# kamperh/segmentalist

Measured on AMD Instinct MI355X. Metric: Gibbs sweeps/sec (10k utts, D=100, K=1000) at 1/2/4/8 MI355X, higher is better.
Workload: dtype fp16 one-product filter + fp16x2 second stage, float32 reference arithmetic for the results; 1 GPU; SegmentalKMeansWordseg batch-synchronous sweep (BASELINE.json configs[2]); utterances=10000, landmarks_per_utt=20, n_slices_max=6, embeddings=1050000, D=100, K=1000, parallelism=utterance shards x1, ONE all-gather of the packed block statistics per sweep, collective=none (single process), sweep_launch=plain launches, corpus=one device holds all rows, device_memory_allocated_bytes_rank0=1237140480, components_after=815

## Files before the change

### include/segk.h

```cpp
#ifndef SEGK_H
#define SEGK_H

#include <stdint.h>

#ifdef __cplusplus
extern "C" {
#endif

#define SEGK_OK 0
#define SEGK_ERR_ARG (-1)
#define SEGK_ERR_HIP (-2)
#define SEGK_ERR_NO_DEVICE (-3)
#define SEGK_ERR_UNSUPPORTED (-4)

#define SEGK_F32 0
#define SEGK_F64 1

typedef struct segk_ctx segk_ctx;

int32_t segk_create(int32_t device_id, segk_ctx **out_ctx);
int32_t segk_destroy(segk_ctx *ctx);
const char *segk_last_error(void);
#define SEGK_ABI_VERSION 15
int32_t segk_abi_version(void);

int32_t segk_profile_enable(segk_ctx *ctx, int32_t on);
int32_t segk_profile_read(segk_ctx *ctx, float *ms_out, int64_t *rows_out, int32_t max);
int32_t segk_profile_last_kind(segk_ctx *ctx);
int32_t segk_profile_last_launches(segk_ctx *ctx);

int32_t segk_graph_begin(segk_ctx *ctx, void *stream);
int32_t segk_graph_end(segk_ctx *ctx, void *stream, void **exec_out);
int32_t segk_graph_launch(segk_ctx *ctx, void *exec, void *stream);
int32_t segk_graph_destroy(segk_ctx *ctx, void *exec);

typedef struct segk_corpus {
    const void *X;
    const float *X32;
    int32_t x_dtype;
    int32_t D;
    int64_t n_emb;
    int64_t ldx;
    int64_t ld32;
    const float *xnorm;
    const int32_t *vec_ids;
    const double *durations;
    const int32_t *lengths;
    int32_t n_utt;
    int32_t N_max;
    const void *Xb3;
    int32_t sp_pieces;
    int32_t band_W;
    const int32_t *band_ids;
    const double *band_dur;
} segk_corpus;

int32_t segk_corpus_prepare(segk_ctx *ctx, const segk_corpus *c, float *X32_out, float *xnorm_out,
                            void *stream);
int64_t segk_corpus_b3_bytes(int64_t n_emb, int32_t D);
int32_t segk_corpus_prepare_b3(segk_ctx *ctx, const segk_corpus *c, void *Xb3_out, int32_t pieces,
                               void *stream);

typedef struct segk_kmeans {
    void *means;
    double *mean_numerators;
    int64_t *counts;
    const void *random_means;
    int32_t *assignments;
    int32_t *K;
    int32_t K_max;
    float *tiles;
    double *mnorm_max;
    float *tiles_b3;
} segk_kmeans;

int64_t segk_kmeans_tiles_floats(int32_t K_max, int32_t D);
int32_t segk_kmeans_mark_duplicates(segk_ctx *ctx, const segk_corpus *c, const segk_kmeans *m, int32_t *n_marked,
                                    void *stream);
int64_t segk_kmeans_tiles_b3_floats(int32_t K_max, int32_t D);

int32_t segk_kmeans_init_stats(segk_ctx *ctx, const segk_corpus *c, segk_kmeans *m, void *stream);

int32_t segk_kmeans_prepare(segk_ctx *ctx, const segk_corpus *c, segk_kmeans *m, void *stream);

typedef struct segk_cand {
    int32_t *k;
    float *f;
    double *s;
    int32_t *queue;
    int32_t *count;
} segk_cand;

int32_t segk_kmeans_score(segk_ctx *ctx, const segk_corpus *c, const segk_kmeans *m,
                          const int32_t *ids, int64_t row0, int64_t n, const segk_cand *cand,
                          int32_t *status, void *stream);

int32_t segk_kmeans_score_hinted(segk_ctx *ctx, const segk_corpus *c, const segk_kmeans *m,
                                 const int32_t *ids, int64_t row0, int64_t n, const segk_cand *cand,
                                 const int32_t *hint_remap, int32_t *status, void *stream);

int32_t segk_kmeans_clear_queue(segk_ctx *ctx, const segk_cand *cand, void *stream);
int32_t segk_kmeans_filter(segk_ctx *ctx, const segk_corpus *c, const segk_kmeans *m,
                           const int32_t *ids, int64_t row0, int64_t n, const segk_cand *cand,
                           void *stream);
int32_t segk_kmeans_resolve(segk_ctx *ctx, const segk_corpus *c, const segk_kmeans *m,
                            const int32_t *ids, int64_t row0, int64_t n, const segk_cand *cand,
                            int32_t *status, void *stream);

int32_t segk_kmeans_stage_counts(segk_ctx *ctx, const segk_cand *cand, int32_t *out, void *stream);

int32_t segk_kmeans_hint_feedback(segk_ctx *ctx, uint32_t *launched, uint32_t *seen, int32_t *permille);

int32_t segk_kmeans_delta_stats(segk_ctx *ctx, int32_t *out);

int32_t segk_kmeans_exact_max(segk_ctx *ctx, const segk_corpus *c, const segk_kmeans *m,
                              const int32_t *ids, int64_t n, const segk_cand *cand,
                              double *out_max, int32_t *out_arg, void *stream);

int32_t segk_kmeans_neg_sqrd_norm(segk_ctx *ctx, const segk_corpus *c, const segk_kmeans *m,
                                  int64_t row, void *out, void *stream);

int32_t segk_kmeans_segment(segk_ctx *ctx, const segk_corpus *c, const segk_kmeans *m,
                            const int32_t *utts, int32_t utt0, int32_t n_utts,
                            int32_t n_slices_min, int32_t n_slices_max, double wip,
                            const segk_cand *cand, uint8_t *boundaries, int32_t *old_tok,
                            int32_t *new_tok, int32_t *new_k, int32_t *n_old, int32_t *n_new,
                            int32_t *n_flag, double *out_total, int32_t *status, void *stream);

int32_t segk_kmeans_update_utt(segk_ctx *ctx, const segk_corpus *c, segk_kmeans *m,
                               int32_t utt, const int32_t *old_tok, const int32_t *new_tok,
                               const int32_t *new_k, const int32_t *n_old, const int32_t *n_new,
                               int32_t *status, void *stream);

int32_t segk_kmeans_add_item(segk_ctx *ctx, const segk_corpus *c, segk_kmeans *m, int64_t i,
                             int32_t k, int32_t *status, void *stream);
int32_t segk_kmeans_del_item(segk_ctx *ctx, const segk_corpus *c, segk_kmeans *m, int64_t i,
                             int32_t *status, void *stream);
int32_t segk_kmeans_clean_components(segk_ctx *ctx, const segk_corpus *c, segk_kmeans *m,
                                     int32_t *status, void *stream);

int32_t segk_kmeans_del_component(segk_ctx *ctx, const segk_corpus *c, segk_kmeans *m, int32_t k,
                                  int32_t *status, void *stream);

int32_t segk_kmeans_sequential_sweep(segk_ctx *ctx, const segk_corpus *c, segk_kmeans *m,
                                     const int32_t *order, int32_t n_order, int32_t n_slices_min,
                                     int32_t n_slices_max, double wip, const segk_cand *cand,
                                     uint64_t *keys_scratch, uint8_t *boundaries, int32_t *old_tok,
                                     int32_t *new_tok, int32_t *new_k, int32_t *n_old, int32_t *n_new,
                                     int32_t *n_flag, double *out_total, int32_t *status, void *stream);

int64_t segk_kmeans_batch_record_words(int32_t K_max, int32_t D, int32_t n_blocks_local, int32_t flag_cap,
                                       int32_t flag_row_bytes);
int32_t segk_kmeans_batch_scratch_words(int32_t K_max, int64_t n_slots, int32_t n_blocks_local, int64_t *sorted_words,
                                        int64_t *koff_words);
int32_t segk_kmeans_batch_partials(segk_ctx *ctx, const segk_corpus *c, const segk_kmeans *m,
                                   const int32_t *blk_lo, int32_t n_blocks_local,
                                   const int32_t *new_tok, const int32_t *new_k, const int32_t *n_flag,
                                   const double *out_total, int32_t *sorted_scratch,
                                   int32_t *koff_scratch, double *record, int32_t flag_cap, int32_t flag_rows,
                                   double *out_scalars, void *stream);
int32_t segk_kmeans_batch_finalize(segk_ctx *ctx, const segk_corpus *c, segk_kmeans *m,
                                   int32_t utt_lo, int32_t utt_hi, const double *records,
                                   int32_t n_blocks_total, int32_t n_blocks_per_rank,
                                   int64_t rank_stride, int32_t flag_cap, int32_t flag_rows, int32_t my_rank,
                                   int32_t *new_k, int32_t *remap_scratch, double *out_scalars,
                                   int32_t *status, void *stream);
int32_t segk_kmeans_batch_record(segk_ctx *ctx, const segk_corpus *c, const segk_kmeans *m, int32_t utt_lo,
                                 int32_t utt_hi, const int32_t *new_tok, const int32_t *new_k,
                                 const int32_t *status, double *out_scalars, void *stream);
int32_t segk_kmeans_assignments_from_tokens(segk_ctx *ctx, const segk_corpus *c, segk_kmeans *m,
                                            int32_t utt_lo, int32_t utt_hi, const int32_t *new_tok,
                                            const int32_t *new_k, const int32_t *n_new,
                                            void *stream);

int32_t segk_kmeans_sum_neg_sqrd_norm(segk_ctx *ctx, const segk_corpus *c, const segk_kmeans *m,
                                      double *out, void *stream);

typedef struct segk_fbgmm {
    int32_t cov_type;
    int32_t K_max;
    double alpha;
    double lms;
    double k_0, v_0;
    const double *prior_a;
    const double *prior_b;
    const double *prior_c;
    double *stat_a;
    double *stat_b;
    double *log_prod;
    double *pred;
    int64_t *counts;
    int32_t *assignments;
    int32_t *K;
    int64_t *lm_unigram;
    int64_t *lm_bigram;
    double lm_lambda, lm_a, lm_b;
    double *kconst;
} segk_fbgmm;

int32_t segk_fbgmm_record_metrics(segk_ctx *ctx, const segk_corpus *c, const struct segk_fbgmm *f,
                                  int32_t urn, double urn_a, double *out, void *stream);

int32_t segk_fbgmm_init_stats(segk_ctx *ctx, const segk_corpus *c, segk_fbgmm *f, void *stream);

int32_t segk_fbgmm_update(segk_ctx *ctx, const segk_corpus *c, segk_fbgmm *f, int32_t op,
                          int32_t utt, int64_t item, int32_t k, const uint8_t *boundaries,
                          void *stream);

int32_t segk_fbgmm_score(segk_ctx *ctx, const segk_corpus *c, const segk_fbgmm *f,
                         const int32_t *ids, int64_t row0, int64_t n, double *out, void *stream);

int32_t segk_fbgmm_pred_vector(segk_ctx *ctx, const segk_corpus *c, const segk_fbgmm *f,
                               int64_t row, double *out, void *stream);

int32_t segk_unigram_segment(segk_ctx *ctx, const segk_corpus *c, int32_t utt, int32_t viterbi,
                             int32_t n_slices_min, int32_t n_slices_max, double wip,
                             double time_power_term, double log_p_continue, double anneal_temp,
                             const double *score, const double *ustream, int64_t *ucursor,
                             int64_t ucap, uint8_t *boundaries, int32_t *new_tok, int32_t *n_new,
                             double *out_logprob, int32_t *status, void *stream);

int32_t segk_fbgmm_assign(segk_ctx *ctx, const segk_corpus *c, segk_fbgmm *f, int32_t utt,
                          int32_t map_assign, int32_t j_prev, double anneal_temp, const int32_t *new_tok,
                          const int32_t *n_new, const double *ustream, int64_t *ucursor,
                          int64_t ucap, int32_t *status, void *stream);

int32_t segk_fbgmm_sequential_sweep(segk_ctx *ctx, const segk_corpus *c, segk_fbgmm *f, const int32_t *order, int32_t n_order,
                                    const int32_t *row_start, int32_t viterbi, int32_t map_assign, int32_t n_slices_min,
                                    int32_t n_slices_max, double wip, double time_power_term, double log_p_continue,
                                    double anneal_temp_fb, double anneal_temp_am, double *score, const double *ustream,
                                    int64_t *ucursor, int64_t ucap, uint8_t *boundaries, int32_t *new_tok, int32_t *n_new,
                                    double *out_logprob, int32_t *status, void *stream);

int32_t segk_fbgmm_gibbs_items(segk_ctx *ctx, const segk_corpus *c, segk_fbgmm *f, const int32_t *ids,
                               int64_t n, int32_t consider_unassigned, double anneal_temp,
                               const double *ustream, int64_t *ucursor, int64_t ucap, int32_t *status,
                               void *stream);

typedef struct {
    int32_t n_slices, n_blocks;
    int32_t u_max;
    int32_t fast_dp;
    const int32_t *utt_range;
    const int32_t *row_range;
    double *partials;
    double *cnt;
    double *mean_t, *q_t;
    double *lconst, *zconst, *half;
    double *scal;
    int32_t *slot;
    int32_t *lm_tok;
    uint64_t seed;
    float *y;
    int64_t ldy;
    float *tiles32;
    void *y16;
    float *tiles16;
    float *rows32;
    double *consts16;
    const double *prior_rows;
    const double *centre;
    float *tab32;
} segk_fbatch;

int32_t segk_fbb_collect(segk_ctx *ctx, const segk_corpus *c, const uint8_t *boundaries,
                         int32_t *new_tok, int32_t *n_new, void *stream);
// ... 87 lines not shown
```

### segmentalist_amd/_abi.py

```python
import ctypes as C
import os
import subprocess

_HERE = os.path.dirname(os.path.abspath(__file__))
LIB_PATH = os.environ.get("SEGK_LIB_PATH") or os.path.join(_HERE, "libsegk.so")

SEGK_F32, SEGK_F64 = 0, 1
SEGK_ERR_UNSUPPORTED = -4
ABI_VERSION = 15


class SegkError(RuntimeError):
    pass


class Corpus(C.Structure):
    _fields_ = [
        ("X", C.c_void_p), ("X32", C.c_void_p), ("x_dtype", C.c_int32), ("D", C.c_int32),
        ("n_emb", C.c_int64), ("ldx", C.c_int64), ("ld32", C.c_int64), ("xnorm", C.c_void_p),
        ("vec_ids", C.c_void_p), ("durations", C.c_void_p), ("lengths", C.c_void_p),
        ("n_utt", C.c_int32), ("N_max", C.c_int32), ("Xb3", C.c_void_p), ("sp_pieces", C.c_int32), ("band_W", C.c_int32),
        ("band_ids", C.c_void_p), ("band_dur", C.c_void_p),
    ]


class KMeansDev(C.Structure):
    _fields_ = [
        ("means", C.c_void_p), ("mean_numerators", C.c_void_p), ("counts", C.c_void_p),
        ("random_means", C.c_void_p), ("assignments", C.c_void_p), ("K", C.c_void_p),
        ("K_max", C.c_int32), ("tiles", C.c_void_p), ("mnorm_max", C.c_void_p), ("tiles_b3", C.c_void_p),
    ]


class FbatchDev(C.Structure):
    _fields_ = [
        ("n_slices", C.c_int32), ("n_blocks", C.c_int32), ("u_max", C.c_int32), ("fast_dp", C.c_int32),
        ("utt_range", C.c_void_p), ("row_range", C.c_void_p), ("partials", C.c_void_p), ("cnt", C.c_void_p),
        ("mean_t", C.c_void_p), ("q_t", C.c_void_p), ("lconst", C.c_void_p), ("zconst", C.c_void_p),
        ("half", C.c_void_p), ("scal", C.c_void_p), ("slot", C.c_void_p), ("lm_tok", C.c_void_p),
        ("seed", C.c_uint64), ("y", C.c_void_p), ("ldy", C.c_int64), ("tiles32", C.c_void_p),
        ("y16", C.c_void_p), ("tiles16", C.c_void_p), ("rows32", C.c_void_p), ("consts16", C.c_void_p),
        ("prior_rows", C.c_void_p), ("centre", C.c_void_p), ("tab32", C.c_void_p),
    ]


class CandDev(C.Structure):
    _fields_ = [("k", C.c_void_p), ("f", C.c_void_p), ("s", C.c_void_p), ("queue", C.c_void_p),
                ("count", C.c_void_p)]


class FbgmmDev(C.Structure):
    _fields_ = [
        ("cov_type", C.c_int32), ("K_max", C.c_int32), ("alpha", C.c_double), ("lms", C.c_double),
        ("k_0", C.c_double), ("v_0", C.c_double), ("prior_a", C.c_void_p), ("prior_b", C.c_void_p),
        ("prior_c", C.c_void_p), ("stat_a", C.c_void_p), ("stat_b", C.c_void_p), ("log_prod", C.c_void_p),
        ("pred", C.c_void_p), ("counts", C.c_void_p), ("assignments", C.c_void_p), ("K", C.c_void_p),
        ("lm_unigram", C.c_void_p), ("lm_bigram", C.c_void_p), ("lm_lambda", C.c_double), ("lm_a", C.c_double),
        ("lm_b", C.c_double), ("kconst", C.c_void_p),
    ]


_P = C.c_void_p
_i32, _i64, _f64, _u64 = C.c_int32, C.c_int64, C.c_double, C.c_uint64
_CP, _KP, _FP, _DP = C.POINTER(Corpus), C.POINTER(KMeansDev), C.POINTER(FbgmmDev), C.POINTER(CandDev)
_BP = C.POINTER(FbatchDev)

SIGNATURES = {
    "segk_create": (_i32, [_i32, C.POINTER(_P)]),
    "segk_destroy": (_i32, [_P]),
    "segk_last_error": (C.c_char_p, []),
    "segk_abi_version": (_i32, []),
    "segk_corpus_prepare": (_i32, [_P, _CP, _P, _P, _P]),
    "segk_kmeans_tiles_floats": (_i64, [_i32, _i32]),
    "segk_kmeans_prepare": (_i32, [_P, _CP, _KP, _P]),
    "segk_kmeans_mark_duplicates": (_i32, [_P, _CP, _KP, _P, _P]),
    "segk_kmeans_init_stats": (_i32, [_P, _CP, _KP, _P]),
    "segk_kmeans_score": (_i32, [_P, _CP, _KP, _P, _i64, _i64, _DP, _P, _P]),
    "segk_kmeans_score_hinted": (_i32, [_P, _CP, _KP, _P, _i64, _i64, _DP, _P, _P, _P]),
    "segk_kmeans_clear_queue": (_i32, [_P, _DP, _P]),
    "segk_kmeans_filter": (_i32, [_P, _CP, _KP, _P, _i64, _i64, _DP, _P]),
    "segk_kmeans_resolve": (_i32, [_P, _CP, _KP, _P, _i64, _i64, _DP, _P, _P]),
    "segk_kmeans_stage_counts": (_i32, [_P, _DP, C.POINTER(_i32), _P]),
    "segk_kmeans_hint_feedback": (_i32, [_P, C.POINTER(C.c_uint32), C.POINTER(C.c_uint32), C.POINTER(_i32)]),
    "segk_kmeans_delta_stats": (_i32, [_P, C.POINTER(_i32)]),
    "segk_kmeans_exact_max": (_i32, [_P, _CP, _KP, _P, _i64, _DP, _P, _P, _P]),
    "segk_kmeans_neg_sqrd_norm": (_i32, [_P, _CP, _KP, _i64, _P, _P]),
    "segk_kmeans_segment": (_i32, [_P, _CP, _KP, _P, _i32, _i32, _i32, _i32, _f64, _DP, _P, _P, _P, _P, _P, _P,
                                   _P, _P, _P, _P]),
    "segk_dp_tri": (_i32, [_P, _i32, _P, _P, _P, _i32, _i32, _i32, _f64, _f64, _P, _i64, _P, _i64, _P, _P, _P,
                           _P, _i64, _P]),
    "segk_kmeans_update_utt": (_i32, [_P, _CP, _KP, _i32, _P, _P, _P, _P, _P, _P, _P]),
    "segk_kmeans_sequential_sweep": (_i32, [_P, _CP, _KP, _P, _i32, _i32, _i32, _f64, _DP, _P, _P, _P, _P, _P, _P, _P, _P, _P,
                                            _P, _P]),
    "segk_kmeans_add_item": (_i32, [_P, _CP, _KP, _i64, _i32, _P, _P]),
    "segk_kmeans_del_item": (_i32, [_P, _CP, _KP, _i64, _P, _P]),
    "segk_kmeans_clean_components": (_i32, [_P, _CP, _KP, _P, _P]),
    "segk_kmeans_del_component": (_i32, [_P, _CP, _KP, _i32, _P, _P]),
    "segk_kmeans_batch_record_words": (_i64, [_i32, _i32, _i32, _i32, _i32]),
    "segk_kmeans_batch_scratch_words": (_i32, [_i32, _i64, _i32, C.POINTER(_i64), C.POINTER(_i64)]),
    "segk_kmeans_batch_partials": (_i32, [_P, _CP, _KP, _P, _i32, _P, _P, _P, _P, _P, _P, _P, _i32, _i32, _P, _P]),
    "segk_kmeans_batch_finalize": (_i32, [_P, _CP, _KP, _i32, _i32, _P, _i32, _i32, _i64, _i32, _i32, _i32, _P, _P, _P, _P,
                                          _P]),
    "segk_kmeans_batch_record": (_i32, [_P, _CP, _KP, _i32, _i32, _P, _P, _P, _P, _P]),
    "segk_kmeans_assignments_from_tokens": (_i32, [_P, _CP, _KP, _i32, _i32, _P, _P, _P, _P]),
    "segk_kmeans_sum_neg_sqrd_norm": (_i32, [_P, _CP, _KP, _P, _P]),
    "segk_fbgmm_record_metrics": (_i32, [_P, _CP, _FP, _i32, _f64, _P, _P]),
    "segk_fbgmm_init_stats": (_i32, [_P, _CP, _FP, _P]),
    "segk_fbgmm_update": (_i32, [_P, _CP, _FP, _i32, _i32, _i64, _i32, _P, _P]),
    "segk_fbgmm_score": (_i32, [_P, _CP, _FP, _P, _i64, _i64, _P, _P]),
    "segk_fbgmm_pred_vector": (_i32, [_P, _CP, _FP, _i64, _P, _P]),
    "segk_unigram_segment": (_i32, [_P, _CP, _i32, _i32, _i32, _i32, _f64, _f64, _f64, _f64, _P, _P, _P, _i64, _P,
                                    _P, _P, _P, _P, _P]),
    "segk_fbgmm_assign": (_i32, [_P, _CP, _FP, _i32, _i32, _i32, _f64, _P, _P, _P, _P, _i64, _P, _P]),
    "segk_fbgmm_gibbs_items": (_i32, [_P, _CP, _FP, _P, _i64, _i32, _f64, _P, _P, _i64, _P, _P]),
    "segk_fbgmm_sequential_sweep": (_i32, [_P, _CP, _FP, _P, _i32, _P, _i32, _i32, _i32, _i32, _f64, _f64, _f64, _f64, _f64,
                                           _P, _P, _P, _i64, _P, _P, _P, _P, _P, _P]),
    "segk_fbb_collect": (_i32, [_P, _CP, _P, _P, _P, _P]),
    "segk_fbb_partials": (_i32, [_P, _CP, _FP, _BP, _i32, _i32, _i32, _P, _P, _P]),
    "segk_fbb_prepare": (_i32, [_P, _CP, _FP, _BP, _i32, _P]),
    "segk_fbb_score": (_i32, [_P, _CP, _FP, _BP, _i32, _i32, _i32, _P, _P, _P]),
    "segk_fbb_score_diag32": (_i32, [_P, _CP, _FP, _BP, _i32, _i32, _i32, _P, _P, _P]),
    "segk_calibrate_vlog": (_i32, [_P, C.POINTER(_f64), _P]),
    "segk_fbb_make_y": (_i32, [_P, _CP, _BP, _P]),
    "segk_fbb_prior_rows": (_i32, [_P, _CP, _FP, _P, _P]),
    "segk_fbb_score_f32": (_i32, [_P, _CP, _FP, _BP, _P, _i64, _P, _P]),
    "segk_fbb_segment": (_i32, [_P, _CP, _FP, _BP, _i32, _i32, _i32, _P, _u64, _i32, _i32, _f64, _f64, _f64, _P, _P,
                                _P, _P, _P, _P, _P]),
    "segk_fbb_assign": (_i32, [_P, _CP, _FP, _BP, _i32, _i32, _i32, _P, _u64, _f64, _P, _P, _P, _i64, _P]),
    "segk_fbb_assign_diag32": (_i32, [_P, _CP, _FP, _BP, _i32, _i32, _i32, _P, _u64, _f64, _P, _P, _P]),
    "segk_fbb_segment_map": (_i32, [_P, _CP, _FP, _BP, _i32, _i32, _i32, _P, _u64, _i32, _i32, _f64, _f64, _P, _P, _P, _P,
                                    _P, _P, _P]),
    "segk_fbb_assign_map": (_i32, [_P, _CP, _FP, _BP, _i32, _i32, _i32, _P, _u64, _P, _P, _i32, _P]),
    "segk_fbb_step_diag32": (_i32, [_P, _CP, _FP, _BP, _i32, _i32, _i32, _P, _u64, _i32, _i32, _f64, _f64, _f64, _f64,
                                    _P, _P, _P, _P, _P, _P, _P]),
    "segk_fbb_token_scores": (_i32, [_P, _CP, _FP, _BP, _P, _i64, _P, _i64, _P]),
    "segk_fbb_set_probe": (_i32, [_P, _P, _P, _i64]),
    "segk_fbi_assign": (_i32, [_P, _CP, _FP, _BP, _i32, _i32, _i32, _P, _u64, _f64, _i32, _P, _P, _P, _i64, _P]),
    "segk_fbt_assign": (_i32, [_P, _CP, _FP, _BP, _i32, _i32, _i32, _P, _P, _u64, _f64, _P, _P, _P, _i64, _P]),
    "segk_fbb_lm_apply": (_i32, [_P, _CP, _FP, _BP, _i32, _i32, _P]),
    "segk_fbb_lm_fill": (_i32, [_P, _CP, _FP, _BP, _i32, _i32, _i32, _P, _P, _P, _P]),
    "segk_fbb_canonical": (_i32, [_P, _CP, _FP, _BP, _P, _P]),
    "segk_corpus_prepare_b3": (_i32, [_P, _CP, _P, _i32, _P]),
    "segk_corpus_b3_bytes": (_i64, [_i64, _i32]),
    "segk_kmeans_tiles_b3_floats": (_i64, [_i32, _i32]),
    "segk_graph_begin": (_i32, [_P, _P]),
    "segk_graph_end": (_i32, [_P, _P, C.POINTER(_P)]),
    "segk_graph_launch": (_i32, [_P, _P, _P]),
    "segk_graph_destroy": (_i32, [_P, _P]),
    "segk_profile_enable": (_i32, [_P, _i32]),
    "segk_profile_read": (_i32, [_P, _P, _P, _i32]),
    "segk_profile_last_kind": (_i32, [_P]),
    "segk_profile_last_launches": (_i32, [_P]),
    "segk_logsumexp": (_f64, [_P, _i64]),
    "segk_draw": (_i32, [_P, _i64, _f64]),
    "segk_sum_doubles": (_f64, [_P, _i64]),
    "segk_sum_ints": (_i64, [_P, _i64]),
    "segk_sum_log": (_f64, [_P, _i64]),
    "segk_sum_square_a_times_b": (_f64, [_P, _P, _i64]),
}

_lib = None


def build(force=False):
    if force and os.path.exists(LIB_PATH):
        os.remove(LIB_PATH)
    subprocess.check_call(["make", "-C", os.path.join(_HERE, "csrc"), "-s"])
    if not os.path.exists(LIB_PATH):
        raise SegkError("building libsegk.so failed")


def lib():
    global _lib
    if _lib is None:
        if not os.path.exists(LIB_PATH):
            raise SegkError(
                "%s not found: build it with `python -c 'import __graft_entry__ as g; g.build()'` "
                "or `make -C segmentalist_amd/csrc`.  segmentalist_amd has no CPU fallback." % LIB_PATH)
        L = C.CDLL(LIB_PATH)
        for name, (res, args) in SIGNATURES.items():
            try:
                fn = getattr(L, name)
            except AttributeError:
                raise SegkError("libsegk.so does not export %s (stale build?)" % name)
            fn.restype = res
            fn.argtypes = args
        got = int(L.segk_abi_version())
        if got != ABI_VERSION:
            raise SegkError("libsegk.so reports ABI version %d, this binding is written against %d (include/segk.h "
                            "SEGK_ABI_VERSION): rebuild the library (`make -C segmentalist_amd/csrc`)" % (got, ABI_VERSION))
        _lib = L
    return _lib


def check(rc):
    if rc != 0:
        raise SegkError("libsegk error %d: %s" % (rc, lib().segk_last_error().decode()))


_ctx = {}


def ctx(device_index=None):
    import torch
    if not torch.cuda.is_available():
        raise SegkError("no ROCm device visible: segmentalist_amd runs its hot path on MI355X only "
                        "(there is no CPU fallback)")
    if device_index is None:
        device_index = torch.cuda.current_device()
    if device_index not in _ctx:
        h = C.c_void_p()
        check(lib().segk_create(int(device_index), C.byref(h)))
        _ctx[device_index] = h
    return _ctx[device_index]


def stream():
    import torch
    return C.c_void_p(torch.cuda.current_stream().cuda_stream)


def ptr(t):
    if t is None:
        return None
    return C.c_void_p(t.data_ptr())
```

### segmentalist_amd/csrc/segk_host.cpp

```cpp
#include <math.h>
#include <stdarg.h>
#include <stdlib.h>
#include <map>
#include <mutex>
#include <tuple>

#include "segk_internal.h"

static thread_local char g_err[512] = "";

void segk_set_error(const char *fmt, ...)
{
    va_list ap;
    va_start(ap, fmt);
    vsnprintf(g_err, sizeof(g_err), fmt, ap);
    va_end(ap);
}

int segk_ws_realloc(segk_ctx *ctx, void **buf, size_t bytes, hipStream_t st)
{
    SEGK_REQUIRE(!ctx->capturing, "workspaces must exist before a graph capture (run the sequence once first)");
    SEGK_CHECK_HIP(hipStreamSynchronize(st));
    if (*buf) (void)hipFree(*buf);
    *buf = nullptr;
// ... 103 lines not shown
        if (ctx->fb_fp_dev) (void)hipFree(ctx->fb_fp_dev);
        if (ctx->fbs_buf) (void)hipFree(ctx->fbs_buf);
        if (ctx->flag_ovf) (void)hipFree(ctx->flag_ovf);
        if (ctx->hint_part) (void)hipFree(ctx->hint_part);
        if (ctx->ws_u64) (void)hipFree(ctx->ws_u64);
        if (ctx->hint_fb) (void)hipFree(ctx->hint_fb);
        if (ctx->delta_buf) (void)hipFree(ctx->delta_buf);
        if (ctx->delta_host) (void)hipHostFree((void *)ctx->delta_host);
        if (ctx->pre_thr) (void)hipFree(ctx->pre_thr);
        if (ctx->band_mask) (void)hipFree(ctx->band_mask);
        if (ctx->miss_host) (void)hipHostFree((void *)ctx->miss_host);
        if (ctx->brute_ws) (void)hipFree(ctx->brute_ws);
        if (ctx->pre_queue) (void)hipFree(ctx->pre_queue);
        if (ctx->row_hash) (void)hipFree(ctx->row_hash);
        if (ctx->rb_sorted) (void)hipFree(ctx->rb_sorted);
        if (ctx->rb_koff) (void)hipFree(ctx->rb_koff);
        if (ctx->rb_misc) (void)hipFree(ctx->rb_misc);
        if (ctx->rb_term) (void)hipFree(ctx->rb_term);
        if (ctx->fc_terms) (void)hipFree(ctx->fc_terms);
        if (ctx->fcb_ll) (void)hipFree(ctx->fcb_ll);
        if (ctx->fbi_z) (void)hipFree(ctx->fbi_z);
        if (ctx->fbt_tok) (void)hipFree(ctx->fbt_tok);
        for (int i = 0; i < SEGK_PROF_SLOTS; i++)
            for (int j = 0; j < 2; j++)
                if (ctx->prof_ev[i][j]) (void)hipEventDestroy(ctx->prof_ev[i][j]);
    }
    free(ctx);
    return SEGK_OK;
}

int32_t segk_profile_enable(segk_ctx *ctx, int32_t on)
{
    SEGK_REQUIRE(ctx, "ctx");
    if (on)
        for (int i = 0; i < SEGK_PROF_SLOTS; i++)
            for (int j = 0; j < 2; j++)
                if (!ctx->prof_ev[i][j]) SEGK_CHECK_HIP(hipEventCreate(&ctx->prof_ev[i][j]));
    ctx->prof_on = on > 0 ? on : 0;
    ctx->prof_calls = 0;
    ctx->prof_n = 0;
    if (on) ctx->prof_kind = -1;
    return SEGK_OK;
}

int32_t segk_profile_read(segk_ctx *ctx, float *ms_out, int64_t *rows_out, int32_t max)
{
    SEGK_REQUIRE(ctx && ms_out && rows_out, "arguments");
    const int have = ctx->prof_n < SEGK_PROF_SLOTS ? ctx->prof_n : SEGK_PROF_SLOTS;
    const int n = have < max ? have : max;
    for (int i = 0; i < n; i++) {
        const int slot = (ctx->prof_n - n + i) % SEGK_PROF_SLOTS;
        SEGK_CHECK_HIP(hipEventSynchronize(ctx->prof_ev[slot][1]));
        SEGK_CHECK_HIP(hipEventElapsedTime(&ms_out[i], ctx->prof_ev[slot][0], ctx->prof_ev[slot][1]));
        rows_out[i] = ctx->prof_rows[slot];
    }
    return n;
}

int32_t segk_profile_last_kind(segk_ctx *ctx)
{
    return ctx ? ctx->prof_kind : -1;
}

int32_t segk_profile_last_launches(segk_ctx *ctx)
{
    return ctx && ctx->prof_launches > 0 ? ctx->prof_launches : 1;
}

int32_t segk_graph_begin(segk_ctx *ctx, void *stream)
{
    SEGK_REQUIRE(ctx && stream, "segk_graph_begin needs a context and a non-default stream");
    SEGK_REQUIRE(!ctx->capturing, "a capture is already open on this context");
    SEGK_REQUIRE(!ctx->prof_on, "segk_profile_enable(1) records events between launches: not inside a capture");
    SEGK_CHECK_HIP(hipStreamBeginCapture((hipStream_t)stream, hipStreamCaptureModeRelaxed));
    ctx->capturing = 1;
    return SEGK_OK;
}

int32_t segk_graph_end(segk_ctx *ctx, void *stream, void **exec_out)
{
    SEGK_REQUIRE(ctx && stream && exec_out, "arguments");
    SEGK_REQUIRE(ctx->capturing, "no capture open");
    ctx->capturing = 0;
    *exec_out = nullptr;
    hipGraph_t graph = nullptr;
    SEGK_CHECK_HIP(hipStreamEndCapture((hipStream_t)stream, &graph));
    hipGraphExec_t exec = nullptr;
    const hipError_t e = hipGraphInstantiate(&exec, graph, nullptr, nullptr, 0);
    (void)hipGraphDestroy(graph);
    if (e != hipSuccess) {
        segk_set_error("segk_graph_end: hipGraphInstantiate -> %s", hipGetErrorString(e));
        return SEGK_ERR_HIP;
    }
    *exec_out = (void *)exec;
    return SEGK_OK;
}

int32_t segk_graph_launch(segk_ctx *ctx, void *exec, void *stream)
{
    (void)ctx;
    SEGK_REQUIRE(exec, "exec");
    SEGK_CHECK_HIP(hipGraphLaunch((hipGraphExec_t)exec, (hipStream_t)stream));
    return SEGK_OK;
}

int32_t segk_graph_destroy(segk_ctx *ctx, void *exec)
{
    (void)ctx;
    if (exec) SEGK_CHECK_HIP(hipGraphExecDestroy((hipGraphExec_t)exec));
    return SEGK_OK;
}

int32_t segk_kmeans_stage_counts(segk_ctx *ctx, const segk_cand *cand, int32_t *out, void *stream)
{
    SEGK_REQUIRE(ctx && cand && cand->count && out, "arguments");
    hipStream_t st = (hipStream_t)stream;
    out[0] = -1;
    int32_t hdr[16] = {0};
    if (ctx->pre_queue) SEGK_CHECK_HIP(hipMemcpyAsync(hdr, ctx->pre_queue, sizeof(hdr), hipMemcpyDeviceToHost, st));
    SEGK_CHECK_HIP(hipMemcpyAsync(&out[1], cand->count, sizeof(int32_t), hipMemcpyDeviceToHost, st));
    SEGK_CHECK_HIP(hipStreamSynchronize(st));
    if (ctx->pre_queue) {
        out[0] = 0;
        for (int i = 0; i < 16; i++) out[0] += hdr[i];
    }
    return SEGK_OK;
}

int32_t segk_kmeans_hint_feedback(segk_ctx *ctx, uint32_t *launched, uint32_t *seen, int32_t *permille)
{
    SEGK_REQUIRE(ctx && launched && seen && permille, "arguments");
    *launched = ctx->miss_seq;
    *seen = 0;
    *permille = 0;
    if (ctx->miss_host) {
        const unsigned long long w = *ctx->miss_host;
        *seen = (uint32_t)(w >> 32);
        *permille = (int32_t)(w & 0xffffffffull);
    }
    return SEGK_OK;
}

int32_t segk_kmeans_delta_stats(segk_ctx *ctx, int32_t *out)
{
    SEGK_REQUIRE(ctx && out, "arguments");
    out[0] = -1; out[1] = 0; out[2] = 0; out[3] = 0;
    if (ctx->delta_host) {
        out[0] = ctx->delta_host[0] - 1;
        for (int i = 1; i < 4; i++) out[i] = ctx->delta_host[i];
    }
    return SEGK_OK;
}

double segk_logsumexp(const double *a, int64_t n)
{
    double mx = a[0], s = 0.0;
    for (int64_t j = 1; j < n; j++)
        if (a[j] > mx) mx = a[j];
    for (int64_t j = 0; j < n; j++) s += exp(a[j] - mx);
    return log(s) + mx;
}

int32_t segk_draw(const double *p_k, int64_t n, double u)
{
    for (int64_t i = 0; i < n; i++) {
        u = u - p_k[i];
        if (u < 0) return (int32_t)i;
    }
    return (int32_t)(n - 1);
}

double segk_sum_doubles(const double *y, int64_t n)
{
    double s = y[0];
    for (int64_t i = 1; i < n; i++) s += y[i];
    return s;
}

int64_t segk_sum_ints(const int64_t *y, int64_t n)
{
    int64_t s = y[0];
    for (int64_t i = 1; i < n; i++) s += y[i];
    return s;
}

double segk_sum_log(const double *y, int64_t n)
{
    double s = log(y[0]);
    for (int64_t i = 1; i < n; i++) s += log(y[i]);
    return s;
}

double segk_sum_square_a_times_b(const double *a, const double *b, int64_t n)
{
    double s = 0.0;
    for (int64_t i = 0; i < n; i++) s += a[i] * a[i] * b[i];
    return s;
}

}


static std::mutex g_attr_mu;
static std::map<std::pair<int, const void *>, size_t> g_dyn_lds;
static std::map<std::tuple<int, const void *, int, size_t>, int> g_occupancy;

hipError_t segk_dyn_lds(const void *fn, size_t lds)
{
    if (lds <= 48 * 1024) return hipSuccess;
    int dev = 0;
    hipError_t e = hipGetDevice(&dev);
    if (e != hipSuccess) return e;
    std::lock_guard<std::mutex> lock(g_attr_mu);
    size_t &have = g_dyn_lds[std::make_pair(dev, fn)];
    if (have >= lds) return hipSuccess;
    e = hipFuncSetAttribute(fn, hipFuncAttributeMaxDynamicSharedMemorySize, (int)lds);
    if (e == hipSuccess) have = lds;
    return e;
}

hipError_t segk_occupancy(const void *fn, int threads, size_t lds, int *wg_per_cu)
{
    int dev = 0;
    hipError_t e = hipGetDevice(&dev);
    if (e != hipSuccess) return e;
    {
        std::lock_guard<std::mutex> lock(g_attr_mu);
        auto it = g_occupancy.find(std::make_tuple(dev, fn, threads, lds));
        if (it != g_occupancy.end()) {
            *wg_per_cu = it->second;
            return hipSuccess;
        }
    }
    e = segk_dyn_lds(fn, lds);
    if (e != hipSuccess) return e;
    int occ = 0;
    e = hipOccupancyMaxActiveBlocksPerMultiprocessor(&occ, fn, threads, lds);
    if (e != hipSuccess) return e;
    *wg_per_cu = occ > 0 ? occ : 1;
    std::lock_guard<std::mutex> lock(g_attr_mu);
    g_occupancy[std::make_tuple(dev, fn, threads, lds)] = *wg_per_cu;
    return hipSuccess;
}
```

### segmentalist_amd/csrc/segk_internal.h

```cpp
#pragma once
#include <hip/hip_runtime.h>
#include <stdint.h>
#include <stdio.h>
#include <stdlib.h>
#include <string.h>

#include "../../include/segk.h"

#define SEGK_WS_ENTRIES (256 * 1024)
#define SEGK_PROF_SLOTS 256

struct segk_ctx {
    int device_id;
    int n_cu;
    char arch[64];
    int32_t *ws_k;
    float *ws_f;
    unsigned long long *ws_u64;
    int32_t *pre_queue;
    int64_t pre_cap;
    float *sp2_part;
    int32_t *sp2_ticket;
    int64_t sp2_blocks;
    void *chain_buf;
    size_t chain_bytes;
    double *fb_ktab;
    int64_t fb_ktab_n;
    double fb_ktab_v0;
    int fb_ktab_D;
    double *fb_ptab;
    int64_t fb_ptab_n;
    unsigned long long fb_ptab_fp;
    int64_t fb_ptab_rows;
    int fb_ptab_D;
    unsigned long long *fb_fp_dev;
    int fb_ptab_nt, fb_ptab_cov;
    double fb_ptab_k0, fb_ptab_v0;
    void *fbchain_buf;
    size_t fbchain_bytes;
    void *fbchain_lm;
    size_t fbchain_lm_bytes;
    void *fbchain_terms;
    size_t fbchain_terms_bytes;
    int32_t *fbs_buf;
    size_t fbs_bytes;
    const void *fbb_scal_zeroed;
    const void *fbb_scal_stream;
    int prof_launches;
    int32_t *defer_zero;
    int pre_zeroed;
    int capturing;
    unsigned long long *row_hash;
    const void *row_hash_means;
    int32_t *rb_sorted;
    int64_t rb_cap;
    int32_t *rb_koff;
    int rb_K;
    int32_t *rb_misc;
    double *rb_term;
    double *fc_terms;
    int64_t fc_terms_n;
    double *fcb_ll;
    int64_t fcb_ll_n;
    double *fbi_z;
    int64_t fbi_z_n;
    int32_t *fbt_tok;
    int64_t fbt_tok_n;
    void *hint_part;
    size_t hint_part_bytes;
    float *pre_thr;
    int64_t pre_thr_cap;
    void *band_mask;
    size_t band_mask_bytes;
    volatile unsigned long long *miss_host;
    unsigned long long *miss_dev;
    unsigned int miss_seq;
    void *delta_buf;
    size_t delta_bytes;
    unsigned int delta_seq;
    int delta_valid;
    const void *delta_key[6];
    int64_t delta_key_n[5];
    int delta_pending;
    const void *delta_pending_remap, *delta_pending_K, *delta_pending_stream;
    int delta_pending_cap, delta_pending_budget, delta_pending_seq;
    volatile int32_t *delta_host;
    int32_t *delta_host_dev;
    void *hint_fb;
    unsigned int hint_fb_launch;
    unsigned long long *brute_ws;
    int64_t brute_ws_cap;
    int32_t *flag_ovf;
    int64_t flag_ovf_cap;
    double *probe_alpha, *probe_ll;
    int64_t probe_ll_ld;
    int prof_on, prof_n, prof_kind;
    unsigned int prof_calls;
    hipEvent_t prof_ev[SEGK_PROF_SLOTS][2];
    int64_t prof_rows[SEGK_PROF_SLOTS];
};

static inline bool segk_prof_now(segk_ctx *ctx)
{
    if (!ctx->prof_on) return false;
    return (ctx->prof_calls++ % (unsigned int)ctx->prof_on) == 0u;
}


void segk_set_error(const char *fmt, ...);

static inline int segk_env_int(const char *name, int dflt)
{
    const char *e = getenv(name);
    return e ? atoi(e) : dflt;
}

#ifdef SEGK_DEV
static inline int segk_dev_env(const char *name) { return segk_env_int(name, 0); }
#else
static inline int segk_dev_env(const char *) { return 0; }
#endif

int segk_rows_by_label(segk_ctx *ctx, const int32_t *labels, int64_t n, int K_max, const int32_t **blk_lo, int *n_blocks,
                       const int32_t **sorted, const int32_t **koff, void *stream);

#define SEGK_CHECK_HIP(expr)                                                                  \
    do {                                                                                      \
        hipError_t _e = (expr);                                                               \
        if (_e != hipSuccess) {                                                               \
            segk_set_error("%s:%d: %s -> %s", __FILE__, __LINE__, #expr, hipGetErrorString(_e)); \
            return SEGK_ERR_HIP;                                                              \
        }                                                                                     \
    } while (0)

#define SEGK_REQUIRE(cond, msg)                                             \
    do {                                                                    \
        if (!(cond)) {                                                      \
            segk_set_error("%s:%d: %s (%s)", __FILE__, __LINE__, msg, #cond); \
            return SEGK_ERR_ARG;                                            \
        }                                                                   \
    } while (0)

#define SEGK_LAUNCH_CHECK() SEGK_CHECK_HIP(hipGetLastError())

#define SEGK_REFUSE_FULLCOV(f, who)                                                                                 \
    do {                                                                                                            \
        if ((f) && (f)->cov_type == 2) {                                                                            \
            segk_set_error("%s: full-covariance components (cov_type 2) are not supported by this entry point", who); \
            return SEGK_ERR_UNSUPPORTED;                                                                            \
        }                                                                                                           \
    } while (0)
int segk_fc_check(const segk_corpus *c, const segk_fbgmm *f, const char *who);
int segk_fc_init_stats(segk_ctx *ctx, const segk_corpus *c, segk_fbgmm *f, void *stream);
int segk_fc_update(const segk_corpus *c, segk_fbgmm *f, int op, int utt, int64_t item, int k, const uint8_t *boundaries, void *stream);
int segk_fc_score(segk_ctx *ctx, const segk_corpus *c, const segk_fbgmm *f, const int32_t *ids, int64_t row0, int64_t n, double *out,
                  void *stream);
int segk_fc_pred_vector(const segk_corpus *c, const segk_fbgmm *f, int64_t row, double *out, void *stream);
int segk_fc_assign(const segk_corpus *c, segk_fbgmm *f, int utt, int map_assign, double anneal_temp, const int32_t *new_tok,
                   const int32_t *n_new, const double *ustream, int64_t *ucursor, int64_t ucap, int32_t *status, void *stream);
int segk_fc_gibbs_items(const segk_corpus *c, segk_fbgmm *f, const int32_t *ids, int64_t n, int consider_unassigned,
                        double anneal_temp, const double *ustream, int64_t *ucursor, int64_t ucap, int32_t *status, void *stream);

int segk_ws_realloc(segk_ctx *ctx, void **buf, size_t bytes, hipStream_t st);
template <class T, class N>
static inline int segk_ws_grow(segk_ctx *ctx, T **buf, N *have, N need, size_t bytes, hipStream_t st)
{
    if (*have >= need) return SEGK_OK;
    *have = 0;
    if (int rc = segk_ws_realloc(ctx, (void **)buf, bytes, st)) return rc;
    *have = need;
    return SEGK_OK;
}

hipError_t segk_dyn_lds(const void *fn, size_t lds);
hipError_t segk_occupancy(const void *fn, int threads, size_t lds, int *wg_per_cu);

static inline __host__ __device__ int segk_G(int D) { return (D + 3) / 4; }
#define SEGK_G_BUCKETS {1, 2, 4, 6, 8, 10, 13, 16, 20, 25, 26, 28, 32, 33, 34, 40, 50, 64, 75, 100}
static inline __host__ __device__ int segk_gmax(int D)
{
    const int b[] = SEGK_G_BUCKETS;
    int G = segk_G(D);
    for (unsigned i = 0; i < sizeof(b) / sizeof(b[0]); i++)
        if (G <= b[i]) return b[i];
    return -1;
}
static inline __host__ __device__ int segk_tile_stride(int D)
{
    int gm = segk_gmax(D);
    if (gm < 0) gm = segk_G(D);
    int f = gm * 128 + 32;
    return (f + 1023) / 1024 * 1024;
}
static inline __host__ __device__ int segk_n_tiles(int K_max) { return (K_max + 31) / 32; }

#define SEGK_SP_HEADER 64
static inline __host__ __device__ int segk_b3_dim(int pos)
{
    const int q = pos & 15, h = q >> 3, i = q & 7;
    return (pos & ~15) + 8 * (i >> 2) + 4 * h + (i & 3);
}
static inline __host__ __device__ int segk_b3_kp(int D) { return (D + 15) & ~15; }
static inline __host__ __device__ int segk_sp_tile_stride(int D, int P)
{
    return ((segk_b3_kp(D) / 16) * P * 256 + 32 + 1023) / 1024 * 1024;
}

int segk_launch_score_lse(segk_ctx *ctx, const float *Y, int64_t ldy, int D2, const int32_t *ids, int64_t row0, int64_t n,
                          const float *tiles, int n_tiles, double norm, double *out, void *stream);

int segk_sp_prepare_rows(const float *Y, int64_t ldy, int64_t n, int D2, void *img, void *stream);
int segk_sp_prepare_tiles(const float *rows, const double *consts, const double *rowmax2, int K, int D2, float *tiles_sp,
                          const void *ximg, void *stream);
int segk_launch_score_lse_sp(segk_ctx *ctx, const void *ximg, int D2, const int32_t *ids, int64_t row0, int64_t n,
                             const float *tiles_sp, int n_tiles, double norm, double *out, void *stream,
                             const int32_t *n_tiles_dev = nullptr);
int segk_launch_score_mat_sp(const void *ximg, int D2, const int32_t *ids, int64_t n, const float *tiles_sp, int n_tiles,
                             float *mat, int64_t mat_ld, void *stream, const int32_t *n_tiles_dev = nullptr, int tiles_hint = 0);
```

### segmentalist_amd/csrc/segk_kmeans_dev.h

```cpp
#pragma once
#include <stdlib.h>

#include "segk_internal.h"

typedef float f32x16 __attribute__((ext_vector_type(16)));

#define NEG_INF_D (-__builtin_huge_val())
#define NEG_INF_F (-__builtin_huge_valf())

template <typename T, typename TM, typename TX>
__device__ __forceinline__ T sqd(const TM &m, const TX *x, int d)
{
    T delta = (T)m[d] - (T)x[d];
    return delta * delta;
}

template <typename T, typename TM, typename TX>
__device__ T pw_base(const TM &m, const TX *x, int n)
{
    if (n < 8) {
        T res = (T)0;
        for (int i = 0; i < n; i++) res += sqd<T>(m, x, i);
        return res;
    }
// ... 525 lines not shown
            int i = idx - G * 128;
            int comp = tile * 32 + i;
            v = (comp < K_max) ? (float)(-0.5 * nrm[i]) : -3.0e38f;
        }
        T[idx] = v;
    }
}

__device__ __forceinline__ void dev_prepare_sp_tile(const float *means, int K_max, int D, float *tiles, const double *mnorm2,
                                                    const unsigned char *ximg, const double *consts, const int tile)
{
    typedef SegkPiece::T T;
    constexpr int P = 2;
    const int KS = segk_b3_kp(D) / 16;
    const int stride = segk_sp_tile_stride(D, P);
    const int eb = sp_exponent((float)(sqrt(*mnorm2) * (1.0 + 1e-6)));
    const int ea = ((const int *)ximg)[1];
    if (tile == 0 && threadIdx.x == 0) ((int *)tiles)[0] = eb;
    float *Tt = tiles + 1024 + (int64_t)tile * stride;
    T *Tb = (T *)Tt;
    __shared__ double nrm[32];
    constexpr int PITCH = 129;
    __shared__ float rowsl[32 * PITCH];
    const bool staged = D <= 128;
    const float *src = means + (int64_t)tile * 32 * D;
    if (staged) {
        const int nrow = K_max - tile * 32 < 32 ? K_max - tile * 32 : 32;
        for (int idx = threadIdx.x; idx < 32 * D; idx += blockDim.x) {
            const int ci = idx / D, d = idx - ci * D;
            rowsl[ci * PITCH + d] = ci < nrow ? src[idx] : 0.f;
        }
    }
    __syncthreads();
    SEGK_TSTAMP(4, 5);
    auto elem = [&](int ci, int d) -> float { return staged ? rowsl[ci * PITCH + d] : src[(int64_t)ci * D + d]; };
    {
        const int ci = threadIdx.x >> 3, sub = threadIdx.x & 7;
        const int comp = tile * 32 + ci;
        double s = 0.0, rs = 0.0;
        if (comp < K_max)
            for (int d = sub; d < D; d += 8) {
                const float mv = elem(ci, d);
                double v = (double)mv;
                s += v * v;
                rs += sp_resid2(ldexpf(mv, eb));
            }
        s += __shfl_xor(s, 1);
        s += __shfl_xor(s, 2);
        s += __shfl_xor(s, 4);
        if (sub == 0) nrm[ci] = s;
        rs += __shfl_xor(rs, 1);
        rs += __shfl_xor(rs, 2);
        rs += __shfl_xor(rs, 4);
        const float em = (float)(ldexp(sqrt(rs), -eb) * (1.0 + 1e-6));
        if (sub == 0 && comp < K_max) atomicMax((unsigned int *)tiles + 1, __float_as_uint(em));
    }
    __syncthreads();
    SEGK_TSTAMP(4, 6);
    for (int pr = threadIdx.x; pr < KS * 64; pr += blockDim.x) {
        const int sidx = pr >> 6, lane = pr & 63;
        const int ci = lane & 31;
        const bool live = tile * 32 + ci < K_max;
        SegkPiece::V8 out[P];
#pragma unroll
        for (int i = 0; i < 8; i++) {
            const int d = segk_b3_dim(16 * sidx + 8 * (lane >> 5) + i);
            const float v = (live && d < D) ? ldexpf(elem(ci, d), eb) : 0.f;
            T pc[P];
            split_sp(v, pc);
#pragma unroll
            for (int q = 0; q < P; q++) out[q][i] = pc[q];
        }
#pragma unroll
        for (int q = 0; q < P; q++) *reinterpret_cast<SegkPiece::V8 *>(Tb + ((sidx * P + q) * 64 + lane) * 8) = out[q];
    }
    for (int idx = threadIdx.x; idx < stride - KS * P * 256; idx += blockDim.x) {
        float v = 0.f;
        if (idx < 32) {
            const int comp = tile * 32 + idx;
            if (consts) v = (comp < K_max && consts[comp] > -1e37) ? (float)ldexp(consts[comp], ea + eb) : -3.0e38f;
            else v = (comp < K_max) ? (float)ldexp(-0.5 * nrm[idx], ea + eb) : -3.0e38f;
        }
        Tt[KS * P * 256 + idx] = v;
    }
}

#define SEGK_DUP_TB 4096
__device__ __forceinline__ void dev_dup_table(unsigned long long *keys, int32_t *first, const unsigned long long *row_hash, int K_max)
{
    const int tid = threadIdx.x;
    for (int i = tid; i < SEGK_DUP_TB; i += blockDim.x) { keys[i] = 0ull; first[i] = 0x7fffffff; }
    __syncthreads();
    for (int k = tid; k < K_max; k += blockDim.x) {
        const unsigned long long h = row_hash[k];
        for (unsigned slot = (unsigned)(h >> 20) & (SEGK_DUP_TB - 1);; slot = (slot + 1) & (SEGK_DUP_TB - 1)) {
            const unsigned long long prev = atomicCAS(&keys[slot], 0ull, h);
            if (prev == 0ull || prev == h) { atomicMin(&first[slot], k); break; }
        }
    }
    __syncthreads();
}
__device__ __forceinline__ int dev_dup_first(const unsigned long long *keys, const int32_t *first, unsigned long long h)
{
    unsigned slot = (unsigned)(h >> 20) & (SEGK_DUP_TB - 1);
    while (keys[slot] != h) slot = (slot + 1) & (SEGK_DUP_TB - 1);
    return first[slot];
}

static __global__ void k_zero_two(int32_t *a, int32_t *b)
{
    if (threadIdx.x == 0) *a = 0;
    if (threadIdx.x < 16) b[threadIdx.x] = 0;
}
static inline void segk_flush_deferred_zero(segk_ctx *ctx, hipStream_t st)
{
    if (ctx && ctx->defer_zero) {
        hipLaunchKernelGGL(k_zero_two, dim3(1), dim3(64), 0, st, ctx->defer_zero, ctx->pre_queue);
        ctx->defer_zero = nullptr;
    }
}

int segk_kmeans_prepare_impl(segk_ctx *ctx, const segk_corpus *c, segk_kmeans *m, void *stream, bool mnorm_zeroed);
int segk_dispatch_score_f32(segk_ctx *ctx, const segk_corpus *c, const segk_kmeans *m, const ScoreArgs &A, hipStream_t st);
int segk_dispatch_score_sp(segk_ctx *ctx, const ScoreArgs &A, int ks, hipStream_t st);
int segk_launch_sp_second(segk_ctx *ctx, const ScoreArgs &B, int ks, hipStream_t st);
int segk_launch_clean(const segk_corpus *c, segk_kmeans *m, int32_t *status, hipStream_t st, int32_t *relog = nullptr);
int segk_launch_seq_chain(segk_ctx *ctx, const segk_corpus *c, segk_kmeans *m, const int32_t *order, int n_order, int n_slices_max,
                          double wip, uint8_t *boundaries, int32_t *old_tok, int32_t *new_tok, int32_t *new_k, int32_t *n_old,
                          int32_t *n_new, int32_t *n_flag, double *out_total, int32_t *status, hipStream_t st);
int segk_dispatch_score_pre(segk_ctx *ctx, const ScoreArgs &A, int ks, hipStream_t st);
#define SEGK_HINT_MAX_TPR 32
#define SEGK_HINT_MAX_RANGES 4
struct HintPlan {
    int max_tiles;
    int n_ranges, tpr;
    size_t map_bytes;
};
static inline bool segk_hint_plan(int K_max, int ks, int n_tiles, HintPlan *p)
{
    const size_t lds_bytes = 160 * 1024, tile_bytes = (size_t)(ks * 256 + 32) * sizeof(float);
    p->map_bytes = (size_t)((K_max + 3) & ~3) * sizeof(int32_t);
    if (p->map_bytes + tile_bytes > lds_bytes) return false;
    p->max_tiles = (int)((lds_bytes - p->map_bytes) / tile_bytes);
    if (p->max_tiles > SEGK_HINT_MAX_TPR) p->max_tiles = SEGK_HINT_MAX_TPR;
    p->n_ranges = (n_tiles + p->max_tiles - 1) / p->max_tiles;
    if (p->n_ranges < 1) p->n_ranges = 1;
    p->tpr = (n_tiles + p->n_ranges - 1) / p->n_ranges;
    return p->n_ranges <= SEGK_HINT_MAX_RANGES;
}
int segk_dispatch_score_hint(segk_ctx *ctx, const ScoreArgs &A, const int32_t *remap, const int32_t *K_dev, int64_t n_emb, int ks, hipStream_t st);

#define SEGK_DELTA_MODE 1
#define SEGK_DELTA_SKIP 2
#define SEGK_PREP_THREADS 256
#define SEGK_PREP_COLS 4
struct DeltaPrepArgs {
    const float *tiles_hdr;
    int n_tiles, stride;
    int K_max, D;
    const float *means32;
    const int32_t *remap;
    const int32_t *K_dev;
    int valid;
    int hint_valid;
    int cap;
    int budget;
    int seq;
    int redo;
    int32_t *ctl, *colchg, *meanchg;
    float *snap_img;
    float *packed;
    float *snap_means;
};
struct DeltaPrepLds { int chg[32], slot[32], nonid, last, n_chg, n_nonid, old[5]; };

static __device__ __forceinline__ void delta_prep_means_rows(const DeltaPrepArgs &P, int wg, int n_wg)
{
    const int lane = threadIdx.x & 63, wave = threadIdx.x >> 6;
    constexpr int NWV = SEGK_PREP_THREADS / 64;
    for (int k = wg * NWV + wave; k < P.K_max; k += n_wg * NWV) {
        const int *cur = (const int *)(P.means32 + (int64_t)k * P.D);
        int *snap = (int *)(P.snap_means + (int64_t)k * P.D);
        bool chg = false;
        for (int d = lane; d < P.D; d += 64) {
            const int c = cur[d];
            chg |= c != snap[d];
            snap[d] = c;
        }
        const bool any = __any(chg);
        if (lane == 0) {
            const bool before = P.redo && P.meanchg[k] != 0;
            P.meanchg[k] = (any || before || !P.hint_valid) ? 1 : 0;
            if (any) atomicAdd(P.ctl + 5 + (P.seq & 1), 1);
        }
    }
}

static __device__ __forceinline__ bool delta_prep_tile(const DeltaPrepArgs &P, const int KS, const int t, const int e_cur, DeltaPrepLds &S)
{
    const int tid = threadIdx.x, lane = tid & 63, wave = tid >> 6;
    constexpr int NWV = SEGK_PREP_THREADS / 64;
    const int TL = KS * 256 + 32, c_off = KS * 512;
    const int c = lane & 31;
    const float *g = P.tiles_hdr + 1024 + (int64_t)t * P.stride;
    const float *q = P.snap_img + 4 + (int64_t)t * TL;
    const bool all = !P.valid || e_cur != (P.redo ? P.ctl[18] : ((const int *)P.snap_img)[0]);
    if (tid < 32) S.chg[tid] = 0;
    if (tid == 0) S.nonid = 0;
    __syncthreads();
    if (!all) {
        bool chg = false;
        for (int ks = wave; ks < KS; ks += NWV) {
            const int4 a = *reinterpret_cast<const int4 *>(g + ks * 512 + lane * 4);
            const int4 b = *reinterpret_cast<const int4 *>(q + ks * 256 + lane * 4);
            chg |= a.x != b.x || a.y != b.y || a.z != b.z || a.w != b.w;
        }
        if (tid < 32) chg |= __float_as_int(g[c_off + c]) != __float_as_int(q[KS * 256 + c]);
        if (chg) atomicOr(&S.chg[c], 1);
    }
    if (P.remap && tid >= SEGK_PREP_THREADS - 32) {
        int K_lab = P.K_dev ? *P.K_dev : P.K_max;
        const int K_prev = P.ctl[P.redo ? 15 : 8];
        if (K_lab < K_prev) K_lab = K_prev;
        if (K_lab > P.K_max || !P.valid) K_lab = P.K_max;
        const int k = t * 32 + c;
        if (k < K_lab && P.remap[k] != k) S.nonid = 1;
    }
    __syncthreads();
    if (wave == 0) {
        const bool chg = lane < 32 && (all || S.chg[lane] != 0);
        if (lane < 32) P.colchg[t * 32 + lane] = chg ? 1 : 0;
        const unsigned long long mask = __ballot(chg);
        unsigned int base = 0;
        if (lane == 0) {
            S.old[0] = P.ctl[P.redo ? 12 : 5 + ((P.seq + 1) & 1)];
            S.old[1] = P.ctl[P.redo ? 13 : 4];
            S.old[2] = P.ctl[P.redo ? 14 : 7];
            S.old[3] = P.ctl[P.redo ? 15 : 8];
            S.old[4] = P.redo ? P.ctl[18] : ((const int *)P.snap_img)[0];
            const int n_own = __popcll(mask), nonid = S.nonid != 0 ? 1 : 0;
            const unsigned long long old = atomicAdd(reinterpret_cast<unsigned long long *>(P.ctl + 16),
                                                     (unsigned long long)n_own | (1ull << 32) | ((unsigned long long)nonid << 48));
            base = (unsigned int)old;
            S.last = (int)((old >> 32) & 0xffffull) == P.n_tiles - 1 ? 1 : 0;
            S.n_chg = (int)base + n_own;
            S.n_nonid = (int)(old >> 48) + nonid;
        }
        base = __shfl(base, 0);
        if (lane < 32) S.slot[lane] = chg ? (int)base + __builtin_amdgcn_mbcnt_hi((unsigned)(mask >> 32), __builtin_amdgcn_mbcnt_lo((unsigned)mask, 0)) : -1;
    }
    __syncthreads();
    {
        const int sl = S.slot[c];
        if (P.valid && sl >= 0 && sl < P.cap * 32) {
            float *o = P.packed + (int64_t)(sl >> 5) * P.stride;
            const int l2 = (lane & 32) + (sl & 31);
            for (int ks = wave; ks < KS; ks += NWV)
                *reinterpret_cast<int4 *>(o + ks * 512 + l2 * 4) = *reinterpret_cast<const int4 *>(g + ks * 512 + lane * 4);
            if (tid < 32) o[c_off + (sl & 31)] = g[c_off + c];
        }
    }
    return S.last != 0;
}

static __device__ __forceinline__ void delta_prep_mode(const DeltaPrepArgs &P, const int KS, const int e_cur, DeltaPrepLds &S)
{
    const int tid = threadIdx.x, c_off = KS * 512;
    const int n_chg = S.n_chg, n_packed = (n_chg + 31) >> 5;
    const bool nonid = S.n_nonid != 0;
    const int moved_prev = S.old[0], acc = S.old[1], chg_prev = S.old[2];
    const bool at_rest = n_chg > 0 && n_chg == chg_prev && moved_prev == 0;
    const bool delta = P.valid && !nonid && n_packed <= P.cap && !at_rest && acc + n_packed <= P.budget;
    if (tid == 0) {
        P.ctl[12] = moved_prev; P.ctl[13] = acc; P.ctl[14] = chg_prev; P.ctl[15] = S.old[3]; P.ctl[18] = S.old[4];
        P.ctl[4] = delta ? acc + n_packed : 0;
        P.ctl[5 + ((P.seq + 1) & 1)] = 0;
        P.ctl[7] = delta ? n_chg : 0;
        P.ctl[8] = P.K_dev ? *P.K_dev : P.K_max;
        P.ctl[0] = (delta ? SEGK_DELTA_MODE : 0) | ((P.hint_valid && !nonid) ? SEGK_DELTA_SKIP : 0);
        P.ctl[1] = n_chg;
        P.ctl[2] = delta ? n_packed : 0;
        P.ctl[3] = 0;
        P.ctl[16] = 0;
        P.ctl[17] = 0;
        if (!delta) ((int *)P.snap_img)[0] = e_cur;
    }
    if (delta && tid < 32 && n_chg + tid < n_packed * 32) {
        const int sl = n_chg + tid;
        P.packed[(int64_t)(sl >> 5) * P.stride + c_off + (sl & 31)] = -3.0e38f;
    }
}
static inline int segk_delta_prep_row_blocks(int K_max) { return (K_max + 7) / 8 < 128 ? (K_max + 7) / 8 : 128; }
bool segk_delta_prep_fold(segk_ctx *ctx, const segk_corpus *c, const segk_kmeans *m, const int32_t *remap, hipStream_t st, DeltaPrepArgs *P);
static inline void segk_delta_pending_drop(segk_ctx *ctx)
{
    if (ctx && ctx->delta_pending == 1) ctx->delta_pending = 2;
}
bool segk_band_applies(const ScoreArgs &A);
int segk_launch_band(segk_ctx *ctx, const ScoreArgs &A, const float *thr, int64_t call_rows, int32_t *lab_last, int ks, hipStream_t st);
int segk_launch_seq_score(const segk_corpus *c, const segk_kmeans *m, int utt, const segk_cand *cand, unsigned long long *keys,
                          hipStream_t st);
int segk_launch_update_utt(const segk_corpus *c, segk_kmeans *m, int utt, const int32_t *old_tok, const int32_t *new_tok,
                           const int32_t *new_k, const int32_t *n_old, const int32_t *n_new, int32_t *status, hipStream_t st);
int segk_resolve_on(segk_ctx *ctx, const segk_corpus *c, const segk_kmeans *m, const int32_t *ids, int64_t row0, int64_t n,
                    const segk_cand *cand, int32_t *status, void *stream);
```

### segmentalist_amd/csrc/segk_score_band.hip

```cpp
#include "segk_kmeans_dev.h"

#define SEGK_BAND_TPR 8
#define SEGK_BAND_MAX_RANGES 8

struct BandArgs {
    const unsigned char *ximg;
    const int32_t *queue;
    const float *thr;
    const int32_t *n_dev;
    int cap;
    const float *tiles;
    int n_tiles, n_ranges;
    int4 *mask;
    unsigned long long *fb;
    unsigned int fb_seq;
    int64_t fb_rows;
};

#define SEGK_BAND_QUAD(MK, AO, q_, THR, FIRST)                                                                       \
    do {                                                                                                              \
        if (FIRST) {       \
            MK = (MK << 1) | (AO[4 * (q_)] >= THR ? 1u : 0u);                                                         \
            asm volatile("v_cmp_ge_f32 vcc, %1, %4\n\tv_addc_co_u32 %0, vcc, %0, %0, vcc\n\t"                        \
                         "v_cmp_ge_f32 vcc, %2, %4\n\tv_addc_co_u32 %0, vcc, %0, %0, vcc\n\t"                        \
                         "v_cmp_ge_f32 vcc, %3, %4\n\tv_addc_co_u32 %0, vcc, %0, %0, vcc"                            \
                         : "+v"(MK) : "v"(AO[4 * (q_) + 1]), "v"(AO[4 * (q_) + 2]), "v"(AO[4 * (q_) + 3]), "v"(THR) : "vcc"); \
        } else {                                                                                                      \
            asm volatile("v_cmp_ge_f32 vcc, %1, %5\n\tv_addc_co_u32 %0, vcc, %0, %0, vcc\n\t"                        \
                         "v_cmp_ge_f32 vcc, %2, %5\n\tv_addc_co_u32 %0, vcc, %0, %0, vcc\n\t"                        \
                         "v_cmp_ge_f32 vcc, %3, %5\n\tv_addc_co_u32 %0, vcc, %0, %0, vcc\n\t"                        \
                         "v_cmp_ge_f32 vcc, %4, %5\n\tv_addc_co_u32 %0, vcc, %0, %0, vcc"                            \
                         : "+v"(MK) : "v"(AO[4 * (q_)]), "v"(AO[4 * (q_) + 1]), "v"(AO[4 * (q_) + 2]), "v"(AO[4 * (q_) + 3]), "v"(THR) : "vcc"); \
        }                                                                                                             \
    } while (0)

template <int KS>
__global__ __launch_bounds__(256, 2) void k_kmeans_band_rs(BandArgs B)
{
    typedef _Float16 T;
    typedef SegkPiece::V8 V8;
    constexpr int P = 2, KP = KS * 16, NW = 4, NBLK = 2, TPR = SEGK_BAND_TPR;
    constexpr int STRIDE = (KS * P * 256 + 32 + 1023) / 1024 * 1024;
    constexpr int TL = KS * 256 + 32;
    extern __shared__ __attribute__((aligned(16))) float lds[];
    const int tid = threadIdx.x, lane = tid & 63, wave = tid >> 6;
    const int j = lane & 31, h = lane >> 5;
    const int R = B.n_ranges;
    int count = *B.n_dev;
    if (count > B.cap) count = B.cap;
    const int64_t n_groups = ((int64_t)count + 32 * NBLK - 1) / (32 * NBLK);
    if (B.fb && blockIdx.x == 0 && tid == 0) {
        const unsigned long long pm = B.fb_rows > 0 ? (unsigned long long)((int64_t)count * 1000 / B.fb_rows) : 0ull;
        __hip_atomic_store(B.fb, ((unsigned long long)B.fb_seq << 32) | pm, __ATOMIC_RELEASE, __HIP_MEMORY_SCOPE_SYSTEM);
    }
    int range, wgr, n_wgr;
    if ((gridDim.x & 7) == 0 && ((gridDim.x >> 3) % R) == 0) {
        const int xcd = blockIdx.x & 7, idx = blockIdx.x >> 3;
        range = idx % R;
        wgr = (idx / R) * 8 + xcd;
        n_wgr = gridDim.x / R;
    } else {
        n_wgr = gridDim.x / R;
        range = blockIdx.x % R;
        wgr = blockIdx.x / R;
        if (wgr >= n_wgr) return;
    }
    if ((int64_t)wgr * NW >= n_groups) return;
    const int t_lo = range * TPR;
    int nt = B.n_tiles - t_lo;
    if (nt > TPR) nt = TPR;
    if (nt < 0) nt = 0;
    const T *plane0 = (const T *)(B.ximg + SEGK_SP_HEADER);
    const int64_t n_slots = (int64_t)n_wgr * NW;
    int64_t g = (int64_t)wgr * NW + wave;

#define SEGK_BD_IDS(g_, RID)                                                                 \
    do {                                                                                      \
        _Pragma("unroll") for (int b = 0; b < NBLK; b++) {                                    \
            const int64_t r = (g_) * (32 * NBLK) + 32 * b + j;                                \
            RID[b] = r < count ? B.queue[r] : -1;                                             \
        }                                                                                     \
    } while (0)
#define SEGK_BD_LOAD(g_, XB, THR, RID)                                                                           \
    do {                                                                                                          \
        _Pragma("unroll") for (int b = 0; b < NBLK; b++) {                                                        \
            const int64_t r = (g_) * (32 * NBLK) + 32 * b + j;                                                    \
            const int64_t rowid = RID[b] >= 0 ? (int64_t)RID[b] : 0;            \
            const T *xp = plane0 + rowid * KP + 8 * h;                                                            \
            _Pragma("unroll") for (int s = 0; s < KS; s++) XB[b][s] = *reinterpret_cast<const V8 *>(xp + 16 * s); \
            THR[b] = (r < count && RID[b] >= 0) ? B.thr[r] : __builtin_huge_valf();                               \
        }                                                                                                         \
    } while (0)

    V8 a[KS];
    f32x16 cs;
    auto load_a = [&](int t, int s) { a[s] = *reinterpret_cast<const V8 *>((const T *)(lds + t * TL) + (s * 64 + lane) * 8); };
    auto load_cs = [&](int t) {
        const float *cv = lds + t * TL + KS * 256 + 4 * h;
#pragma unroll
        for (int q = 0; q < 4; q++) {
            const float4 c4 = *reinterpret_cast<const float4 *>(cv + 8 * q);
            cs[4 * q + 0] = c4.x; cs[4 * q + 1] = c4.y; cs[4 * q + 2] = c4.z; cs[4 * q + 3] = c4.w;
        }
    };

#define SEGK_BD_UNIT(XB, N_, AN, AO, MK, THR, DRAIN, REFILL, tn_)                                                     \
    do {                                                                                                              \
        _Pragma("unroll") for (int s = 0; s < KS; s++) {                                                              \
            asm volatile("" : "+v"(a[s]));                                                                            \
            AN = __builtin_amdgcn_mfma_f32_32x32x16_f16(a[s], XB[N_][s], s == 0 ? cs : AN, 0, 0, 0);                  \
            asm volatile("" : "+v"(AN), "+v"(THR));     \
            if (REFILL) {                                                                                             \
                load_a(tn_, s);                                                                                       \
                if (s == 0) load_cs(tn_);                                                                             \
            }                                                                                                         \
            __builtin_amdgcn_sched_barrier(0);                                                                        \
            constexpr int SL = KS > 1 ? KS - 1 : 1;                                                                   \
            const int q_lo = KS > 1 ? ((s - 1) * 4 + SL - 1) / SL : 0, q_hi = KS > 1 ? (s * 4 + SL - 1) / SL : 4;     \
            if (DRAIN && (KS == 1 || s >= 1)) {                                                                       \
                if (0 >= q_lo && 0 < q_hi) SEGK_BAND_QUAD(MK, AO, 0, THR, true);                                      \
                if (1 >= q_lo && 1 < q_hi) SEGK_BAND_QUAD(MK, AO, 1, THR, false);                                     \
                if (2 >= q_lo && 2 < q_hi) SEGK_BAND_QUAD(MK, AO, 2, THR, false);                                     \
                if (3 >= q_lo && 3 < q_hi) SEGK_BAND_QUAD(MK, AO, 3, THR, false);                                     \
            }                                                                                                         \
            __builtin_amdgcn_sched_barrier(0);                                                                        \
        }                                                                                                             \
    } while (0)

#define SEGK_BD_GROUP(g_, XB, THR)                                                                                     \
    do {                                                                                                               \
        unsigned int mk[NBLK][TPR / 2];                                                                                \
        _Pragma("unroll") for (int b = 0; b < NBLK; b++)                                                               \
            _Pragma("unroll") for (int w = 0; w < TPR / 2; w++) mk[b][w] = 0u;                                         \
        f32x16 acc0, acc1;                                                                                             \
        _Pragma("unroll") for (int t = 0; t < TPR; t++) {                                                              \
            const int tn = t + 1 < TPR ? t + 1 : 0;        \
            if (t == 0) SEGK_BD_UNIT(XB, 0, acc0, acc1, mk[1][0], THR[1], false, false, tn);                           \
            else        SEGK_BD_UNIT(XB, 0, acc0, acc1, mk[1][(t - 1) >> 1], THR[1], true, false, tn);                 \
            SEGK_BD_UNIT(XB, 1, acc1, acc0, mk[0][t >> 1], THR[0], true, true, tn);                                    \
        }                                                                                                              \
        SEGK_BAND_QUAD(mk[1][(TPR - 1) >> 1], acc1, 0, THR[1], true);                                                  \
        SEGK_BAND_QUAD(mk[1][(TPR - 1) >> 1], acc1, 1, THR[1], false);                                                 \
        SEGK_BAND_QUAD(mk[1][(TPR - 1) >> 1], acc1, 2, THR[1], false);                                                 \
        SEGK_BAND_QUAD(mk[1][(TPR - 1) >> 1], acc1, 3, THR[1], false);                                                 \
        _Pragma("unroll") for (int b = 0; b < NBLK; b++)                                                               \
            _Pragma("unroll") for (int w = 0; w < TPR / 2; w++) pend[b][w] = mk[b][w];                                 \
        pend_g = (g_);                                                                                                 \
    } while (0)

#define SEGK_BD_STORE()                                                                                                \
    do {                                                                                                               \
        if (pend_g >= 0) {                                                                                             \
            _Pragma("unroll") for (int b = 0; b < NBLK; b++) {                                                         \
                const int64_t r = pend_g * (32 * NBLK) + 32 * b + j;                                                   \
                if (r < count)                                                                                         \
                    B.mask[((int64_t)range * B.cap + r) * 2 + h] = make_int4((int)pend[b][0], (int)pend[b][1], (int)pend[b][2], (int)pend[b][3]); \
            }                                                                                                          \
        }                                                                                                              \
    } while (0)
    static_assert(TPR == 8, "four mask words per (row, lane half, range)");

    unsigned int pend[NBLK][TPR / 2];
    int64_t pend_g = -1;
    V8 xa[NBLK][KS], xb[NBLK][KS];
    float thr_a[NBLK], thr_b[NBLK];
    int32_t rid_a[NBLK], rid_b[NBLK];
    _Pragma("unroll") for (int b = 0; b < NBLK; b++) { rid_a[b] = -1; rid_b[b] = -1; thr_a[b] = 0.f; thr_b[b] = 0.f; }
    if (g < n_groups) SEGK_BD_IDS(g, rid_a);
    if (g + n_slots < n_groups) SEGK_BD_IDS(g + n_slots, rid_b);
    {
        constexpr int MAXB = TPR * KS;
        constexpr int PER_W = (MAXB + NW - 1) / NW;
        const int n_blk = nt * KS;
        float4 v[PER_W];
#pragma unroll
        for (int u = 0; u < PER_W; u++) {
            int c = wave + u * NW;
            const bool live = c < n_blk;
            if (!live) c = 0;
            const int t = c / KS, ks = c - t * KS;
            v[u] = make_float4(0.f, 0.f, 0.f, 0.f);
            if (live) v[u] = *reinterpret_cast<const float4 *>(B.tiles + (int64_t)(t_lo + t) * STRIDE + ks * (P * 256) + lane * 4);
        }
        float4 cv4 = make_float4(-3.0e38f, -3.0e38f, -3.0e38f, -3.0e38f);
        const bool is_c = tid < TPR * 8;
        if (is_c && (tid >> 3) < nt) cv4 = *reinterpret_cast<const float4 *>(B.tiles + (int64_t)(t_lo + (tid >> 3)) * STRIDE + KS * P * 256 + (tid & 7) * 4);
#pragma unroll
        for (int u = 0; u < PER_W; u++) {
            const int c = wave + u * NW;
            if (c < MAXB) {
                const int t = c / KS, ks = c - t * KS;
                *reinterpret_cast<float4 *>(lds + t * TL + ks * 256 + lane * 4) = v[u];
            }
        }
        if (is_c) *reinterpret_cast<float4 *>(lds + (tid >> 3) * TL + KS * 256 + (tid & 7) * 4) = cv4;
        static_assert(256 >= TPR * 8, "one thread per float4 of the constants");
    }
    if (g < n_groups) SEGK_BD_LOAD(g, xa, thr_a, rid_a);
    __syncthreads();
    if (g >= n_groups) return;
#pragma unroll
    for (int s = 0; s < KS; s++) load_a(0, s);
    load_cs(0);
    for (;;) {
        __builtin_amdgcn_s_waitcnt(0x0F70);
        const int64_t g1 = g + n_slots;
        if (g1 < n_groups) SEGK_BD_LOAD(g1, xb, thr_b, rid_b);
        if (g1 + n_slots < n_groups) SEGK_BD_IDS(g1 + n_slots, rid_a);
        SEGK_BD_STORE();
        SEGK_BD_GROUP(g, xa, thr_a);
        if (g1 >= n_groups) break;
        __builtin_amdgcn_s_waitcnt(0x0F70);
        g = g1 + n_slots;
        if (g < n_groups) SEGK_BD_LOAD(g, xa, thr_a, rid_a);
        if (g + n_slots < n_groups) SEGK_BD_IDS(g + n_slots, rid_b);
        SEGK_BD_STORE();
        SEGK_BD_GROUP(g1, xb, thr_b);
        if (g >= n_groups) break;
    }
    SEGK_BD_STORE();
#undef SEGK_BD_STORE
#undef SEGK_BD_GROUP
#undef SEGK_BD_UNIT
#undef SEGK_BD_LOAD
#undef SEGK_BD_IDS
}
#undef SEGK_BAND_QUAD

struct BandExactArgs {
    const int32_t *queue;
    const int32_t *n_dev;
    int cap;
    const int4 *mask;
    int n_ranges, K_max, D;
    const float *xrows32;
    int64_t ld32;
    const float *means32;
    segk_cand cand;
    int amb_cap;
    int32_t *lab_last;
    int64_t row0;
};

#define SEGK_BAND_CLIST 128
template <int D>
__global__ __launch_bounds__(256) void k_band_exact(BandExactArgs E)
{
    __shared__ int2 clist[4][SEGK_BAND_CLIST];
    __shared__ unsigned long long best[4][8];
    const int tid = threadIdx.x, lane = tid & 63, wv = tid >> 6;
    const int wpr = E.n_ranges * 8;
    const int rpw = 64 / wpr;
    int count = *E.n_dev;
    if (count > E.cap) count = E.cap;
    const int row_l = lane / wpr, w = lane - row_l * wpr;
    const int range = w >> 3, h = (w >> 2) & 1, ww = w & 3;
    const bool worker = row_l < rpw;
    constexpr int nblk = D / 8, rem = D & 7;
    const int grp = lane >> 3, a = lane & 7;
    const int64_t wave_g = ((int64_t)blockIdx.x * 256 + tid) >> 6, n_waves = ((int64_t)gridDim.x * 256) >> 6;
    for (int64_t q0 = wave_g * rpw; q0 < count; q0 += n_waves * rpw) {
        const int64_t q = q0 + row_l;
        unsigned int word = 0u;
        int32_t rid = -1;
        if (worker && q < count) {
            word = ((const unsigned int *)E.mask)[(((int64_t)range * E.cap + q) * 2 + h) * 4 + ww];
            rid = E.queue[q];
        }
        const int pc = __popc(word);
        int pre = pc;
#pragma unroll
        for (int off = 1; off < 64; off <<= 1) {
            const int o = __shfl_up(pre, off);
            if (lane >= off) pre += o;
        }
        const int total = __shfl(pre, 63);
        pre -= pc;
        if (lane < 8) best[wv][lane] = 0ull;
        const bool overflow = total > SEGK_BAND_CLIST;
        if (!overflow) {
            int at = pre;
            while (word != 0u) {
                const int pb = 31 - __clz((int)word);
                word &= ~(1u << pb);
                const int tile = range * SEGK_BAND_TPR + 2 * ww + (pb < 16 ? 1 : 0);
                const int qq = 15 - (pb & 15);
                const int comp = 32 * tile + 4 * h + (qq & 3) + 8 * (qq >> 2);
                clist[wv][at++] = make_int2(row_l, comp < E.K_max ? comp : -1);
            }
        }
        asm volatile("s_waitcnt lgkmcnt(0)" ::: "memory");
        if (!overflow) {
            for (int c0 = 0; c0 < total; c0 += 8) {
                const int c = c0 + grp;
                int2 cd = make_int2(0, -1);
                if (c < total) cd = clist[wv][c];
                const int32_t rid_c = __shfl(rid, cd.x * wpr);
                const bool live = cd.y >= 0 && rid_c >= 0;
                const float *mp = E.means32 + (int64_t)(live ? cd.y : 0) * D + a;
                const float *xp = E.xrows32 + (int64_t)(live ? rid_c : 0) * E.ld32 + a;
                float mv[nblk], xv[nblk], mt = 0.f, xt = 0.f;
#pragma unroll
                for (int b = 0; b < nblk; b++) mv[b] = mp[8 * b];
#pragma unroll
                for (int b = 0; b < nblk; b++) xv[b] = xp[8 * b];
                if constexpr (rem != 0) {
                    if (a < rem) { mt = mp[8 * nblk]; xt = xp[8 * nblk]; }
                }
                float r = 0.f;
#pragma unroll
                for (int b = 0; b < nblk; b++) {
                    const float dlt = mv[b] - xv[b];
                    const float t = dlt * dlt;
                    r = b == 0 ? t : r + t;
                }
                r = r + __shfl_xor(r, 1);
                r = r + __shfl_xor(r, 2);
                r = r + __shfl_xor(r, 4);
                if constexpr (rem != 0) {
                    const float dlt = mt - xt;
                    const float t = dlt * dlt;
#pragma unroll
                    for (int i = 0; i < rem; i++) r += __shfl(t, (lane & ~7) + i);
                }
                if (live && a == 0) {
                    const float sc = -r;
                    const unsigned int bits = __float_as_uint(sc);
                    const unsigned int ord = (bits & 0x80000000u) ? ~bits : (bits | 0x80000000u);
                    const unsigned long long pk = ((unsigned long long)ord << 32) | (unsigned long long)(0xffffffffu - (unsigned int)cd.y);
                    atomicMax(&best[wv][cd.x], pk);
                }
            }
        }
        asm volatile("s_waitcnt lgkmcnt(0)" ::: "memory");
        if (worker && q < count && w == 0) {
            const unsigned long long mine = overflow ? 0ull : best[wv][row_l];
            if (mine != 0ull) {
                const unsigned int ord = (unsigned int)(mine >> 32);
                const unsigned int bits = (ord & 0x80000000u) ? (ord & 0x7fffffffu) : ~ord;
                E.cand.k[rid] = (int32_t)(0xffffffffu - (unsigned int)(mine & 0xffffffffu));
                E.cand.s[rid] = (double)__uint_as_float(bits);
                if (E.lab_last) E.lab_last[(int64_t)rid - E.row0] = (int32_t)(0xffffffffu - (unsigned int)(mine & 0xffffffffu));
            } else {
                const int q2 = atomicAdd(E.cand.count, 1);
                if (q2 < E.amb_cap) E.cand.queue[q2] = rid;
            }
        }
        asm volatile("s_waitcnt lgkmcnt(0)" ::: "memory");
    }
}

template <int KS>
static int launch_band(segk_ctx *ctx, const ScoreArgs &A, const float *thr, int64_t call_rows, int32_t *lab_last, hipStream_t st)
{
    const int n_cu = ctx->n_cu;
    const int n_ranges = (A.n_tiles + SEGK_BAND_TPR - 1) / SEGK_BAND_TPR;
    SEGK_REQUIRE(n_ranges >= 1 && n_ranges <= SEGK_BAND_MAX_RANGES, "band stage: K_max out of range");
    const int cap = A.pre_cap;
    const size_t need = (size_t)n_ranges * (size_t)cap * 2 * sizeof(int4);
    if (int rc = segk_ws_grow(ctx, &ctx->band_mask, &ctx->band_mask_bytes, need, need, st)) return rc;
    BandArgs B{};
    B.ximg = (const unsigned char *)A.X32;
    B.queue = A.pre_queue;
    B.thr = thr;
    B.n_dev = A.pre_count;
    B.cap = cap;
    B.tiles = A.tiles + 1024;
    B.n_tiles = A.n_tiles;
    B.n_ranges = n_ranges;
    B.mask = (int4 *)ctx->band_mask;
    B.fb = ctx->miss_dev;
    B.fb_seq = ++ctx->miss_seq;
    B.fb_rows = call_rows;
    constexpr int TL = KS * 256 + 32;
    const size_t lds = (size_t)SEGK_BAND_TPR * TL * sizeof(float);
    int grid = (2 * n_cu / n_ranges) * n_ranges;
    {
        const int64_t steps = ((int64_t)cap + 255) / 256;
        if ((int64_t)grid / n_ranges > steps) grid = (int)steps * n_ranges;
    }
    SEGK_CHECK_HIP(segk_dyn_lds((const void *)k_kmeans_band_rs<KS>, lds));
    hipLaunchKernelGGL((k_kmeans_band_rs<KS>), dim3((unsigned)grid), dim3(256), lds, st, B);

    BandExactArgs E{};
    E.queue = A.pre_queue;
    E.n_dev = A.pre_count;
    E.cap = cap;
    E.mask = (const int4 *)ctx->band_mask;
    E.n_ranges = n_ranges;
    E.K_max = A.K_max;
    E.D = A.D;
    E.xrows32 = A.xrows32;
    E.ld32 = A.ld32;
    E.means32 = A.means32;
    E.cand = A.cand;
    E.amb_cap = A.amb_cap;
    E.lab_last = A.ids ? nullptr : lab_last;
    E.row0 = A.row0;
    const int rpw = 64 / (n_ranges * 8);
    int64_t grid4 = ((int64_t)cap + 4 * rpw - 1) / (4 * rpw);
    if (grid4 > 16 * (int64_t)n_cu) grid4 = 16 * (int64_t)n_cu;
    switch ((16 * KS - A.D) / 4) {
        case 0: hipLaunchKernelGGL((k_band_exact<16 * KS>), dim3((unsigned)grid4), dim3(256), 0, st, E); break;
        case 1: hipLaunchKernelGGL((k_band_exact<16 * KS - 4>), dim3((unsigned)grid4), dim3(256), 0, st, E); break;
        case 2: hipLaunchKernelGGL((k_band_exact<16 * KS - 8>), dim3((unsigned)grid4), dim3(256), 0, st, E); break;
        default: hipLaunchKernelGGL((k_band_exact<(16 * KS - 12 >= 8 ? 16 * KS - 12 : 8)>), dim3((unsigned)grid4), dim3(256), 0, st, E); break;
    }
    SEGK_LAUNCH_CHECK();
    return SEGK_OK;
}

bool segk_band_applies(const ScoreArgs &A)
{
    const int n_ranges = (A.n_tiles + SEGK_BAND_TPR - 1) / SEGK_BAND_TPR;
    return n_ranges >= 1 && n_ranges <= SEGK_BAND_MAX_RANGES && A.D % 4 == 0 && A.D >= 8 && A.D <= 128;
}

int segk_launch_band(segk_ctx *ctx, const ScoreArgs &A, const float *thr, int64_t call_rows, int32_t *lab_last, int ks, hipStream_t st)
{
    switch (ks) {
        case 1: return launch_band<1>(ctx, A, thr, call_rows, lab_last, st);
        case 2: return launch_band<2>(ctx, A, thr, call_rows, lab_last, st);
        case 3: return launch_band<3>(ctx, A, thr, call_rows, lab_last, st);
        case 4: return launch_band<4>(ctx, A, thr, call_rows, lab_last, st);
        case 5: return launch_band<5>(ctx, A, thr, call_rows, lab_last, st);
        case 6: return launch_band<6>(ctx, A, thr, call_rows, lab_last, st);
        case 7: return launch_band<7>(ctx, A, thr, call_rows, lab_last, st);
        case 8: return launch_band<8>(ctx, A, thr, call_rows, lab_last, st);
        default: break;
    }
    segk_set_error("band stage: D out of range");
    return SEGK_ERR_UNSUPPORTED;
}
```

### segmentalist_amd/csrc/segk_score_hint.hip

```cpp
#include "segk_kmeans_dev.h"

#define SEGK_K1_NW 4
#define SEGK_HINT_CHUNK 8

#ifndef SEGK_K1_ABL
#define SEGK_K1_ABL 0
#endif

struct K1Set {
    const float *tiles;
    int n_tiles;
    int tpr, n_ranges;
    float2 *part;
    int grid;
};

struct HintArgs {
    const unsigned char *ximg;
    const int32_t *ids;
    int64_t row0, n;
    K1Set full, delta;
    int K_max;
    int dbg;
    unsigned long long *stamp;
    float *fb_w;
    unsigned int *fb_t;
    int fb_cur;
    const int32_t *remap;
    int32_t *zero_cnt, *pre_hdr;
    int64_t k1_groups;
    const float *xrows32;
    int64_t ld32;
    const float *means32;
    const int32_t *cand_k;
    const float *nxx;
    float4 *hint_out;
    int32_t *ctl;
    const int32_t *meanchg;
    float *snap_img;
};

#define SEGK_MEANCHG_BIT 0x40000000

#define SEGK_RS_DRAIN_QUAD(O_, AO, q_, FIRST)                                                                               \
    do {                                                                                                                     \
        float x1_, u_;                                                                                                       \
        if (FIRST) {                                                                                                         \
            const float t1_ = __builtin_amdgcn_fmed3f(m1[O_], AO[4 * (q_)], AO[4 * (q_) + 1]);                              \
            asm volatile("v_max3_f32 %2, %0, %4, %5\n\t"                                                                     \
                         "v_med3_f32 %3, %2, %6, %7\n\t"                                                                     \
                         "v_max3_f32 %0, %2, %6, %7\n\t"                                                                     \
                         "v_max3_f32 %1, %1, %8, %3"                                                                          \
                         : "+v"(m1[O_]), "+v"(m2[O_]), "=&v"(x1_), "=&v"(u_)                                                 \
                         : "v"(AO[4 * (q_)]), "v"(AO[4 * (q_) + 1]), "v"(AO[4 * (q_) + 2]), "v"(AO[4 * (q_) + 3]), "v"(t1_)); \
        } else {                                                                                                             \
            float t1_;                                                                                                       \
            asm volatile("v_med3_f32 %4, %0, %5, %6\n\t"                                                                     \
                         "v_max3_f32 %2, %0, %5, %6\n\t"                                                                     \
                         "v_med3_f32 %3, %2, %7, %8\n\t"                                                                     \
                         "v_max3_f32 %0, %2, %7, %8\n\t"                                                                     \
                         "v_max3_f32 %1, %1, %4, %3"                                                                          \
                         : "+v"(m1[O_]), "+v"(m2[O_]), "=&v"(x1_), "=&v"(u_), "=&v"(t1_)                                     \
                         : "v"(AO[4 * (q_)]), "v"(AO[4 * (q_) + 1]), "v"(AO[4 * (q_) + 2]), "v"(AO[4 * (q_) + 3]));         \
        }                                                                                                                    \
    } while (0)

template <int KS, int V>
__device__ __forceinline__ void hint_wave_rows(const HintArgs &H, const int32_t *map , int64_t w, int64_t n_w, bool skip_ok)
{
    constexpr int D = 16 * KS - 4 * V;
    constexpr int nfull = D & ~7, nblk = nfull >> 3, rem = D & 7;
    constexpr int NX = nblk + (rem ? 1 : 0);
    typedef float f32x4_t __attribute__((ext_vector_type(4)));
    typedef float f32x2_t __attribute__((ext_vector_type(2)));
    typedef const __attribute__((address_space(1))) f32x4_t *gptr_t;
    const int lane = threadIdx.x & 63, row = lane >> 1, h = lane & 1;
    auto pk_sub = [](f32x2_t a, f32x2_t b2) -> f32x2_t {
        f32x2_t d;
        asm("v_pk_add_f32 %0, %1, %2 neg_lo:[0,1] neg_hi:[0,1]" : "=v"(d) : "v"(a), "v"(b2));
        return d;
    };
    const int64_t n_steps = (H.n + 31) >> 5;
    if (H.dbg & 8) return;
    auto rid_of = [&](int64_t s_) -> int32_t {
        const int64_t p_ = s_ * 32 + row;
        return p_ < H.n ? (H.ids ? H.ids[p_] : (int32_t)(H.row0 + p_)) : -1;
    };
    auto step_body = [&](int64_t s, int32_t rid_c, int32_t hint, bool skip, auto &&mid) {
        f32x4_t xv[NX], mv[NX];
#pragma unroll
        for (int b = 0; b < NX; b++) { xv[b] = f32x4_t{0.f, 0.f, 0.f, 0.f}; mv[b] = xv[b]; }
        if (!skip) {
            int64_t r_any = rid_c >= 0 ? (int64_t)rid_c : (H.ids ? 0 : H.row0);
            if (H.dbg & 16) r_any &= 1023;
            const uintptr_t xa = (uintptr_t)(H.xrows32 + r_any * H.ld32);
            const uintptr_t ma = (uintptr_t)(H.means32 + (int64_t)(hint >= 0 ? hint : 0) * D);
#pragma unroll
            for (int b = 0; b < nblk; b++) xv[b] = *reinterpret_cast<gptr_t>(xa + 16u * h + 32u * b);
            if constexpr (rem != 0) xv[nblk] = *reinterpret_cast<gptr_t>(xa + 4u * nfull);
#pragma unroll
            for (int b = 0; b < nblk; b++) mv[b] = *reinterpret_cast<gptr_t>(ma + 16u * h + 32u * b);
            if constexpr (rem != 0) mv[nblk] = *reinterpret_cast<gptr_t>(ma + 4u * nfull);
        }
        const float nx = rid_c >= 0 ? H.nxx[rid_c] : 0.f;
        if (H.dbg & 64) __builtin_amdgcn_s_sleep(64);
        mid();
        f32x2_t rl = {0.f, 0.f}, rh = {0.f, 0.f};
#pragma unroll
        for (int b = 0; b < ((H.dbg & 32) ? 1 : nblk); b++) {
            const f32x2_t dl = pk_sub(mv[b].xy, xv[b].xy), dh = pk_sub(mv[b].zw, xv[b].zw);
            const f32x2_t tl = dl * dl, th = dh * dh;
            rl = b == 0 ? tl : rl + tl;
            rh = b == 0 ? th : rh + th;
        }
        float res = (rl.x + rl.y) + (rh.x + rh.y);
        const float ro = __shfl_xor(res, 1);
        res = (h == 0) ? res + ro : ro + res;
        if constexpr (rem != 0) {
            const f32x2_t dl = pk_sub(mv[nblk].xy, xv[nblk].xy), dh = pk_sub(mv[nblk].zw, xv[nblk].zw);
            const f32x2_t tl = dl * dl, th = dh * dh;
            res += tl.x;
            if (rem > 1) res += tl.y;
            if (rem > 2) res += th.x;
            if (rem > 3) res += th.y;
        }
        const float sc = -res;
        const int64_t p = s * 32 + row;
        if (h == 0 && p < H.n && !skip) H.hint_out[p] = make_float4(sc, 0.5f * (sc - nx), __int_as_float(rid_c >= 0 ? hint : -1), 0.f);
    };
    int n_skipped = 0;
    if (skip_ok) {
        constexpr int CH = SEGK_HINT_CHUNK, PPL = CH / 2;
        const int crow = lane & 31, chalf = lane >> 5;
        auto chunk_load = [&](int64_t s0, int32_t (&rd)[PPL], int32_t (&kp)[PPL], int32_t (&pzv)[PPL]) {
#pragma unroll
            for (int u = 0; u < PPL; u++) {
                const int64_t s_ = s0 + (int64_t)(2 * u + chalf) * n_w, p_ = s_ * 32 + crow;
                const bool in = s_ < n_steps && p_ < H.n;
                rd[u] = in ? (H.ids ? H.ids[p_] : (int32_t)(H.row0 + p_)) : -1;
                pzv[u] = in ? __float_as_int(H.hint_out[p_].z) : -2;
            }
#pragma unroll
            for (int u = 0; u < PPL; u++) kp[u] = rd[u] >= 0 ? H.cand_k[rd[u]] : -1;
        };
        for (int64_t s0 = w; s0 < n_steps; s0 += (int64_t)CH * n_w) {
            int32_t rd[PPL], hv[PPL];
            unsigned long long live[PPL];
            {
                int32_t kp[PPL], pzv[PPL];
                chunk_load(s0, rd, kp, pzv);
#pragma unroll
                for (int u = 0; u < PPL; u++) {
                    const int64_t s_ = s0 + (int64_t)(2 * u + chalf) * n_w;
                    const bool in = s_ < n_steps && s_ * 32 + crow < H.n;
                    int32_t hint = (rd[u] >= 0 && kp[u] >= 0 && kp[u] < H.K_max) ? map[kp[u]] : -1;
                    const bool mchg = hint >= 0 && (hint & SEGK_MEANCHG_BIT) != 0;
                    if (hint >= 0) hint &= ~SEGK_MEANCHG_BIT;
                    const bool skip = rd[u] >= 0 && hint >= 0 && !mchg && pzv[u] == hint;
                    hv[u] = skip ? (hint | SEGK_MEANCHG_BIT) : hint;
                    live[u] = __ballot(in && !skip);
                    n_skipped += __popcll(__ballot(skip));
                }
            }
#pragma unroll 1
            for (int i = 0; i < CH; i++) {
                const int64_t s_ = s0 + (int64_t)i * n_w;
                if (s_ >= n_steps) break;
                int32_t rd_s = rd[0], hv_s = hv[0];
                unsigned long long lv = live[0];
#pragma unroll
                for (int u = 1; u < PPL; u++)
                    if ((i >> 1) == u) { rd_s = rd[u]; hv_s = hv[u]; lv = live[u]; }
                const int sh = 32 * (i & 1);
                if ((unsigned)(lv >> sh) == 0u) continue;
                const int src = sh + row;
                const int32_t rid_c = __shfl(rd_s, src);
                int32_t hint = __shfl(hv_s, src);
                const bool skip = hint >= 0 && (hint & SEGK_MEANCHG_BIT) != 0;
                if (hint >= 0) hint &= ~SEGK_MEANCHG_BIT;
                step_body(s_, rid_c, rid_c >= 0 ? hint : -1, skip, [] {});
            }
        }
        if (n_skipped > 0 && lane == 0) atomicAdd(H.ctl + 3, n_skipped);
        return;
    }
    int64_t s = w;
    int32_t rid = -1, rid_n = -1, kprev = -1;
    if (s < n_steps) {
        rid = rid_of(s);
        if (s + n_w < n_steps) rid_n = rid_of(s + n_w);
        kprev = rid >= 0 ? H.cand_k[rid] : -1;
    }
    for (; s < n_steps; s += n_w) {
        int32_t hint = (rid >= 0 && kprev >= 0 && kprev < H.K_max) ? map[kprev] : -1;
        if (hint >= 0) hint &= ~SEGK_MEANCHG_BIT;
        step_body(s, rid, hint, false, [&] {
            rid = rid_n;
            kprev = rid >= 0 ? H.cand_k[rid] : -1;
            const int64_t s2 = s + 2 * n_w;
            rid_n = s2 < n_steps ? rid_of(s2) : -1;
        });
    }
}

struct XcdShare { int64_t lo, hi; };
__device__ __forceinline__ XcdShare k1_xcd_share(const HintArgs &H, int64_t total_groups, bool delta, bool record)
{
    const int lane = threadIdx.x & 63, x = lane & 7;
    const int cur = H.fb_cur, prev = (cur + 2) % 3, next = (cur + 1) % 3;
    const float wp = H.fb_w[prev * 8 + x];
    const unsigned int tp = H.fb_t ? H.fb_t[prev * 8 + x] : 0u;
    const bool ok = __all(tp > 0u && wp > 0.f);
    const float rate = ok ? wp / (float)tp : 0.f;
    float rsum = rate;
    rsum += __shfl_xor(rsum, 1);
    rsum += __shfl_xor(rsum, 2);
    rsum += __shfl_xor(rsum, 4);
    float w = !(wp > 0.f) ? 0.125f : ok ? 0.5f * wp + 0.5f * (rate / rsum) : wp;
    w = fminf(fmaxf(w, 0.0625f), 0.25f);
    float wsum = w;
    wsum += __shfl_xor(wsum, 1);
    wsum += __shfl_xor(wsum, 2);
    wsum += __shfl_xor(wsum, 4);
    double cum = 0.0;
    for (int y = 0; y < 8; y++) {
        const float wy = __shfl(w, y);
        if (y < x) cum += (double)wy;
    }
    const int64_t split = (int64_t)(cum * ((double)total_groups / (double)wsum));
    const int xcd = blockIdx.x & 7;
    XcdShare s;
    s.lo = __shfl(split, xcd);
    s.hi = xcd == 7 ? total_groups : __shfl(split, (xcd + 1) & 7);
    if (record && lane < 8) {
        H.fb_w[cur * 8 + x] = delta ? (wp > 0.f ? wp : 0.125f) : w / wsum;
        if (H.fb_t) {
            H.fb_t[next * 8 + x] = 0u;
            if (delta) H.fb_t[cur * 8 + x] = tp;
        }
    }
    return s;
}

template <int KS, int V>
__global__ __launch_bounds__(128 * SEGK_K1_NW, 1) void k_kmeans_top2_rs(HintArgs H)
{
    typedef _Float16 T;
    typedef SegkPiece::V8 V8;
    constexpr int P = 2, KP = KS * 16, NBLK = 2;
    constexpr int STRIDE = (KS * P * 256 + 32 + 1023) / 1024 * 1024;
    constexpr int TL = KS * 256 + 32;
    extern __shared__ __attribute__((aligned(16))) float lds[];
    const int tid = threadIdx.x, lane = tid & 63, wave = tid >> 6;
    const int j = lane & 31, h = lane >> 5;
    const int mw = H.ctl ? __builtin_amdgcn_readfirstlane(H.ctl[0]) : 0;
    const bool delta = (mw & SEGK_DELTA_MODE) != 0, skip_ok = (mw & SEGK_DELTA_SKIP) != 0;
    const K1Set S = delta ? H.delta : H.full;
    const int n_tiles = delta ? __builtin_amdgcn_readfirstlane(H.ctl[2]) : S.n_tiles;
    const int tpr = S.tpr, R = S.n_ranges, grid = S.grid;
    const float *tiles = S.tiles;
    float2 *part = S.part;
    if ((int)blockIdx.x >= grid) return;
    const int map_off = tpr * TL;
    const bool is_hint = wave >= SEGK_K1_NW;
    if (!is_hint) __builtin_amdgcn_s_setprio(2);
#ifdef SEGK_STAMP
    const unsigned long long st_k0 = __builtin_amdgcn_s_memtime(), st_r0 = __builtin_amdgcn_s_memrealtime();
#endif
    int range, wgr, n_wgr;
    const bool xcd_aware = (grid & 7) == 0 && ((grid >> 3) % R) == 0;
    if (xcd_aware) {
        const int xcd = blockIdx.x & 7, idx = blockIdx.x >> 3;
        range = idx % R;
        wgr = (idx / R) * 8 + xcd;
        n_wgr = grid / R;
    } else {
        n_wgr = grid / R;
        range = blockIdx.x % R;
        wgr = blockIdx.x / R;
    }
    const int t_lo = range * tpr;
    int nt = n_tiles - t_lo;
    if (nt > tpr) nt = tpr;
    const bool mm_on = wgr < n_wgr && nt > 0;
    if (nt < 1) nt = 1;
    const T *plane0 = (const T *)(H.ximg + SEGK_SP_HEADER);
    const int64_t total_groups = (H.n + 32 * NBLK - 1) / (32 * NBLK);
    int64_t n_groups = H.k1_groups < total_groups ? H.k1_groups : total_groups, n_slots = (int64_t)n_wgr * SEGK_K1_NW, g_first = (int64_t)wgr * SEGK_K1_NW + wave;
    const unsigned long long fb_t0 = __builtin_amdgcn_s_memrealtime();
    if (blockIdx.x == 0 && tid == 0) {
        if (H.zero_cnt) *H.zero_cnt = 0;
#pragma unroll
        for (int i = 0; i < 16; i++) H.pre_hdr[i] = 0;
    }
    const XcdShare share = k1_xcd_share(H, total_groups, delta, blockIdx.x == 0 && wave == 0);
    const bool fb = xcd_aware && H.fb_t != nullptr && !delta;
    if (fb) {
        n_slots = (int64_t)(n_wgr >> 3) * SEGK_K1_NW;
        g_first = share.lo + (int64_t)(wgr >> 3) * SEGK_K1_NW + wave;
        n_groups = share.hi;
    }

#define SEGK_RS_LOAD(g_, XB)                                                                                    \
    do {                                                                                                         \
        _Pragma("unroll") for (int b = 0; b < NBLK; b++) {                                                       \
            const int64_t r = (g_) * (32 * NBLK) + 32 * b + j;                                                   \
            int64_t rowid = -1;                                                                                  \
            if (r < H.n) rowid = H.ids ? (int64_t)H.ids[r] : H.row0 + r;                                         \
            if (rowid < 0) rowid = 0;           \
            const T *xp = plane0 + rowid * KP + 8 * h;                                                           \
            _Pragma("unroll") for (int s = 0; s < KS; s++) XB[b][s] = *reinterpret_cast<const V8 *>(xp + 16 * s); \
        }                                                                                                        \
    } while (0)

#define SEGK_RS_UNIT(XB, N_, AN, O_, AO, REFILL)                                                                     \
    do {                                                                                                              \
        _Pragma("unroll") for (int s = 0; s < KS; s++) {                                                              \
            asm volatile("" : "+v"(a[s]));                                                                            \
            AN = __builtin_amdgcn_mfma_f32_32x32x16_f16(a[s], XB[N_][s], s == 0 ? cs : AN, 0, 0, 0);                  \
            asm volatile("" : "+v"(AN));                                                                              \
            if (REFILL && !(SEGK_K1_ABL & 2)) {    \
                load_a(tn, s);                                                                                        \
                if (s == 0) load_cs(tn);                                                                              \
            }                                                                                                         \
            __builtin_amdgcn_sched_barrier(0);                                                                        \
                      \
            constexpr int SL = KS > 1 ? KS - 1 : 1;                                                                   \
            const int q_lo = KS > 1 ? ((s - 1) * 4 + SL - 1) / SL : 0, q_hi = KS > 1 ? (s * 4 + SL - 1) / SL : 4;     \
            if ((KS == 1 || s >= 1) && !(SEGK_K1_ABL & 1)) {                                                          \
                if (0 >= q_lo && 0 < q_hi) SEGK_RS_DRAIN_QUAD(O_, AO, 0, true);                                       \
                if (1 >= q_lo && 1 < q_hi) SEGK_RS_DRAIN_QUAD(O_, AO, 1, false);                                      \
                if (2 >= q_lo && 2 < q_hi) SEGK_RS_DRAIN_QUAD(O_, AO, 2, false);                                      \
                if (3 >= q_lo && 3 < q_hi) SEGK_RS_DRAIN_QUAD(O_, AO, 3, false);                                      \
            }                                                                                                         \
            __builtin_amdgcn_sched_barrier(0);                                                                        \
        }                                                                                                             \
    } while (0)

#define SEGK_RS_TILE(XB, t_)                                        \
    do {                                                            \
        const int tn = (t_) + 1 < nt ? (t_) + 1 : 0;      \
        SEGK_RS_UNIT(XB, 0, acc0, 1, acc1, false);                  \
        SEGK_RS_UNIT(XB, 1, acc1, 0, acc0, true);                   \
    } while (0)

#define SEGK_RS_GROUP(g_, XB)                                                                                             \
    do {                                                                                                                   \
        float m1[NBLK], m2[NBLK];                                                                                          \
        _Pragma("unroll") for (int b = 0; b < NBLK; b++) { m1[b] = NEG_INF_F; m2[b] = NEG_INF_F; }                         \
        f32x16 acc0, acc1;                                                                                                 \
        _Pragma("unroll") for (int q = 0; q < 16; q++) acc1[q] = NEG_INF_F;         \
        int t = 0;                                                                                                         \
        for (; t + 1 < nt; t += 2) {                                                                                       \
            SEGK_RS_TILE(XB, t);                                                                                           \
            SEGK_RS_TILE(XB, t + 1);                                                                                       \
        }                                                                                                                  \
        if (t < nt) SEGK_RS_TILE(XB, t);                                                                                   \
        SEGK_RS_DRAIN_QUAD(NBLK - 1, acc1, 0, true);                                                                       \
        SEGK_RS_DRAIN_QUAD(NBLK - 1, acc1, 1, false);                                                                      \
        SEGK_RS_DRAIN_QUAD(NBLK - 1, acc1, 2, false);                                                                      \
        SEGK_RS_DRAIN_QUAD(NBLK - 1, acc1, 3, false);                                                                      \
           \
          \
          \
        _Pragma("unroll") for (int b = 0; b < NBLK; b++) {                                                                 \
            const float o1 = __shfl_xor(m1[b], 32), o2 = __shfl_xor(m2[b], 32);                                            \
            pend1[b] = fmaxf(m1[b], o1);                                                                                   \
            pend2[b] = fmaxf(fminf(m1[b], o1), fmaxf(m2[b], o2));                                                          \
        }                                                                                                                  \
        pend_g = (g_);                                                                                                     \
    } while (0)

#define SEGK_RS_STORE()                                                                                                    \
    do {                                                                                                                   \
        if (pend_g >= 0) {                                                                                                 \
            _Pragma("unroll") for (int b = 0; b < NBLK; b++) {                                                             \
                const int64_t r = pend_g * (32 * NBLK) + 32 * b + j;                                                       \
                if (h == 0 && r < H.n && !(H.dbg & 1)) part[(int64_t)range * H.n + r] = make_float2(pend1[b], pend2[b]); \
            }                                                                                                              \
        }                                                                                                                  \
    } while (0)

    V8 a[KS];
    f32x16 cs;
    auto load_a = [&](int t, int s) { a[s] = *reinterpret_cast<const V8 *>((const T *)(lds + t * TL) + (s * 64 + lane) * 8); };
    auto load_cs = [&](int t) {
        const float *cv = lds + t * TL + KS * 256 + 4 * h;
#pragma unroll
        for (int q = 0; q < 4; q++) {
            const float4 c4 = *reinterpret_cast<const float4 *>(cv + 8 * q);
            cs[4 * q + 0] = c4.x; cs[4 * q + 1] = c4.y; cs[4 * q + 2] = c4.z; cs[4 * q + 3] = c4.w;
        }
    };
    int64_t g = g_first;
    float pend1[NBLK], pend2[NBLK];
    int64_t pend_g = -1;
    V8 xa[NBLK][KS];
    typedef __attribute__((address_space(3))) void *lptr_t;
    if (!is_hint && mm_on && g < n_groups && !(H.dbg & 4)) SEGK_RS_LOAD(g, xa);
#ifdef SEGK_STAMP
    const unsigned long long st_k1 = __builtin_amdgcn_s_memtime();
#endif
    {
        constexpr int MAXT = (160 * 1024 / (TL * 4)) < SEGK_HINT_MAX_TPR ? (160 * 1024 / (TL * 4)) : SEGK_HINT_MAX_TPR;
        constexpr int MAXB = MAXT * KS;
        constexpr int NWF = 2 * SEGK_K1_NW;
        constexpr int PER_W = (MAXB + NWF - 1) / NWF;
        const int n_blk = nt * KS;
        const int rot = (int)(((unsigned)wgr * 2654435761u) >> 8) % n_blk;
        const unsigned lds0 = __builtin_amdgcn_readfirstlane((unsigned)(uintptr_t)(lptr_t)lds);
#pragma unroll
        for (int u = 0; u < PER_W; u++) {
            int c = wave + u * NWF;
            if (mm_on && c < n_blk) {
                c += rot;
                if (c >= n_blk) c -= n_blk;
                const int t = __builtin_amdgcn_readfirstlane(c / KS), ks = __builtin_amdgcn_readfirstlane(c) - t * KS;
                const float *src = tiles + (int64_t)(t_lo + t) * STRIDE + ks * (P * 256) + lane * 4;
                const unsigned dst = lds0 + (unsigned)(t * TL + ks * 256) * 4u;
                unsigned keep_;
                asm volatile("s_mov_b32 %0, m0\n\ts_mov_b32 m0, %2\n\ts_nop 0\n\t"
                             "global_load_lds_dwordx4 %1, off\n\ts_mov_b32 m0, %0"
                             : "=&s"(keep_)
                             : "v"(src), "s"(dst)
                             : "memory");
            }
        }
        float4 cv4 = make_float4(0.f, 0.f, 0.f, 0.f);
        const bool has_c = mm_on && tid < nt * 8;
        if (has_c) cv4 = *reinterpret_cast<const float4 *>(tiles + (int64_t)(t_lo + (tid >> 3)) * STRIDE + KS * P * 256 + (tid & 7) * 4);
        int32_t *map_l = reinterpret_cast<int32_t *>(lds + map_off);
        for (int k = tid; k < H.K_max; k += 128 * SEGK_K1_NW) {
            int v = H.remap ? H.remap[k] : k;
            if (v < 0 || v >= H.K_max) v = -1;
            else if (H.full.tiles[(int64_t)(v >> 5) * STRIDE + KS * P * 256 + (v & 31)] < -1.0e37f) v = -1;
            if (skip_ok && v >= 0 && H.meanchg[v]) v |= SEGK_MEANCHG_BIT;
            map_l[k] = v;
        }
        if (has_c) *reinterpret_cast<float4 *>(lds + (tid >> 3) * TL + KS * 256 + (tid & 7) * 4) = cv4;
        static_assert(128 * SEGK_K1_NW >= MAXT * 8, "one thread per float4 of the constants");
    }
    asm volatile("s_waitcnt vmcnt(0)" ::: "memory");
    __syncthreads();
    if (is_hint) {
        if (H.ctl && !delta && mm_on && wgr == 0) {
            float4 *dst = reinterpret_cast<float4 *>(H.snap_img + 4 + (int64_t)t_lo * TL);
            const float4 *src = reinterpret_cast<const float4 *>(lds);
            for (int i = tid - 64 * SEGK_K1_NW; i < nt * (TL / 4); i += 64 * SEGK_K1_NW) dst[i] = src[i];
        }
        hint_wave_rows<KS, V>(H, reinterpret_cast<const int32_t *>(lds + map_off), (int64_t)blockIdx.x * SEGK_K1_NW + (wave - SEGK_K1_NW),
                              (int64_t)grid * SEGK_K1_NW, skip_ok);
        return;
    }
#ifdef SEGK_STAMP
    const unsigned long long st_k2 = __builtin_amdgcn_s_memtime();
#endif
    if (!mm_on || g >= n_groups || (H.dbg & 128)) return;
    if (H.dbg & 4) SEGK_RS_LOAD(g, xa);
#pragma unroll
    for (int s = 0; s < KS; s++) load_a(0, s);
    load_cs(0);
    V8 xb[NBLK][KS];
#ifdef SEGK_STAMP
    unsigned long long st_wait = 0, st_loop = 0, st_groups = 0;
    const unsigned long long st_begin = __builtin_amdgcn_s_memtime();
#define SEGK_ST(var) const unsigned long long var = __builtin_amdgcn_s_memtime()
#else
#define SEGK_ST(var) do { } while (0)
#endif
    for (;;) {
        SEGK_ST(s0);
        __builtin_amdgcn_s_waitcnt(0x0F70);
        SEGK_ST(s1);
        const int64_t g1 = g + n_slots;
        if (g1 < n_groups) SEGK_RS_LOAD(g1, xb);
        SEGK_RS_STORE();
        SEGK_ST(s2);
        SEGK_RS_GROUP(g, xa);
        SEGK_ST(s3);
#ifdef SEGK_STAMP
        st_wait += s1 - s0; st_loop += s3 - s2; st_groups++;
#endif
        if (g1 >= n_groups) break;
        SEGK_ST(s4);
        __builtin_amdgcn_s_waitcnt(0x0F70);
        SEGK_ST(s5);
        g = g1 + n_slots;
        if (g < n_groups) SEGK_RS_LOAD(g, xa);
        SEGK_RS_STORE();
        SEGK_ST(s6);
        SEGK_RS_GROUP(g1, xb);
        SEGK_ST(s7);
#ifdef SEGK_STAMP
        st_wait += s5 - s4; st_loop += s7 - s6; st_groups++;
#endif
        if (g >= n_groups) break;
    }
#ifdef SEGK_STAMP
    if (H.stamp && lane == 0) {
        unsigned long long *o = H.stamp + ((int64_t)blockIdx.x * SEGK_K1_NW + wave) * 8;
        o[0] = st_wait; o[1] = st_loop; o[2] = __builtin_amdgcn_s_memtime() - st_begin; o[3] = st_groups;
        o[4] = st_begin - st_k0; o[5] = st_r0; o[6] = __builtin_amdgcn_s_memrealtime(); o[7] = ((st_k1 - st_k0) << 32) | (st_k2 - st_k1);
    }
#endif
#undef SEGK_ST
    SEGK_RS_STORE();
    if (fb && lane == 0) atomicMax(&H.fb_t[H.fb_cur * 8 + (blockIdx.x & 7)], (unsigned int)(__builtin_amdgcn_s_memrealtime() - fb_t0));
#undef SEGK_RS_STORE
#undef SEGK_RS_GROUP
#undef SEGK_RS_TILE
#undef SEGK_RS_UNIT
#undef SEGK_RS_LOAD
}
#undef SEGK_RS_DRAIN_QUAD

template <int KS>
__global__ __launch_bounds__(SEGK_PREP_THREADS) void k_delta_prep(DeltaPrepArgs P)
{
    if ((int)blockIdx.x >= P.n_tiles) {
        delta_prep_means_rows(P, (int)blockIdx.x - P.n_tiles, (int)gridDim.x - P.n_tiles);
        return;
    }
    __shared__ DeltaPrepLds S;
    const int e_cur = ((const int *)P.tiles_hdr)[0];
    if (delta_prep_tile(P, KS, (int)blockIdx.x, e_cur, S)) delta_prep_mode(P, KS, e_cur, S);
}

struct HintMergeArgs {
    const float2 *part;
    const float4 *hint_out;
    int n_ranges;
    const float *tiles_hdr;
    const unsigned char *ximg;
    const int32_t *ctl;
    const float2 *part_delta;
    int32_t *lab_base;
    const int32_t *colchg;
    const int32_t *meanchg;
    int32_t *lab_last;
    int32_t *stats_host;
};

#define SEGK_MERGE_ROWS 6144
#define SEGK_MERGE_THREADS 1024
__global__ __launch_bounds__(SEGK_MERGE_THREADS) void k_hint_merge(ScoreArgs A, HintMergeArgs H, int KP, int64_t per, float *pre_thr, int64_t first_skipped)
{
    __shared__ int32_t ulist[SEGK_MERGE_ROWS];
    __shared__ float uthr[SEGK_MERGE_ROWS];
    __shared__ int32_t ucnt, ubase;
    const int tid = threadIdx.x, lane = tid & 63;
    if (tid == 0) ucnt = 0;
    const int mw = H.ctl ? H.ctl[0] : 0;
    const bool delta = (mw & SEGK_DELTA_MODE) != 0;
    const int n_chg = H.ctl ? H.ctl[1] : 0, n_packed = H.ctl ? H.ctl[2] : 0;
    if (H.stats_host && blockIdx.x == 0 && tid == 0) {
        H.stats_host[1] = n_chg;
        H.stats_host[2] = n_packed;
        H.stats_host[3] = H.ctl ? H.ctl[3] : 0;
        __hip_atomic_store(H.stats_host, H.ctl ? 1 + (delta ? 1 : 0) : 0, __ATOMIC_RELEASE, __HIP_MEMORY_SCOPE_SYSTEM);
    }
    __syncthreads();
    bool carry = false;
    if (delta && (mw & SEGK_DELTA_SKIP) != 0 && H.lab_last) {
        const int c_off = (KP / 16) * 512;
        bool bad = false;
        for (int k = tid; k < A.K_max; k += SEGK_MERGE_THREADS)
            if (H.meanchg[k] && !H.colchg[k])
                bad |= !(H.tiles_hdr[1024 + (int64_t)(k >> 5) * A.tile_stride + c_off + (k & 31)] < -1.0e37f);
        carry = __syncthreads_or(bad ? 1 : 0) == 0;
    }
    const int64_t p_lo = (int64_t)blockIdx.x * per, p_hi = p_lo + per < A.n ? p_lo + per : A.n;
    const int e_ab = ((const int *)H.ximg)[1] + ((const int *)H.tiles_hdr)[0];
    const float unscale = ldexpf(1.f, -e_ab), scale = ldexpf(1.f, e_ab);
    const float M = (float)(sqrt(*A.mnorm2) * (1.0 + 1e-6)) + 1e-30f;
    const float Em = H.tiles_hdr[1];
    constexpr int U = 5;
    for (int64_t p0 = p_lo; p0 < p_hi; p0 += SEGK_MERGE_THREADS * U) {
        int32_t rid[U];
        float4 ho[U];
        float t1[U], t2[U], xnb[U], xer[U], d1[U];
        int32_t last[U];
        bool cw[U];
#pragma unroll
        for (int j = 0; j < U; j++) {
            const int64_t p = p0 + j * SEGK_MERGE_THREADS + tid;
            rid[j] = -1;
            if (p < p_hi) rid[j] = A.ids ? A.ids[p] : (int32_t)(A.row0 + p);
        }
#pragma unroll
        for (int j = 0; j < U; j++) {
            const int64_t p = p0 + j * SEGK_MERGE_THREADS + tid;
            ho[j] = make_float4(0.f, 0.f, __int_as_float(-1), 0.f);
            t1[j] = NEG_INF_F; t2[j] = NEG_INF_F; xnb[j] = 0.f; xer[j] = 0.f;
            if (rid[j] >= 0) {
                ho[j] = H.hint_out[p];
                for (int r = 0; r < H.n_ranges; r++) {
                    const float2 pv = H.part[(int64_t)r * A.n + p];
                    const float n1 = fmaxf(t1[j], pv.x);
                    t2[j] = fmaxf(fminf(t1[j], pv.x), fmaxf(t2[j], pv.y));
                    t1[j] = n1;
                }
                xnb[j] = A.xnorm[rid[j]];
                xer[j] = A.xerr[rid[j]];
            }
            d1[j] = NEG_INF_F;
            last[j] = -2;
            cw[j] = false;
            if (rid[j] >= 0 && carry) {
                const int32_t hint = __float_as_int(ho[j].z);
                last[j] = H.lab_last[p];
                cw[j] = hint >= 0 && last[j] == hint && H.meanchg[hint] == 0;
            }
            if (rid[j] >= 0 && delta) {
                const int32_t hint = __float_as_int(ho[j].z);
                if (hint >= 0 && H.colchg[hint] && H.lab_base[p] == hint) {
                    t1[j] = t2[j];
                }
                if (n_packed > 0) {
                    const float2 pv = H.part_delta[p];
                    d1[j] = pv.x;
                    const float n1 = fmaxf(t1[j], pv.x);
                    t2[j] = fmaxf(fminf(t1[j], pv.x), fmaxf(t2[j], pv.y));
                    t1[j] = n1;
                }
            }
        }
#pragma unroll
        for (int j = 0; j < U; j++) {
            bool und = false;
            float thr = 0.f;
            int32_t keep = -1;
            if (rid[j] >= 0 && p0 + j * SEGK_MERGE_THREADS + tid >= first_skipped) {
                const int q2 = atomicAdd(A.cand.count, 1);
                if (q2 < A.amb_cap) A.cand.queue[q2] = rid[j];
            } else if (rid[j] >= 0) {
                const int32_t hint = __float_as_int(ho[j].z);
                und = true;
                const float tau = filter_tau_h1(xnb[j], M, A.D, xer[j], Em);
                float lower = t1[j];
                thr = t1[j] - tau * scale * 1.000001f;
                thr -= 4e-7f * fabsf(t1[j]);
                bool ok = false;
                if (hint >= 0) {
                    const float top1 = t1[j] * unscale, top2 = t2[j] * unscale;
                    const float u = 5.9604645e-8f;
                    const float e1 = (1.02f * (float)(KP + 16) + 16.f) * u * (xnb[j] * M + 0.5f * M * M);
                    const float rnd = 1.00001f * fminf((xnb[j] + xer[j]) * Em + xer[j] * M, 1.01f * 9.765625e-4f * xnb[j] * M);
                    const float s2 = xnb[j] + M;
                    const float dl = ((float)(A.D / 8 + 13) + 4.f) * u * s2 * s2;
                    ok = (top1 - top2 > tau) && (ho[j].y >= top1 - tau + (e1 + rnd + dl) * 1.0001f);
                    const bool carried = !ok && cw[j] && ho[j].y > d1[j] * unscale + (e1 + rnd + dl) * 1.0001f;
                    if (ok || carried) {
                        A.cand.k[rid[j]] = hint;
                        A.cand.s[rid[j]] = (double)ho[j].x;
                        und = false;
                        keep = hint;
                    }
                    lower = (ho[j].y - (e1 + rnd + dl) * 1.0001f) * scale;
                    lower -= 4e-7f * fabsf(lower);
                }
                if (H.lab_base && !delta) H.lab_base[p0 + j * SEGK_MERGE_THREADS + tid] = ok ? hint : -1;
                if (und && delta && n_chg > 0) {
                    if (hint < 0) {
                        und = false;
                        const int q2 = atomicAdd(A.cand.count, 1);
                        if (q2 < A.amb_cap) A.cand.queue[q2] = rid[j];
                    } else {
                        lower = fmaxf(lower, d1[j]);
                        thr = lower - tau * scale * 1.000001f;
                        thr -= 4e-7f * fabsf(lower);
                    }
                }
            }
            if (H.lab_last && rid[j] >= 0 && last[j] != keep) H.lab_last[p0 + j * SEGK_MERGE_THREADS + tid] = keep;
            const unsigned long long mask = __ballot(und);
            if (mask != 0ull) {
                const int before = __builtin_amdgcn_mbcnt_hi((unsigned)(mask >> 32), __builtin_amdgcn_mbcnt_lo((unsigned)mask, 0));
                int base = 0;
                if (lane == 0) base = atomicAdd(&ucnt, __popcll(mask));
                base = __shfl(base, 0);
                if (und) {
                    ulist[base + before] = rid[j];
                    uthr[base + before] = thr;
                }
            }
        }
    }
    __syncthreads();
    const int cnt = ucnt;
    if (cnt == 0) return;
    if (tid == 0) ubase = atomicAdd(A.pre_count, cnt);
    __syncthreads();
    const int base = ubase;
    for (int i = tid; i < cnt; i += SEGK_MERGE_THREADS) {
        const int q = base + i;
        const int32_t rid = ulist[i];
        if (q < A.pre_cap) {
            A.pre_queue[q] = rid;
            if (pre_thr) pre_thr[q] = uthr[i];
        } else {
            const int q2 = atomicAdd(A.cand.count, 1);
            if (q2 < A.amb_cap) A.cand.queue[q2] = rid;
        }
    }
}

struct HintLaunch {
    HintPlan lds;
    bool band;
    int grid;
    int64_t k1_groups;
    float *fb_w;
    unsigned int *fb_t;
    int fb_cur;
    float4 *hint_out;
    bool part_fresh;
};

static int hint_workspaces(segk_ctx *ctx, ScoreArgs &A, HintLaunch &L, hipStream_t st)
{
    if (int rc = segk_ws_grow(ctx, &ctx->pre_queue, &ctx->pre_cap, A.n, sizeof(int32_t) * (size_t)(A.n + 16), st)) return rc;
    A.pre_queue = ctx->pre_queue + 16;
    A.pre_count = ctx->pre_queue;
    A.pre_cap = (int)A.n;
    if (L.band)
        if (int rc = segk_ws_grow(ctx, &ctx->pre_thr, &ctx->pre_thr_cap, A.n, sizeof(float) * (size_t)A.n, st)) return rc;
    const size_t part_bytes = ((size_t)L.lds.n_ranges * (size_t)A.n * sizeof(float2) + 255) & ~(size_t)255;
    const size_t need_part = part_bytes + (size_t)A.n * sizeof(float4);
    L.part_fresh = ctx->hint_part_bytes < need_part;
    if (int rc = segk_ws_grow(ctx, &ctx->hint_part, &ctx->hint_part_bytes, need_part, need_part, st)) return rc;
    L.hint_out = (float4 *)((unsigned char *)ctx->hint_part + part_bytes);
    if (!ctx->hint_fb) {
        float init[3 * 8 + 3 * 8];
        SEGK_CHECK_HIP(hipMalloc(&ctx->hint_fb, sizeof(init)));
        for (int i = 0; i < 24; i++) init[i] = 0.125f;
        memset(init + 24, 0, 24 * sizeof(unsigned int));
        SEGK_CHECK_HIP(hipMemcpyAsync(ctx->hint_fb, init, sizeof(init), hipMemcpyHostToDevice, st));
        SEGK_CHECK_HIP(hipStreamSynchronize(st));
        ctx->hint_fb_launch = 0;
    }
    return SEGK_OK;
}

static void hint_plan_rows(segk_ctx *ctx, const ScoreArgs &A, HintLaunch &L)
{
    const int n_ranges = L.lds.n_ranges;
    const int64_t total_groups = (A.n + 63) / 64;
    L.fb_w = (float *)ctx->hint_fb;
    const bool fb_big = total_groups >= 192 * 64;
    L.fb_t = (segk_env_int("SEGK_HINT_BALANCE", 1) == 0 || !fb_big) ? nullptr : (unsigned int *)(L.fb_w + 24);
    L.fb_cur = (int)(ctx->hint_fb_launch++ % 3u);
    L.grid = (ctx->n_cu / n_ranges) * n_ranges;
    const int64_t steps = (A.n + 64 * SEGK_K1_NW - 1) / (64 * SEGK_K1_NW);
    if ((int64_t)L.grid / n_ranges > steps) L.grid = (int)steps * n_ranges;
    L.k1_groups = total_groups;
    if (!L.fb_t && !L.band) {
        const int64_t slots = (int64_t)(L.grid / n_ranges) * SEGK_K1_NW;
        const int64_t whole = slots > 0 ? (total_groups / slots) * slots : 0;
        if (whole > 0 && total_groups - whole <= 32) L.k1_groups = whole;
    }
}

struct DeltaBuf {
    int32_t *ctl;
    int32_t *colchg, *meanchg;
    float *snap_img;
    float *packed;
    float *snap_means;
    float2 *part;
    int32_t *lab_base;
    int32_t *lab_last;
    size_t zero_bytes;
};
static size_t delta_layout(unsigned char *b, int n_tiles, int K_max, int D, int64_t n, int stride, DeltaBuf *B)
{
    const size_t TL = (size_t)(segk_b3_kp(D) / 16) * 256 + 32;
    size_t off = 0;
    auto take = [&](size_t bytes) {
        unsigned char *p = b ? b + off : nullptr;
        off += (bytes + 255) & ~(size_t)255;
        return p;
    };
    B->ctl = (int32_t *)take(256);
    B->colchg = (int32_t *)take((size_t)n_tiles * 32 * 4);
    B->meanchg = (int32_t *)take((size_t)K_max * 4);
    B->snap_img = (float *)take(((size_t)n_tiles * TL + 4) * 4);
    B->packed = (float *)take((size_t)n_tiles * stride * 4);
    B->zero_bytes = off;
    B->snap_means = (float *)take((size_t)K_max * D * 4);
    B->part = (float2 *)take((size_t)n * 8);
    B->lab_base = (int32_t *)take((size_t)n * 4);
    B->lab_last = (int32_t *)take((size_t)n * 4);
    return off;
}

static int delta_cap(const HintPlan &lds)
{
    int cap = segk_env_int("SEGK_DELTA_CAP", lds.tpr);
    if (cap > lds.max_tiles) cap = lds.max_tiles;
    return cap < 1 ? 1 : cap;
}
static int delta_budget(int n_tiles) { return segk_env_int("SEGK_DELTA_BUDGET", n_tiles); }

static DeltaPrepArgs delta_prep_args(segk_ctx *ctx, const DeltaBuf &B, const float *tiles, int n_tiles, int stride, int K_max, int D,
                                     const float *means32, const int32_t *remap, const int32_t *K_dev, bool valid, int cap, int budget,
                                     int redo_seq = -1)
{
    DeltaPrepArgs P{};
    P.tiles_hdr = tiles; P.n_tiles = n_tiles; P.stride = stride;
    P.K_max = K_max; P.D = D; P.means32 = means32; P.remap = remap; P.K_dev = K_dev;
    P.valid = valid ? 1 : 0; P.hint_valid = valid ? 1 : 0; P.cap = cap;
    P.budget = budget;
    P.redo = redo_seq >= 0 ? 1 : 0;
    P.seq = redo_seq >= 0 ? redo_seq : (int)(ctx->delta_seq++ & 1u);
    P.ctl = B.ctl; P.colchg = B.colchg; P.meanchg = B.meanchg;
    P.snap_img = B.snap_img; P.packed = B.packed; P.snap_means = B.snap_means;
    return P;
}

bool segk_delta_prep_fold(segk_ctx *ctx, const segk_corpus *c, const segk_kmeans *m, const int32_t *remap, hipStream_t st, DeltaPrepArgs *P)
{
    *P = DeltaPrepArgs{};
    if (!ctx || ctx->delta_pending != 0 || !ctx->delta_valid || ctx->capturing || !ctx->delta_buf) return false;
    if (segk_env_int("SEGK_DELTA_PREP_FOLD", 1) == 0 || segk_env_int("SEGK_SCORE_DELTA", 1) == 0) return false;
    const void *key[4] = {c->Xb3, c->X32, m->tiles_b3, m->means};
    const int64_t key_n[5] = {0, c->n_emb, c->n_emb, m->K_max, c->D};
    if (memcmp(key, ctx->delta_key, sizeof(key)) != 0 || memcmp(key_n, ctx->delta_key_n, sizeof(key_n)) != 0) return false;
    const int n_tiles = segk_n_tiles(m->K_max), stride_sp = segk_sp_tile_stride(c->D, 2);
    HintPlan lds;
    if (n_tiles > 32 * SEGK_PREP_COLS || !segk_hint_plan(m->K_max, segk_b3_kp(c->D) / 16, n_tiles, &lds)) return false;
    DeltaBuf B{};
    if (ctx->delta_bytes != delta_layout(nullptr, n_tiles, m->K_max, c->D, c->n_emb, stride_sp, &B)) return false;
    delta_layout((unsigned char *)ctx->delta_buf, n_tiles, m->K_max, c->D, c->n_emb, stride_sp, &B);
    const int cap = delta_cap(lds), budget = delta_budget(n_tiles);
    *P = delta_prep_args(ctx, B, m->tiles_b3, n_tiles, stride_sp, m->K_max, c->D, (const float *)m->means, remap, m->K, true, cap, budget);
    ctx->delta_pending = 1;
    ctx->delta_pending_remap = remap; ctx->delta_pending_K = m->K; ctx->delta_pending_stream = (const void *)st;
    ctx->delta_pending_cap = cap; ctx->delta_pending_budget = budget; ctx->delta_pending_seq = P->seq;
    return true;
}

template <int KS>
static int launch_delta_prep(segk_ctx *ctx, const ScoreArgs &A, const int32_t *remap, const int32_t *K_dev, int64_t n_emb,
                             const HintLaunch &L, hipStream_t st, DeltaBuf *B, int *cap)
{
    *B = DeltaBuf{};
    *cap = 0;
    const int pending = ctx->delta_pending;
    ctx->delta_pending = 0;
    const bool delta_on = segk_env_int("SEGK_SCORE_DELTA", 1) != 0 && L.band && A.ids == nullptr && A.n_tiles <= 32 * SEGK_PREP_COLS;
    const void *key[6] = {A.X32, A.xrows32, A.tiles, A.means32, A.cand.k, A.cand.s};
    const int64_t key_n[5] = {A.row0, A.n, n_emb, A.K_max, A.D};
    bool state_valid = delta_on && !L.part_fresh && ctx->delta_valid && memcmp(key, ctx->delta_key, sizeof(key)) == 0 &&
                       memcmp(key_n, ctx->delta_key_n, sizeof(key_n)) == 0;
    ctx->delta_valid = 0;
    if (!delta_on) return SEGK_OK;
    const int stride_sp = segk_sp_tile_stride(A.D, 2);
    const size_t need = delta_layout(nullptr, A.n_tiles, A.K_max, A.D, A.n, stride_sp, B);
    if (ctx->delta_bytes != need) {
        ctx->delta_bytes = 0;
        if (int rc = segk_ws_realloc(ctx, &ctx->delta_buf, need, st)) return rc;
        ctx->delta_bytes = need;
        state_valid = false;
        SEGK_CHECK_HIP(hipMemsetAsync(ctx->delta_buf, 0, B->zero_bytes, st));
    }
    delta_layout((unsigned char *)ctx->delta_buf, A.n_tiles, A.K_max, A.D, A.n, stride_sp, B);
    *cap = delta_cap(L.lds);
    const int budget = delta_budget(A.n_tiles);
    const bool folded = pending == 1 && state_valid && remap == ctx->delta_pending_remap && K_dev == ctx->delta_pending_K &&
                        (const void *)st == ctx->delta_pending_stream && *cap == ctx->delta_pending_cap &&
                        budget == ctx->delta_pending_budget;
    if (!folded) {
        const DeltaPrepArgs P = delta_prep_args(ctx, *B, A.tiles, A.n_tiles, stride_sp, A.K_max, A.D, A.means32, remap, K_dev, state_valid,
                                                *cap, budget, pending != 0 && state_valid ? ctx->delta_pending_seq : -1);
        hipLaunchKernelGGL(k_delta_prep<KS>, dim3(A.n_tiles + segk_delta_prep_row_blocks(A.K_max)), dim3(SEGK_PREP_THREADS), 0, st, P);
    }
    memcpy(ctx->delta_key, key, sizeof(key));
    memcpy(ctx->delta_key_n, key_n, sizeof(key_n));
    ctx->delta_valid = 1;
    return SEGK_OK;
}

template <int KS>
static int launch_k1(segk_ctx *ctx, const ScoreArgs &A, const int32_t *remap, int64_t n_emb, const HintLaunch &L, const DeltaBuf &B,
                     int delta_cap, hipStream_t st)
{
    constexpr int TL = KS * 256 + 32;
    HintArgs H{};
    H.ximg = (const unsigned char *)A.X32;
    H.ids = A.ids; H.row0 = A.row0; H.n = A.n;
    H.K_max = A.K_max;
    H.dbg = segk_dev_env("SEGK_HINT_DBG");
#ifdef SEGK_STAMP
    H.stamp = getenv("SEGK_STAMP_PTR") ? (unsigned long long *)strtoull(getenv("SEGK_STAMP_PTR"), nullptr, 0) : nullptr;
#endif
    H.fb_w = L.fb_w; H.fb_t = L.fb_t; H.fb_cur = L.fb_cur;
    H.remap = remap;
    H.zero_cnt = ctx->defer_zero;
    ctx->defer_zero = nullptr;
    H.pre_hdr = ctx->pre_queue;
    H.k1_groups = L.k1_groups;
    H.xrows32 = A.xrows32; H.ld32 = A.ld32; H.means32 = A.means32;
    H.cand_k = A.cand.k;
    H.nxx = A.xerr + n_emb;
    H.hint_out = L.hint_out;
    H.ctl = B.ctl; H.meanchg = B.meanchg; H.snap_img = B.snap_img;
    H.full = K1Set{A.tiles + 1024, A.n_tiles, L.lds.tpr, L.lds.n_ranges, (float2 *)ctx->hint_part, L.grid};
    size_t lds = (size_t)L.lds.tpr * TL * sizeof(float) + L.lds.map_bytes;
    int grid = L.grid;
    if (B.ctl) {
        const int64_t steps = (A.n + 64 * SEGK_K1_NW - 1) / (64 * SEGK_K1_NW);
        H.delta = K1Set{B.packed, 0, delta_cap, 1, B.part, (int64_t)ctx->n_cu > steps ? (int)steps : ctx->n_cu};
        const size_t lds_d = (size_t)delta_cap * TL * sizeof(float) + L.lds.map_bytes;
        if (H.delta.grid > grid) grid = H.delta.grid;
        if (lds_d > lds) lds = lds_d;
    }
    const bool prof = segk_prof_now(ctx);
    const int slot = ctx->prof_n % SEGK_PROF_SLOTS;
#define SEGK_K1_LAUNCH(VV)                                                                                                  \
    do {                                                                                                                     \
        SEGK_CHECK_HIP(segk_dyn_lds((const void *)k_kmeans_top2_rs<KS, VV>, lds));                                           \
        if (prof) SEGK_CHECK_HIP(hipEventRecord(ctx->prof_ev[slot][0], st));                                                 \
        hipLaunchKernelGGL((k_kmeans_top2_rs<KS, VV>), dim3((unsigned)grid), dim3(128 * SEGK_K1_NW), lds, st, H);            \
    } while (0)
    switch ((16 * KS - A.D) / 4) {
        case 0: SEGK_K1_LAUNCH(0); break;
        case 1: SEGK_K1_LAUNCH(1); break;
        case 2: SEGK_K1_LAUNCH(2); break;
        default: SEGK_K1_LAUNCH(3); break;
    }
#undef SEGK_K1_LAUNCH
    if (prof) {
        SEGK_CHECK_HIP(hipEventRecord(ctx->prof_ev[slot][1], st));
        ctx->prof_rows[slot] = A.n;
        ctx->prof_kind = 5;
        ctx->prof_launches = 1;
        ctx->prof_n++;
    }
    return SEGK_OK;
}

static void launch_merge(segk_ctx *ctx, const ScoreArgs &A, const HintLaunch &L, const DeltaBuf &B, int ks, hipStream_t st)
{
    HintMergeArgs E{};
    E.part = (const float2 *)ctx->hint_part;
    E.hint_out = L.hint_out;
    E.n_ranges = L.lds.n_ranges;
    E.tiles_hdr = A.tiles;
    E.ximg = (const unsigned char *)A.X32;
    E.ctl = B.ctl;
    E.part_delta = B.part;
    E.lab_base = B.lab_base;
    E.colchg = B.colchg;
    E.meanchg = B.meanchg;
    E.lab_last = B.lab_last;
    E.stats_host = ctx->delta_host_dev;
    int64_t grid = (int64_t)ctx->n_cu;
    if (grid * SEGK_MERGE_THREADS > A.n) grid = (A.n + SEGK_MERGE_THREADS - 1) / SEGK_MERGE_THREADS;
    if (grid * SEGK_MERGE_ROWS < A.n) grid = (A.n + SEGK_MERGE_ROWS - 1) / SEGK_MERGE_ROWS;
    const int64_t per = (A.n + grid - 1) / grid;
    hipLaunchKernelGGL(k_hint_merge, dim3((unsigned)grid), dim3(SEGK_MERGE_THREADS), 0, st, A, E, ks * 16, per,
                       L.band ? ctx->pre_thr : nullptr, L.k1_groups * 64);
}

template <int KS>
static int launch_score_hint(segk_ctx *ctx, ScoreArgs A, const int32_t *remap, const int32_t *K_dev, int64_t n_emb, hipStream_t st)
{
    HintLaunch L{};
    L.band = segk_band_applies(A);
    SEGK_REQUIRE(segk_hint_plan(A.K_max, KS, A.n_tiles, &L.lds),
                 "hinted score path: K_max too large for K1's LDS (the label map beside four ranges of tile images at most)");
    if (int rc = hint_workspaces(ctx, A, L, st)) return rc;
    hint_plan_rows(ctx, A, L);
    DeltaBuf B;
    int delta_cap;
    if (int rc = launch_delta_prep<KS>(ctx, A, remap, K_dev, n_emb, L, st, &B, &delta_cap)) return rc;
    if (int rc = launch_k1<KS>(ctx, A, remap, n_emb, L, B, delta_cap, st)) return rc;
    launch_merge(ctx, A, L, B, KS, st);
    if (L.band) return segk_launch_band(ctx, A, ctx->pre_thr, A.n, B.lab_last, KS, st);
    ScoreArgs B2 = A;
    B2.ids = A.pre_queue;
    B2.row0 = 0;
    B2.n = A.n;
    B2.n_dev = ctx->pre_queue;
    if (int rc = segk_launch_sp_second(ctx, B2, KS, st)) return rc;
    SEGK_LAUNCH_CHECK();
    return SEGK_OK;
}

int segk_dispatch_score_hint(segk_ctx *ctx, const ScoreArgs &A, const int32_t *remap, const int32_t *K_dev, int64_t n_emb, int ks, hipStream_t st)
{
    switch (ks) {
        case 1: return launch_score_hint<1>(ctx, A, remap, K_dev, n_emb, st);
        case 2: return launch_score_hint<2>(ctx, A, remap, K_dev, n_emb, st);
        case 3: return launch_score_hint<3>(ctx, A, remap, K_dev, n_emb, st);
        case 4: return launch_score_hint<4>(ctx, A, remap, K_dev, n_emb, st);
        case 5: return launch_score_hint<5>(ctx, A, remap, K_dev, n_emb, st);
        case 6: return launch_score_hint<6>(ctx, A, remap, K_dev, n_emb, st);
        case 7: return launch_score_hint<7>(ctx, A, remap, K_dev, n_emb, st);
        case 8: return launch_score_hint<8>(ctx, A, remap, K_dev, n_emb, st);
        default: break;
    }
    segk_set_error("hinted score path: D out of range");
    return SEGK_ERR_UNSUPPORTED;
}
```

### segmentalist_amd/device.py

```python
import ctypes as C

import numpy as np

from . import _abi
from ._abi import SEGK_F32, SEGK_F64, SegkError, check, ptr
from .comm import SingleComm, get_comm


def _torch():
    import torch
    return torch


def _dev():
    torch = _torch()
    if not torch.cuda.is_available():
        raise SegkError("segmentalist_amd needs an MI355X: no ROCm device is visible and there is no "
                        "CPU fallback for the hot path")
    return torch.device("cuda", torch.cuda.current_device())


def to_dev(a, dtype=None):
    torch = _torch()
    a = np.ascontiguousarray(a if dtype is None else np.asarray(a, dtype=dtype))
# ... 99 lines not shown
        return torch.float32 if self.x_dtype == SEGK_F32 else torch.float64


class DeviceKMeans(object):

    def __init__(self, corpus, K_max, assignments, random_means, shard=None):
        torch = _torch()
        dev = _dev()
        self.corpus = corpus
        c = corpus
        self.K_max = int(K_max)
        self.row_base, self.n_rows_global, self.shard = 0, c.n_emb, None
        assignments = np.asarray(assignments)
        init = None
        if shard is not None:
            lo, hi, X_host = shard
            assert hi - lo == c.n_emb and len(assignments) == X_host.shape[0]
            self.row_base, self.n_rows_global, self.shard = lo, len(assignments), (lo, hi)
            init = _host_init_stats(X_host, assignments, self.K_max, np.asarray(random_means, dtype=c.x_np_dtype))
            assignments = assignments[lo:hi]
        xd = c.torch_xdtype
        self.means = torch.empty((self.K_max, c.D), dtype=xd, device=dev)
        self.mean_numerators = torch.zeros((self.K_max, c.D), dtype=torch.float64, device=dev)
        self.counts = torch.zeros(self.K_max, dtype=torch.int64, device=dev)
        self.random_means = to_dev(np.asarray(random_means, dtype=c.x_np_dtype))
        self.assignments = to_dev(assignments, np.int32)
        self.K = torch.zeros(1, dtype=torch.int32, device=dev)
        n_tiles_f = _abi.lib().segk_kmeans_tiles_floats(self.K_max, c.D)
        self.tiles = torch.zeros(int(n_tiles_f), dtype=torch.float32, device=dev)
        self.mnorm_max = torch.zeros(1, dtype=torch.float64, device=dev)
        self.tiles_b3 = None
        if c.ensure_b3():
            self.tiles_b3 = torch.zeros(int(_abi.lib().segk_kmeans_tiles_b3_floats(self.K_max, c.D)), dtype=torch.float32,
                                        device=dev)
        self.m = _abi.KMeansDev(
            tiles_b3=self.tiles_b3.data_ptr() if self.tiles_b3 is not None else None,
            means=self.means.data_ptr(), mean_numerators=self.mean_numerators.data_ptr(),
            counts=self.counts.data_ptr(), random_means=self.random_means.data_ptr(),
            assignments=self.assignments.data_ptr(), K=self.K.data_ptr(), K_max=self.K_max,
            tiles=self.tiles.data_ptr(), mnorm_max=self.mnorm_max.data_ptr())
        self.cand_k = torch.zeros(c.n_emb, dtype=torch.int32, device=dev)
        self.cand_f = torch.zeros((c.n_emb, 2), dtype=torch.float32, device=dev)
        self.cand_s = torch.zeros(c.n_emb, dtype=torch.float64, device=dev)
        self.cand_queue = torch.zeros(c.n_emb, dtype=torch.int32, device=dev)
        self.cand_count = torch.zeros(1, dtype=torch.int32, device=dev)
        self.cand = _abi.CandDev(k=self.cand_k.data_ptr(), f=self.cand_f.data_ptr(), s=self.cand_s.data_ptr(),
                                 queue=self.cand_queue.data_ptr(), count=self.cand_count.data_ptr())
        self.status = torch.zeros(8, dtype=torch.int32, device=dev)
        self.assign_stale = None
        self.batch_comm = SingleComm()
        self.bounds_stale = None
        self._L = _abi.lib()
        self._ctx = _abi.ctx()
        if init is None:
            check(self._L.segk_kmeans_init_stats(self._ctx, C.byref(c.c), C.byref(self.m), _abi.stream()))
        else:
            means, numer, counts, K = init
            self.means.copy_(torch.from_numpy(means))
            self.mean_numerators.copy_(torch.from_numpy(numer))
            self.counts.copy_(torch.from_numpy(counts))
            self.K.fill_(int(K))
            self.prepare()
        if c.n_utt:
            self._alloc_utt_buffers()

    def _alloc_utt_buffers(self):
        torch = _torch()
        dev = _dev()
        c = self.corpus
        nu, nm = c.n_utt, c.N_max
        self.old_tok = torch.zeros((nu, nm), dtype=torch.int32, device=dev)
        self.new_tok = torch.zeros((nu, nm), dtype=torch.int32, device=dev)
        self.new_k = torch.zeros((nu, nm), dtype=torch.int32, device=dev)
        self.n_old = torch.zeros(nu, dtype=torch.int32, device=dev)
        self.n_new = torch.zeros(nu, dtype=torch.int32, device=dev)
        self.n_flag = torch.zeros(nu, dtype=torch.int32, device=dev)
        self.out_total = torch.zeros(nu, dtype=torch.float64, device=dev)
        self.utt_arange = torch.arange(nu, dtype=torch.int32, device=dev)
        self.remap = torch.zeros(self.K_max, dtype=torch.int32, device=dev)
        self.out_scalars = torch.zeros(8, dtype=torch.float64, device=dev)

    def _cp(self):
        return C.byref(self.corpus.c)

    def require_whole_corpus(self, what):
        if self.shard is not None:
            raise SegkError("%s needs every row of the embedding matrix on this device, but the segmenter holds a shard (rows "
                            "%d..%d of %d): construct it with shard_corpus=False" % (what, self.shard[0], self.shard[1],
                                                                                     self.n_rows_global))

    def global_assignments(self):
        self.ensure_assignments()
        a = self.assignments.cpu().numpy()
        if self.shard is None:
            return a
        out = np.full(self.n_rows_global, -1, dtype=a.dtype)
        for lo, hi, part in self.batch_comm.all_gather_object((self.shard[0], self.shard[1], a)):
            out[lo:hi] = part
        return out

    def set_global_assignments(self, a):
        torch = _torch()
        a = np.asarray(a)
        if self.shard is not None:
            a = a[self.shard[0]:self.shard[1]]
        self.assignments.copy_(torch.from_numpy(np.ascontiguousarray(a)).to(self.assignments.dtype))

    def ensure_assignments(self, group=None):
        if self.assign_stale is None:
            return
        lo, hi, world = self.assign_stale
        check(self._L.segk_kmeans_assignments_from_tokens(self._ctx, self._cp(), C.byref(self.m), lo, hi,
                                                          ptr(self.new_tok), ptr(self.new_k), ptr(self.n_new),
                                                          _abi.stream()))
        if world > 1 and self.shard is None:
            (self.batch_comm if group is None else get_comm(group)).all_reduce_max(self.assignments)
        self.assign_stale = None

    def ensure_boundaries(self):
        if self.bounds_stale is None:
            return
        bounds, pt = self.bounds_stale
        torch = _torch()
        mine = torch.zeros_like(bounds)
        mine[pt.utt_lo:pt.utt_hi] = bounds[pt.utt_lo:pt.utt_hi]
        self.batch_comm.all_reduce_max(mine)
        bounds.copy_(mine)
        self.bounds_stale = None

    def ensure_state(self):
        self.ensure_assignments()
        self.ensure_boundaries()

    def prepare(self):
        check(self._L.segk_kmeans_prepare(self._ctx, self._cp(), C.byref(self.m), _abi.stream()))

    def score_rows(self, ids=None, row0=0, n=None, hint_remap=None):
        if ids is not None:
            n = ids.numel()
            p = ptr(ids)
        else:
            p = None
            n = self.corpus.n_emb - row0 if n is None else n
        if hint_remap is not None:
            check(self._L.segk_kmeans_score_hinted(self._ctx, self._cp(), C.byref(self.m), p, int(row0), int(n),
                                                   C.byref(self.cand), ptr(hint_remap), ptr(self.status), _abi.stream()))
            return
        check(self._L.segk_kmeans_score(self._ctx, self._cp(), C.byref(self.m), p, int(row0), int(n),
                                        C.byref(self.cand), ptr(self.status), _abi.stream()))

    def delta_stats(self):
        out = (C.c_int32 * 4)()
        check(self._L.segk_kmeans_delta_stats(self._ctx, out))
        return tuple(int(v) for v in out)

    def score_ptr(self, ids_ptr, n):
        check(self._L.segk_kmeans_score(self._ctx, self._cp(), C.byref(self.m), C.c_void_p(ids_ptr), 0, int(n),
                                        C.byref(self.cand), ptr(self.status), _abi.stream()))

    def exact_max(self, ids):
        torch = _torch()
        ids_t = to_dev(self._local_rows(ids), np.int32)
        n = ids_t.numel()
        out_max = torch.empty(n, dtype=torch.float64, device=ids_t.device)
        out_arg = torch.empty(n, dtype=torch.int32, device=ids_t.device)
        self.score_rows(ids_t)
        check(self._L.segk_kmeans_exact_max(self._ctx, self._cp(), C.byref(self.m), ptr(ids_t), n,
                                            C.byref(self.cand), ptr(out_max), ptr(out_arg), _abi.stream()))
        return out_max.cpu().numpy(), out_arg.cpu().numpy(), int(self.cand_count.item())

    def _local_rows(self, ids):
        if self.shard is None:
            return ids
        a = np.asarray(ids, dtype=np.int64)
        if a.size and (a.min() < self.shard[0] or a.max() >= self.shard[1]):
            self.require_whole_corpus("scoring rows outside this rank's shard")
        return a - self.shard[0]

    def neg_sqrd_norm(self, row):
        torch = _torch()
        row = int(self._local_rows([row])[0])
        out = torch.empty(self.K_max, dtype=self.corpus.torch_xdtype, device=self.means.device)
        check(self._L.segk_kmeans_neg_sqrd_norm(self._ctx, self._cp(), C.byref(self.m), int(row), ptr(out),
                                                _abi.stream()))
        return out.cpu().numpy()

    def add_item(self, i, k):
        self.require_whole_corpus("add_item")
        self.ensure_assignments()
        check(self._L.segk_kmeans_add_item(self._ctx, self._cp(), C.byref(self.m), int(i), int(k),
                                           ptr(self.status), _abi.stream()))

    def del_item(self, i):
        self.require_whole_corpus("del_item")
        self.ensure_assignments()
        check(self._L.segk_kmeans_del_item(self._ctx, self._cp(), C.byref(self.m), int(i), ptr(self.status),
                                           _abi.stream()))

    def del_component(self, k):
        self.require_whole_corpus("del_component")
        self.ensure_assignments()
        check(self._L.segk_kmeans_del_component(self._ctx, self._cp(), C.byref(self.m), int(k),
                                                ptr(self.status), _abi.stream()))

    def clean_components(self):
        self.require_whole_corpus("clean_components")
        self.ensure_assignments()
        check(self._L.segk_kmeans_clean_components(self._ctx, self._cp(), C.byref(self.m), ptr(self.status),
                                                   _abi.stream()))

    def sum_neg_sqrd_norm(self):
        self.ensure_assignments()
        torch = _torch()
        out = torch.zeros(1, dtype=torch.float64, device=self.means.device)
        check(self._L.segk_kmeans_sum_neg_sqrd_norm(self._ctx, self._cp(), C.byref(self.m), ptr(out),
                                                    _abi.stream()))
        if self.shard is not None:
            return float(sum(self.batch_comm.all_gather_object(float(out.item()))))
        return float(out.item())

    def segment(self, boundaries, n_slices_min, n_slices_max, wip, utt=None, utt0=0, n_utts=None):
        c = self.corpus
        if utt is not None:
            up = C.c_void_p(self.utt_arange.data_ptr() + 4 * int(utt))
            utt0, n = 0, 1
        else:
            up = None
            n = c.n_utt - utt0 if n_utts is None else n_utts
        check(self._L.segk_kmeans_segment(
            self._ctx, self._cp(), C.byref(self.m), up, int(utt0), int(n), int(n_slices_min), int(n_slices_max),
            float(wip), C.byref(self.cand), ptr(boundaries), ptr(self.old_tok),
            ptr(self.new_tok), ptr(self.new_k), ptr(self.n_old), ptr(self.n_new), ptr(self.n_flag),
            ptr(self.out_total), ptr(self.status), _abi.stream()))

    def segment_utt_sequential(self, boundaries, i, n_slices_min, n_slices_max, wip):
        c = self.corpus
        self.require_whole_corpus("the sequential chain (segment_i)")
        self.ensure_state()
        N = int(c.lengths_np[i])
        tri_i = N * (N + 1) // 2
        self.score_ptr(c.vec_ids.data_ptr() + 4 * i * c.tri, tri_i)
        self.segment(boundaries, n_slices_min, n_slices_max, wip, utt=i)
        check(self._L.segk_kmeans_update_utt(self._ctx, self._cp(), C.byref(self.m), int(i), ptr(self.old_tok),
                                             ptr(self.new_tok), ptr(self.new_k), ptr(self.n_old),
                                             ptr(self.n_new), ptr(self.status), _abi.stream()))

    def sequential_sweep(self, boundaries, order, n_slices_min, n_slices_max, wip):
        if self.corpus.x_dtype != SEGK_F32 or self.corpus.N_max > 63:
            return False
        torch = _torch()
        self.require_whole_corpus("the sequential chain (segment)")
        self.ensure_state()
        if getattr(self, "_seq_keys", None) is None:
            self._seq_keys = torch.zeros(self.corpus.tri + 2, dtype=torch.int64, device=self.means.device)
        arr = np.ascontiguousarray(order, dtype=np.int32)
        check(self._L.segk_kmeans_sequential_sweep(
            self._ctx, self._cp(), C.byref(self.m), arr.ctypes.data, len(order), int(n_slices_min), int(n_slices_max), float(wip),
            C.byref(self.cand), ptr(self._seq_keys), ptr(boundaries), ptr(self.old_tok), ptr(self.new_tok), ptr(self.new_k),
            ptr(self.n_old), ptr(self.n_new), ptr(self.n_flag), ptr(self.out_total), ptr(self.status), _abi.stream()))
        return True

    def batch_record(self, lo, hi):
        check(self._L.segk_kmeans_batch_record(self._ctx, self._cp(), C.byref(self.m), int(lo), int(hi), ptr(self.new_tok),
                                               ptr(self.new_k), ptr(self.status), ptr(self.out_scalars), _abi.stream()))
        o = self.out_scalars.cpu().numpy()
        self._raise_status(int(o[5]))
        return float(o[0]), int(o[1]), int(o[2]), float(o[4])

    def _raise_status(self, bits):
        if bits & 1:
            raise AssertionError("a new segment has no embedding (vec_id == -1): the reference asserts in "
                                 "KMeansComponents.add_item (kmeans_components.py:100)")
        if bits & 2:
            raise AssertionError("add_item on an item that is already assigned (kmeans_components.py:101)")
        if bits & 4:
            raise SegkError("batch sweep: in one statistics block more new tokens chose an inactive component than "
                            "`flag_cap`; the tokens beyond were dropped, so the statistics of this sweep are not usable: "
                            "rebuild the segmenter (or load a checkpoint) with a larger flag_cap")

    def check_status(self):
        st = self.status.cpu().numpy()
        self._raise_status(int(st[0]))
        return int(st[1])


class Partition(object):

    def __init__(self, n_utt, utt_row_start, n_blocks=8, rank=0, world=1):
        if n_blocks % world != 0:
            raise SegkError("the number of statistics blocks (%d) must be a multiple of the number of "
                            "ranks (%d)" % (n_blocks, world))
        self.n_blocks, self.rank, self.world = n_blocks, rank, world
        self.nbl = n_blocks // world
        self.bounds = np.array([(b * n_utt) // n_blocks for b in range(n_blocks + 1)], dtype=np.int32)
        self.utt_lo = int(self.bounds[rank * self.nbl])
        self.utt_hi = int(self.bounds[(rank + 1) * self.nbl])
        self.row_lo = int(utt_row_start[self.utt_lo])
        self.row_hi = int(utt_row_start[self.utt_hi])
        self.local_bounds = self.bounds[rank * self.nbl:(rank + 1) * self.nbl + 1].copy()
        self._row_start = utt_row_start

    def minibatch(self, n_batches):
        steps = []
        for j in range(n_batches):
            utts, rows = [], []
            for b in range(self.rank * self.nbl, (self.rank + 1) * self.nbl):
# ... 824 lines not shown
```

Before: 7231 sweeps/s.

## Skip rescoring rows whose hinted mean stays closer by a triangle-inequality bound

Adds a geometric pruning stage. When only a few means change (up to 16), delta prep computes a rounded-down distance from each changed mean to every other mean and stores it in a sequence-tagged table. The hint kernel and merge then skip product work for rows whose carried hint satisfies the closed-form bound G^2 > c^2*S, and accept the hint directly. This cuts per-sweep distance computation in the incremental path. The cost is extra prep work, more LDS use, more control state, and careful rounding margins to keep results exact.

```diff
diff --git a/include/segk.h b/include/segk.h
--- a/include/segk.h
+++ b/include/segk.h
@@ -112,6 +112,9 @@
 int32_t segk_kmeans_hint_feedback(segk_ctx *ctx, uint32_t *launched, uint32_t *seen, int32_t *permille);
 
 int32_t segk_kmeans_delta_stats(segk_ctx *ctx, int32_t *out);
+
+int32_t segk_kmeans_geo_stats(segk_ctx *ctx, int32_t *out);
+int32_t segk_kmeans_geo_closed(double G, float s, int32_t D);
 
 int32_t segk_kmeans_exact_max(segk_ctx *ctx, const segk_corpus *c, const segk_kmeans *m,
                               const int32_t *ids, int64_t n, const segk_cand *cand,
diff --git a/segmentalist_amd/_abi.py b/segmentalist_amd/_abi.py
--- a/segmentalist_amd/_abi.py
+++ b/segmentalist_amd/_abi.py
@@ -83,6 +83,8 @@
     "segk_kmeans_stage_counts": (_i32, [_P, _DP, C.POINTER(_i32), _P]),
     "segk_kmeans_hint_feedback": (_i32, [_P, C.POINTER(C.c_uint32), C.POINTER(C.c_uint32), C.POINTER(_i32)]),
     "segk_kmeans_delta_stats": (_i32, [_P, C.POINTER(_i32)]),
+    "segk_kmeans_geo_stats": (_i32, [_P, C.POINTER(_i32)]),
+    "segk_kmeans_geo_closed": (_i32, [_f64, C.c_float, _i32]),
     "segk_kmeans_exact_max": (_i32, [_P, _CP, _KP, _P, _i64, _DP, _P, _P, _P]),
     "segk_kmeans_neg_sqrd_norm": (_i32, [_P, _CP, _KP, _i64, _P, _P]),
     "segk_kmeans_segment": (_i32, [_P, _CP, _KP, _P, _i32, _i32, _i32, _i32, _f64, _DP, _P, _P, _P, _P, _P, _P,
diff --git a/segmentalist_amd/csrc/segk_host.cpp b/segmentalist_amd/csrc/segk_host.cpp
--- a/segmentalist_amd/csrc/segk_host.cpp
+++ b/segmentalist_amd/csrc/segk_host.cpp
@@ -279,6 +279,17 @@
     return SEGK_OK;
 }
 
+int32_t segk_kmeans_geo_stats(segk_ctx *ctx, int32_t *out)
+{
+    SEGK_REQUIRE(ctx && out, "arguments");
+    out[0] = -1; out[1] = 0; out[2] = 0; out[3] = 0;
+    if (ctx->delta_host)
+        for (int i = 0; i < 4; i++) out[i] = ctx->delta_host[4 + i];
+    return SEGK_OK;
+}
+
+int32_t segk_kmeans_geo_closed(double G, float s, int32_t D) { return geo_closed(G, s, D) ? 1 : 0; }
+
 double segk_logsumexp(const double *a, int64_t n)
 {
     double mx = a[0], s = 0.0;
diff --git a/segmentalist_amd/csrc/segk_internal.h b/segmentalist_amd/csrc/segk_internal.h
--- a/segmentalist_amd/csrc/segk_internal.h
+++ b/segmentalist_amd/csrc/segk_internal.h
@@ -83,7 +83,9 @@
     int64_t delta_key_n[5];
     int delta_pending;
     const void *delta_pending_remap, *delta_pending_K, *delta_pending_stream;
-    int delta_pending_cap, delta_pending_budget, delta_pending_seq;
+    int delta_pending_cap, delta_pending_budget, delta_pending_seq, delta_pending_geo;
+    unsigned int geo_seq;
+    int geo_retired;
     volatile int32_t *delta_host;
     int32_t *delta_host_dev;
     void *hint_fb;
@@ -206,6 +208,23 @@
     return ((segk_b3_kp(D) / 16) * P * 256 + 32 + 1023) / 1024 * 1024;
 }
 
+#define SEGK_GEO_CAP 16
+static inline __host__ __device__ double segk_geo_kappa(int D) { return (double)(D + 4) * 0x1p-22; }
+static inline __host__ __device__ bool geo_closed(double G, float s, int D)
+{
+    const double S = -(double)s;
+    if (D < 1 || D > 128) return false;
+    if (!(G > 0.0 && G <= 0x1p100)) return false;
+    if (!(S >= 0x1p-100 && S <= 0x1p100)) return false;
+    const double c = 2.0 + segk_geo_kappa(D);
+    return G * G > c * c * S;
+}
+static inline __host__ __device__ float segk_geo_round_down(float q, int D)
+{
+    if (!(q >= 0x1p-100f && q <= 0x1p100f)) return 0.f;
+    return sqrtf(q) * (1.f - (float)(D + 8) * 0x1p-24f);
+}
+
 int segk_launch_score_lse(segk_ctx *ctx, const float *Y, int64_t ldy, int D2, const int32_t *ids, int64_t row0, int64_t n,
                           const float *tiles, int n_tiles, double norm, double *out, void *stream);
 
diff --git a/segmentalist_amd/csrc/segk_kmeans_dev.h b/segmentalist_amd/csrc/segk_kmeans_dev.h
--- a/segmentalist_amd/csrc/segk_kmeans_dev.h
+++ b/segmentalist_amd/csrc/segk_kmeans_dev.h
@@ -701,6 +701,7 @@
 
 #define SEGK_DELTA_MODE 1
 #define SEGK_DELTA_SKIP 2
+#define SEGK_DELTA_GEO 4
 #define SEGK_PREP_THREADS 256
 #define SEGK_PREP_COLS 4
 struct DeltaPrepArgs {
@@ -720,13 +721,55 @@
     float *snap_img;
     float *packed;
     float *snap_means;
+    int geo;
+    unsigned int gseq;
+    unsigned long long *gtab;
 };
 struct DeltaPrepLds { int chg[32], slot[32], nonid, last, n_chg, n_nonid, old[5]; };
 
+static __device__ __forceinline__ void delta_prep_geo_row(const DeltaPrepArgs &P, int k)
+{
+    const float *mk = P.means32 + (int64_t)k * P.D;
+    const bool vec = (P.D & 3) == 0 && ((uintptr_t)P.means32 & 15) == 0;
+    for (int h = threadIdx.x; h < P.K_max; h += SEGK_PREP_THREADS) {
+        if (h == k) continue;
+        const float *mh = P.means32 + (int64_t)h * P.D;
+        float q = 0.f;
+        if (vec) {
+#pragma unroll 13
+            for (int d = 0; d < P.D; d += 4) {
+                const float4 a = *reinterpret_cast<const float4 *>(mk + d), b = *reinterpret_cast<const float4 *>(mh + d);
+                const float t0 = a.x - b.x, t1 = a.y - b.y, t2 = a.z - b.z, t3 = a.w - b.w;
+                q = fmaf(t3, t3, fmaf(t2, t2, fmaf(t1, t1, fmaf(t0, t0, q))));
+            }
+        } else {
+            for (int d = 0; d < P.D; d++) {
+                const float t = mk[d] - mh[d];
+                q = fmaf(t, t, q);
+            }
+        }
+        const float g = segk_geo_round_down(q, P.D);
+        atomicMax(P.gtab + h, ((unsigned long long)P.gseq << 32) | (unsigned long long)(0xFFFFFFFFu - __float_as_uint(g)));
+    }
+}
+static __device__ __forceinline__ bool segk_geo_on(const int32_t *ctl, int mw, unsigned int *gseq, int *n_means)
+{
+    *gseq = (unsigned int)ctl[19];
+    *n_means = ctl[20 + (int)(*gseq & 1u)];
+    return (mw & SEGK_DELTA_GEO) != 0 && *n_means >= 1 && *n_means <= SEGK_GEO_CAP;
+}
+static __device__ __forceinline__ float segk_geo_g(unsigned long long e, unsigned int gseq)
+{
+    return (unsigned int)(e >> 32) == gseq ? __uint_as_float(0xFFFFFFFFu - (unsigned int)e) : __builtin_inff();
+}
+
 static __device__ __forceinline__ void delta_prep_means_rows(const DeltaPrepArgs &P, int wg, int n_wg)
 {
     const int lane = threadIdx.x & 63, wave = threadIdx.x >> 6;
     constexpr int NWV = SEGK_PREP_THREADS / 64;
+    __shared__ int geo_rows[SEGK_GEO_CAP], geo_n;
+    if (threadIdx.x == 0) geo_n = 0;
+    __syncthreads();
     for (int k = wg * NWV + wave; k < P.K_max; k += n_wg * NWV) {
         const int *cur = (const int *)(P.means32 + (int64_t)k * P.D);
         int *snap = (int *)(P.snap_means + (int64_t)k * P.D);
@@ -737,12 +780,17 @@
             snap[d] = c;
         }
         const bool any = __any(chg);
+        const bool before = P.redo && P.meanchg[k] != 0;
+        const bool flag = any || before || !P.hint_valid;
         if (lane == 0) {
-            const bool before = P.redo && P.meanchg[k] != 0;
-            P.meanchg[k] = (any || before || !P.hint_valid) ? 1 : 0;
+            P.meanchg[k] = flag ? 1 : 0;
             if (any) atomicAdd(P.ctl + 5 + (P.seq & 1), 1);
-        }
-    }
+            if (P.geo && flag && atomicAdd(P.ctl + 20 + (int)(P.gseq & 1u), 1) < SEGK_GEO_CAP) geo_rows[atomicAdd(&geo_n, 1)] = k;
+        }
+    }
+    __syncthreads();
+    if (P.geo)
+        for (int i = 0; i < geo_n; i++) delta_prep_geo_row(P, geo_rows[i]);
 }
 
 static __device__ __forceinline__ bool delta_prep_tile(const DeltaPrepArgs &P, const int KS, const int t, const int e_cur, DeltaPrepLds &S)
@@ -826,7 +874,11 @@
         P.ctl[5 + ((P.seq + 1) & 1)] = 0;
         P.ctl[7] = delta ? n_chg : 0;
         P.ctl[8] = P.K_dev ? *P.K_dev : P.K_max;
-        P.ctl[0] = (delta ? SEGK_DELTA_MODE : 0) | ((P.hint_valid && !nonid) ? SEGK_DELTA_SKIP : 0);
+        const bool skip = P.hint_valid && !nonid;
+        P.ctl[0] = (delta ? SEGK_DELTA_MODE : 0) | (skip ? SEGK_DELTA_SKIP : 0) | ((P.geo && delta && skip) ? SEGK_DELTA_GEO : 0);
+        P.ctl[19] = (int)P.gseq;
+        P.ctl[20 + (int)((P.gseq + 1u) & 1u)] = 0;
+        P.ctl[22] = 0; P.ctl[23] = 0; P.ctl[24] = 0;
         P.ctl[1] = n_chg;
         P.ctl[2] = delta ? n_packed : 0;
         P.ctl[3] = 0;
@@ -846,7 +898,8 @@
     if (ctx && ctx->delta_pending == 1) ctx->delta_pending = 2;
 }
 bool segk_band_applies(const ScoreArgs &A);
-int segk_launch_band(segk_ctx *ctx, const ScoreArgs &A, const float *thr, int64_t call_rows, int32_t *lab_last, int ks, hipStream_t st);
+int segk_launch_band(segk_ctx *ctx, const ScoreArgs &A, const float *thr, int64_t call_rows, int32_t *lab_last, const int32_t *geo_ctl, int ks,
+                     hipStream_t st);
 int segk_launch_seq_score(const segk_corpus *c, const segk_kmeans *m, int utt, const segk_cand *cand, unsigned long long *keys,
                           hipStream_t st);
 int segk_launch_update_utt(const segk_corpus *c, segk_kmeans *m, int utt, const int32_t *old_tok, const int32_t *new_tok,
diff --git a/segmentalist_amd/csrc/segk_score_band.hip b/segmentalist_amd/csrc/segk_score_band.hip
--- a/segmentalist_amd/csrc/segk_score_band.hip
+++ b/segmentalist_amd/csrc/segk_score_band.hip
@@ -15,6 +15,8 @@
     unsigned long long *fb;
     unsigned int fb_seq;
     int64_t fb_rows;
+    const int32_t *geo_ctl;
+    int32_t *geo_host;
 };
 
 #define SEGK_BAND_QUAD(MK, AO, q_, THR, FIRST)                                                                       \
@@ -52,6 +54,15 @@
     if (B.fb && blockIdx.x == 0 && tid == 0) {
         const unsigned long long pm = B.fb_rows > 0 ? (unsigned long long)((int64_t)count * 1000 / B.fb_rows) : 0ull;
         __hip_atomic_store(B.fb, ((unsigned long long)B.fb_seq << 32) | pm, __ATOMIC_RELEASE, __HIP_MEMORY_SCOPE_SYSTEM);
+    }
+    if (B.geo_host && blockIdx.x == 0 && tid == 0) {
+        unsigned int gseq = 0;
+        int n_means = 0;
+        const bool on = B.geo_ctl && segk_geo_on(B.geo_ctl, B.geo_ctl[0], &gseq, &n_means) && B.geo_ctl[25] != 0;
+        B.geo_host[1] = on ? B.geo_ctl[22] : 0;
+        B.geo_host[2] = on ? B.geo_ctl[23] : 0;
+        B.geo_host[3] = on ? B.geo_ctl[24] : 0;
+        __hip_atomic_store(B.geo_host, on ? n_means : -1, __ATOMIC_RELEASE, __HIP_MEMORY_SCOPE_SYSTEM);
     }
     int range, wgr, n_wgr;
     if ((gridDim.x & 7) == 0 && ((gridDim.x >> 3) % R) == 0) {
@@ -351,7 +362,8 @@
 }
 
 template <int KS>
-static int launch_band(segk_ctx *ctx, const ScoreArgs &A, const float *thr, int64_t call_rows, int32_t *lab_last, hipStream_t st)
+static int launch_band(segk_ctx *ctx, const ScoreArgs &A, const float *thr, int64_t call_rows, int32_t *lab_last, const int32_t *geo_ctl,
+                       hipStream_t st)
 {
     const int n_cu = ctx->n_cu;
     const int n_ranges = (A.n_tiles + SEGK_BAND_TPR - 1) / SEGK_BAND_TPR;
@@ -372,6 +384,8 @@
     B.fb = ctx->miss_dev;
     B.fb_seq = ++ctx->miss_seq;
     B.fb_rows = call_rows;
+    B.geo_ctl = geo_ctl;
+    B.geo_host = ctx->delta_host_dev ? ctx->delta_host_dev + 4 : nullptr;
     constexpr int TL = KS * 256 + 32;
     const size_t lds = (size_t)SEGK_BAND_TPR * TL * sizeof(float);
     int grid = (2 * n_cu / n_ranges) * n_ranges;
@@ -416,17 +430,18 @@
     return n_ranges >= 1 && n_ranges <= SEGK_BAND_MAX_RANGES && A.D % 4 == 0 && A.D >= 8 && A.D <= 128;
 }
 
-int segk_launch_band(segk_ctx *ctx, const ScoreArgs &A, const float *thr, int64_t call_rows, int32_t *lab_last, int ks, hipStream_t st)
+int segk_launch_band(segk_ctx *ctx, const ScoreArgs &A, const float *thr, int64_t call_rows, int32_t *lab_last, const int32_t *geo_ctl, int ks,
+                     hipStream_t st)
 {
     switch (ks) {
-        case 1: return launch_band<1>(ctx, A, thr, call_rows, lab_last, st);
-        case 2: return launch_band<2>(ctx, A, thr, call_rows, lab_last, st);
-        case 3: return launch_band<3>(ctx, A, thr, call_rows, lab_last, st);
-        case 4: return launch_band<4>(ctx, A, thr, call_rows, lab_last, st);
-        case 5: return launch_band<5>(ctx, A, thr, call_rows, lab_last, st);
-        case 6: return launch_band<6>(ctx, A, thr, call_rows, lab_last, st);
-        case 7: return launch_band<7>(ctx, A, thr, call_rows, lab_last, st);
-        case 8: return launch_band<8>(ctx, A, thr, call_rows, lab_last, st);
+        case 1: return launch_band<1>(ctx, A, thr, call_rows, lab_last, geo_ctl, st);
+        case 2: return launch_band<2>(ctx, A, thr, call_rows, lab_last, geo_ctl, st);
+        case 3: return launch_band<3>(ctx, A, thr, call_rows, lab_last, geo_ctl, st);
+        case 4: return launch_band<4>(ctx, A, thr, call_rows, lab_last, geo_ctl, st);
+        case 5: return launch_band<5>(ctx, A, thr, call_rows, lab_last, geo_ctl, st);
+        case 6: return launch_band<6>(ctx, A, thr, call_rows, lab_last, geo_ctl, st);
+        case 7: return launch_band<7>(ctx, A, thr, call_rows, lab_last, geo_ctl, st);
+        case 8: return launch_band<8>(ctx, A, thr, call_rows, lab_last, geo_ctl, st);
         default: break;
     }
     segk_set_error("band stage: D out of range");
diff --git a/segmentalist_amd/csrc/segk_score_hint.hip b/segmentalist_amd/csrc/segk_score_hint.hip
--- a/segmentalist_amd/csrc/segk_score_hint.hip
+++ b/segmentalist_amd/csrc/segk_score_hint.hip
@@ -38,7 +38,13 @@
     int32_t *ctl;
     const int32_t *meanchg;
     float *snap_img;
+    int geo_k1;
+    int geo_all;
+    const unsigned long long *gtab;
+    const int32_t *lab_last;
+    const int32_t *colchg;
 };
+#define SEGK_GEO_NO_PRODUCT __builtin_inff()
 
 #define SEGK_MEANCHG_BIT 0x40000000
 
@@ -255,6 +261,8 @@
     const int j = lane & 31, h = lane >> 5;
     const int mw = H.ctl ? __builtin_amdgcn_readfirstlane(H.ctl[0]) : 0;
     const bool delta = (mw & SEGK_DELTA_MODE) != 0, skip_ok = (mw & SEGK_DELTA_SKIP) != 0;
+    constexpr bool GEO_K1 = KS <= 7;
+    const bool geo_pre = GEO_K1 && H.geo_k1 != 0 && (mw & SEGK_DELTA_GEO) != 0;
     const K1Set S = delta ? H.delta : H.full;
     const int n_tiles = delta ? __builtin_amdgcn_readfirstlane(H.ctl[2]) : S.n_tiles;
     const int tpr = S.tpr, R = S.n_ranges, grid = S.grid;
@@ -310,6 +318,21 @@
             if (rowid < 0) rowid = 0;           \
             const T *xp = plane0 + rowid * KP + 8 * h;                                                           \
             _Pragma("unroll") for (int s = 0; s < KS; s++) XB[b][s] = *reinterpret_cast<const V8 *>(xp + 16 * s); \
+        }                                                                                                        \
+    } while (0)
+
+#define SEGK_RS_LOAD_M(g_, XB, M_)                                                                              \
+    do {                                                                                                         \
+        _Pragma("unroll") for (int b = 0; b < NBLK; b++) {                                                       \
+            const int64_t r = (g_) * (32 * NBLK) + 32 * b + j;                                                   \
+            int64_t rowid = -1;                                                                                  \
+            if (r < H.n) rowid = H.ids ? (int64_t)H.ids[r] : H.row0 + r;                                         \
+            if (rowid < 0) rowid = 0;                                                                            \
+            const T *xp = plane0 + rowid * KP + 8 * h;                                                           \
+            _Pragma("unroll") for (int s = 0; s < KS; s++) XB[b][s] = V8{};                                      \
+            if (((M_) >> (32 * b + j)) & 1ull) {                                                                 \
+                _Pragma("unroll") for (int s = 0; s < KS; s++) XB[b][s] = *reinterpret_cast<const V8 *>(xp + 16 * s); \
+            }                                                                                                    \
         }                                                                                                        \
     } while (0)
 
@@ -397,7 +420,7 @@
     int64_t pend_g = -1;
     V8 xa[NBLK][KS];
     typedef __attribute__((address_space(3))) void *lptr_t;
-    if (!is_hint && mm_on && g < n_groups && !(H.dbg & 4)) SEGK_RS_LOAD(g, xa);
+    if (!is_hint && mm_on && g < n_groups && !(H.dbg & 4) && !geo_pre) SEGK_RS_LOAD(g, xa);
 #ifdef SEGK_STAMP
     const unsigned long long st_k1 = __builtin_amdgcn_s_memtime();
 #endif
@@ -437,6 +460,11 @@
             if (skip_ok && v >= 0 && H.meanchg[v]) v |= SEGK_MEANCHG_BIT;
             map_l[k] = v;
         }
+        if (geo_pre) {
+            float *g_l = lds + map_off + ((H.K_max + 3) & ~3);
+            const unsigned int gseq = (unsigned int)H.ctl[19];
+            for (int k = tid; k < H.K_max; k += 128 * SEGK_K1_NW) g_l[k] = segk_geo_g(H.gtab[k], gseq);
+        }
         if (has_c) *reinterpret_cast<float4 *>(lds + (tid >> 3) * TL + KS * 256 + (tid & 7) * 4) = cv4;
         static_assert(128 * SEGK_K1_NW >= MAXT * 8, "one thread per float4 of the constants");
     }
@@ -461,6 +489,92 @@
     for (int s = 0; s < KS; s++) load_a(0, s);
     load_cs(0);
     V8 xb[NBLK][KS];
+    if constexpr (GEO_K1) if (geo_pre) {
+        unsigned int gseq_;
+        int n_means_;
+        bool geo_bad = false;
+        for (int k = lane; k < H.K_max; k += 64)
+            if (H.meanchg[k] && !H.colchg[k])
+                geo_bad |= !(H.full.tiles[(int64_t)(k >> 5) * STRIDE + KS * P * 256 + (k & 31)] < -1.0e37f);
+        if (__any(geo_bad) || !segk_geo_on(H.ctl, mw, &gseq_, &n_means_)) {
+            SEGK_RS_LOAD(g, xa);
+        } else {
+            const int32_t *map_g = reinterpret_cast<const int32_t *>(lds + map_off);
+            const float *g_l = lds + map_off + ((H.K_max + 3) & ~3);
+            constexpr int D = 16 * KS - 4 * V;
+            const float c_ = 2.f + (float)((D + 4) * 0x1p-22), c2 = c_ * c_ * 1.00002f;
+            int32_t hz = -2, hk = -1, hl = -3;
+            float hs = 0.f;
+            auto geo_issue = [&](int64_t g_) {
+                const int64_t r = g_ * (32 * NBLK) + lane;
+                hz = -2; hk = -1; hl = -3; hs = 0.f;
+                if (g_ < n_groups && r < H.n) {
+                    hs = H.hint_out[r].x;
+                    hz = __float_as_int(H.hint_out[r].z);
+                    hk = H.cand_k[H.row0 + r];
+                    hl = H.lab_last[r];
+                }
+            };
+            auto geo_open = [&](int64_t g_) -> unsigned long long {
+                const bool valid = g_ * (32 * NBLK) + lane < H.n;
+                const bool k_ok = hk >= 0 && hk < H.K_max;
+                const int32_t hint = map_g[k_ok ? hk : 0];
+                const bool cand = valid && k_ok && hint >= 0 && (hint & SEGK_MEANCHG_BIT) == 0 && hint == hz && hl == hint;
+                const float gv = g_l[cand ? hint : 0], S = -hs;
+                const bool closed = H.geo_all != 0 || (cand && S >= 1e-30f && S <= 1e30f && gv <= 1e30f && gv * gv > c2 * S);
+                return __ballot(valid && !closed);
+            };
+            int n_rows_out = 0, n_groups_out = 0;
+#define SEGK_RS_GROUP_M(g_, XB, M_)                                                                                    \
+            do {                                                                                                       \
+                if ((M_) != 0ull) {                                                                                    \
+                    SEGK_RS_GROUP(g_, XB);                                                                             \
+                } else {                                                                                               \
+                    pend_g = (g_);                                                                                     \
+                    n_groups_out++;                                                                                    \
+                }                                                                                                      \
+                _Pragma("unroll") for (int b = 0; b < NBLK; b++)                                                       \
+                    if (!(((M_) >> (32 * b + j)) & 1ull)) { pend1[b] = SEGK_GEO_NO_PRODUCT; pend2[b] = SEGK_GEO_NO_PRODUCT; } \
+                const int64_t left_ = H.n - (g_) * (32 * NBLK);                                                        \
+                n_rows_out += (int)(left_ < 32 * NBLK ? left_ : 32 * NBLK) - __popcll(M_);                             \
+            } while (0)
+            unsigned long long m_a, m_b = 0ull;
+            geo_issue(g);
+            __builtin_amdgcn_s_waitcnt(0x0F70);
+            m_a = geo_open(g);
+            SEGK_RS_LOAD_M(g, xa, m_a);
+            geo_issue(g + n_slots);
+            for (;;) {
+                __builtin_amdgcn_s_waitcnt(0x0F70);
+                const int64_t g1 = g + n_slots;
+                if (g1 < n_groups) {
+                    m_b = geo_open(g1);
+                    SEGK_RS_LOAD_M(g1, xb, m_b);
+                }
+                geo_issue(g1 + n_slots);
+                SEGK_RS_STORE();
+                SEGK_RS_GROUP_M(g, xa, m_a);
+                if (g1 >= n_groups) break;
+                __builtin_amdgcn_s_waitcnt(0x0F70);
+                g = g1 + n_slots;
+                if (g < n_groups) {
+                    m_a = geo_open(g);
+                    SEGK_RS_LOAD_M(g, xa, m_a);
+                }
+                geo_issue(g + n_slots);
+                SEGK_RS_STORE();
+                SEGK_RS_GROUP_M(g1, xb, m_b);
+                if (g >= n_groups) break;
+            }
+#undef SEGK_RS_GROUP_M
+            SEGK_RS_STORE();
+            if (lane == 0) {
+                if (n_rows_out > 0) atomicAdd(H.ctl + 23, n_rows_out);
+                if (n_groups_out > 0) atomicAdd(H.ctl + 24, n_groups_out);
+            }
+            return;
+        }
+    }
 #ifdef SEGK_STAMP
     unsigned long long st_wait = 0, st_loop = 0, st_groups = 0;
     const unsigned long long st_begin = __builtin_amdgcn_s_memtime();
@@ -510,6 +624,7 @@
 #undef SEGK_RS_GROUP
 #undef SEGK_RS_TILE
 #undef SEGK_RS_UNIT
+#undef SEGK_RS_LOAD_M
 #undef SEGK_RS_LOAD
 }
 #undef SEGK_RS_DRAIN_QUAD
@@ -539,6 +654,8 @@
     const int32_t *meanchg;
     int32_t *lab_last;
     int32_t *stats_host;
+    const unsigned long long *gtab;
+    int32_t *geo_closed_cnt;
 };
 
 #define SEGK_MERGE_ROWS 6144
@@ -547,9 +664,9 @@
 {
     __shared__ int32_t ulist[SEGK_MERGE_ROWS];
     __shared__ float uthr[SEGK_MERGE_ROWS];
-    __shared__ int32_t ucnt, ubase;
+    __shared__ int32_t ucnt, ubase, gcnt;
     const int tid = threadIdx.x, lane = tid & 63;
-    if (tid == 0) ucnt = 0;
+    if (tid == 0) { ucnt = 0; gcnt = 0; }
     const int mw = H.ctl ? H.ctl[0] : 0;
     const bool delta = (mw & SEGK_DELTA_MODE) != 0;
     const int n_chg = H.ctl ? H.ctl[1] : 0, n_packed = H.ctl ? H.ctl[2] : 0;
@@ -569,6 +686,11 @@
                 bad |= !(H.tiles_hdr[1024 + (int64_t)(k >> 5) * A.tile_stride + c_off + (k & 31)] < -1.0e37f);
         carry = __syncthreads_or(bad ? 1 : 0) == 0;
     }
+    unsigned int gseq = 0;
+    int n_geo_means = 0;
+    const bool geo = carry && H.gtab && segk_geo_on(H.ctl, mw, &gseq, &n_geo_means);
+    int n_geo = 0;
+    if (H.geo_closed_cnt && blockIdx.x == 0 && tid == 0) H.geo_closed_cnt[3] = geo ? 1 : 0;
     const int64_t p_lo = (int64_t)blockIdx.x * per, p_hi = p_lo + per < A.n ? p_lo + per : A.n;
     const int e_ab = ((const int *)H.ximg)[1] + ((const int *)H.tiles_hdr)[0];
     const float unscale = ldexpf(1.f, -e_ab), scale = ldexpf(1.f, e_ab);
@@ -581,6 +703,7 @@
         float t1[U], t2[U], xnb[U], xer[U], d1[U];
         int32_t last[U];
         bool cw[U];
+        bool g5[U], nod[U];
 #pragma unroll
         for (int j = 0; j < U; j++) {
             const int64_t p = p0 + j * SEGK_MERGE_THREADS + tid;
@@ -606,22 +729,29 @@
             d1[j] = NEG_INF_F;
             last[j] = -2;
             cw[j] = false;
-            if (rid[j] >= 0 && carry) {
+            g5[j] = false;
+            nod[j] = false;
+            if (rid[j] >= 0 && (carry || geo)) {
                 const int32_t hint = __float_as_int(ho[j].z);
                 last[j] = H.lab_last[p];
                 cw[j] = hint >= 0 && last[j] == hint && H.meanchg[hint] == 0;
+                if (geo && cw[j] && p < first_skipped) g5[j] =geo_closed((double)segk_geo_g(H.gtab[hint], gseq), ho[j].x, A.D);
+                n_geo += g5[j] ? 1 : 0;
             }
-            if (rid[j] >= 0 && delta) {
+            if (rid[j] >= 0 && delta && !g5[j]) {
                 const int32_t hint = __float_as_int(ho[j].z);
                 if (hint >= 0 && H.colchg[hint] && H.lab_base[p] == hint) {
                     t1[j] = t2[j];
                 }
                 if (n_packed > 0) {
                     const float2 pv = H.part_delta[p];
-                    d1[j] = pv.x;
-                    const float n1 = fmaxf(t1[j], pv.x);
-                    t2[j] = fmaxf(fminf(t1[j], pv.x), fmaxf(t2[j], pv.y));
-                    t1[j] = n1;
+                    nod[j] = pv.x == SEGK_GEO_NO_PRODUCT;
+                    if (!nod[j]) {
+                        d1[j] = pv.x;
+                        const float n1 = fmaxf(t1[j], pv.x);
+                        t2[j] = fmaxf(fminf(t1[j], pv.x), fmaxf(t2[j], pv.y));
+                        t1[j] = n1;
+                    }
                 }
             }
         }
@@ -648,8 +778,8 @@
                     const float rnd = 1.00001f * fminf((xnb[j] + xer[j]) * Em + xer[j] * M, 1.01f * 9.765625e-4f * xnb[j] * M);
                     const float s2 = xnb[j] + M;
                     const float dl = ((float)(A.D / 8 + 13) + 4.f) * u * s2 * s2;
-                    ok = (top1 - top2 > tau) && (ho[j].y >= top1 - tau + (e1 + rnd + dl) * 1.0001f);
-                    const bool carried = !ok && cw[j] && ho[j].y > d1[j] * unscale + (e1 + rnd + dl) * 1.0001f;
+                    ok = !nod[j] && !g5[j] && (top1 - top2 > tau) && (ho[j].y >= top1 - tau + (e1 + rnd + dl) * 1.0001f);
+                    const bool carried = g5[j] || (!ok && carry && !nod[j] && cw[j] && ho[j].y > d1[j] * unscale + (e1 + rnd + dl) * 1.0001f);
                     if (ok || carried) {
                         A.cand.k[rid[j]] = hint;
                         A.cand.s[rid[j]] = (double)ho[j].x;
@@ -686,7 +816,12 @@
             }
         }
     }
+    if (geo) {
+        for (int o = 32; o > 0; o >>= 1) n_geo += __shfl_xor(n_geo, o);
+        if (lane == 0 && n_geo > 0) atomicAdd(&gcnt, n_geo);
+    }
     __syncthreads();
+    if (geo && tid == 0 && gcnt > 0) atomicAdd(H.geo_closed_cnt, gcnt);
     const int cnt = ucnt;
     if (cnt == 0) return;
     if (tid == 0) ubase = atomicAdd(A.pre_count, cnt);
@@ -766,6 +901,7 @@
     int32_t *colchg, *meanchg;
     float *snap_img;
     float *packed;
+    unsigned long long *gtab;
     float *snap_means;
     float2 *part;
     int32_t *lab_base;
@@ -786,6 +922,7 @@
     B->meanchg = (int32_t *)take((size_t)K_max * 4);
     B->snap_img = (float *)take(((size_t)n_tiles * TL + 4) * 4);
     B->packed = (float *)take((size_t)n_tiles * stride * 4);
+    B->gtab = (unsigned long long *)take((size_t)K_max * 8);
     B->zero_bytes = off;
     B->snap_means = (float *)take((size_t)K_max * D * 4);
     B->part = (float2 *)take((size_t)n * 8);
@@ -801,6 +938,7 @@
     return cap < 1 ? 1 : cap;
 }
 static int delta_budget(int n_tiles) { return segk_env_int("SEGK_DELTA_BUDGET", n_tiles); }
+static int geo_setting() { return segk_env_int("SEGK_SCORE_GEO", 1); }
 
 static DeltaPrepArgs delta_prep_args(segk_ctx *ctx, const DeltaBuf &B, const float *tiles, int n_tiles, int stride, int K_max, int D,
                                      const float *means32, const int32_t *remap, const int32_t *K_dev, bool valid, int cap, int budget,
@@ -815,6 +953,10 @@
     P.seq = redo_seq >= 0 ? redo_seq : (int)(ctx->delta_seq++ & 1u);
     P.ctl = B.ctl; P.colchg = B.colchg; P.meanchg = B.meanchg;
     P.snap_img = B.snap_img; P.packed = B.packed; P.snap_means = B.snap_means;
+    P.gseq = ++ctx->geo_seq;
+    if (P.gseq >= 0xFFFFFFF0u) ctx->geo_retired = 1;
+    P.geo = (valid && geo_setting() != 0 && !ctx->geo_retired) ? 1 : 0;
+    P.gtab = B.gtab;
     return P;
 }
 
@@ -837,6 +979,7 @@
     ctx->delta_pending = 1;
     ctx->delta_pending_remap = remap; ctx->delta_pending_K = m->K; ctx->delta_pending_stream = (const void *)st;
     ctx->delta_pending_cap = cap; ctx->delta_pending_budget = budget; ctx->delta_pending_seq = P->seq;
+    ctx->delta_pending_geo = P->geo;
     return true;
 }
 
@@ -869,7 +1012,8 @@
     const int budget = delta_budget(A.n_tiles);
     const bool folded = pending == 1 && state_valid && remap == ctx->delta_pending_remap && K_dev == ctx->delta_pending_K &&
                         (const void *)st == ctx->delta_pending_stream && *cap == ctx->delta_pending_cap &&
-                        budget == ctx->delta_pending_budget;
+                        budget == ctx->delta_pending_budget &&
+                        ctx->delta_pending_geo == ((geo_setting() != 0 && !ctx->geo_retired) ? 1 : 0);
     if (!folded) {
         const DeltaPrepArgs P = delta_prep_args(ctx, *B, A.tiles, A.n_tiles, stride_sp, A.K_max, A.D, A.means32, remap, K_dev, state_valid,
                                                 *cap, budget, pending != 0 && state_valid ? ctx->delta_pending_seq : -1);
@@ -905,13 +1049,19 @@
     H.nxx = A.xerr + n_emb;
     H.hint_out = L.hint_out;
     H.ctl = B.ctl; H.meanchg = B.meanchg; H.snap_img = B.snap_img;
+    H.geo_all = geo_setting() == 2 ? 1 : 0;
     H.full = K1Set{A.tiles + 1024, A.n_tiles, L.lds.tpr, L.lds.n_ranges, (float2 *)ctx->hint_part, L.grid};
     size_t lds = (size_t)L.lds.tpr * TL * sizeof(float) + L.lds.map_bytes;
     int grid = L.grid;
     if (B.ctl) {
         const int64_t steps = (A.n + 64 * SEGK_K1_NW - 1) / (64 * SEGK_K1_NW);
         H.delta = K1Set{B.packed, 0, delta_cap, 1, B.part, (int64_t)ctx->n_cu > steps ? (int)steps : ctx->n_cu};
-        const size_t lds_d = (size_t)delta_cap * TL * sizeof(float) + L.lds.map_bytes;
+        size_t lds_d = (size_t)delta_cap * TL * sizeof(float) + L.lds.map_bytes;
+        H.geo_k1 = (KS <= 7 && geo_setting() != 0 && A.ids == nullptr && lds_d + L.lds.map_bytes <= 160 * 1024) ? 1 : 0;
+        if (H.geo_k1) lds_d += L.lds.map_bytes;
+        H.gtab = B.gtab;
+        H.lab_last = B.lab_last;
+        H.colchg = B.colchg;
         if (H.delta.grid > grid) grid = H.delta.grid;
         if (lds_d > lds) lds = lds_d;
     }
@@ -955,6 +1105,8 @@
     E.meanchg = B.meanchg;
     E.lab_last = B.lab_last;
     E.stats_host = ctx->delta_host_dev;
+    E.gtab = B.gtab;
+    E.geo_closed_cnt = B.ctl ? B.ctl + 22 : nullptr;
     int64_t grid = (int64_t)ctx->n_cu;
     if (grid * SEGK_MERGE_THREADS > A.n) grid = (A.n + SEGK_MERGE_THREADS - 1) / SEGK_MERGE_THREADS;
     if (grid * SEGK_MERGE_ROWS < A.n) grid = (A.n + SEGK_MERGE_ROWS - 1) / SEGK_MERGE_ROWS;
@@ -977,7 +1129,7 @@
     if (int rc = launch_delta_prep<KS>(ctx, A, remap, K_dev, n_emb, L, st, &B, &delta_cap)) return rc;
     if (int rc = launch_k1<KS>(ctx, A, remap, n_emb, L, B, delta_cap, st)) return rc;
     launch_merge(ctx, A, L, B, KS, st);
-    if (L.band) return segk_launch_band(ctx, A, ctx->pre_thr, A.n, B.lab_last, KS, st);
+    if (L.band) return segk_launch_band(ctx, A, ctx->pre_thr, A.n, B.lab_last, B.ctl, KS, st);
     ScoreArgs B2 = A;
     B2.ids = A.pre_queue;
     B2.row0 = 0;
diff --git a/segmentalist_amd/device.py b/segmentalist_amd/device.py
--- a/segmentalist_amd/device.py
+++ b/segmentalist_amd/device.py
@@ -275,6 +275,11 @@
     def delta_stats(self):
         out = (C.c_int32 * 4)()
         check(self._L.segk_kmeans_delta_stats(self._ctx, out))
+        return tuple(int(v) for v in out)
+
+    def geo_stats(self):
+        out = (C.c_int32 * 4)()
+        check(self._L.segk_kmeans_geo_stats(self._ctx, out))
         return tuple(int(v) for v in out)
 
     def score_ptr(self, ids_ptr, n):
```

Result: slower. 6960 sweeps/s (-3.7%).
